# MDFahimAnjum/AliasFree-Diffusion-Models-PyTorch

Hardware: AMD Instinct MI355X
Metric: train_step_images_per_sec (higher is better)
Workload: dtype f32; 1 GPU; CIFAR-10 32x32x3 synthetic, UNet variant=3 (Config D), batch 256/GPU, T=1000, AdamW lr 3e-4, random-init weights (seed 42); global_batch=256, parallelism=dp1, hip_graph=True, launch_mode=lanes

## Files before the change

### aliasfree-diffusion-models-pytorch_amd/csrc/conv.hip

```cpp
#include <cstdlib>
#include <algorithm>
#include "common.h"

namespace afd {

using f32x16 = __attribute__((ext_vector_type(16))) float;

static inline int gs_grid(long total, int block = 256) {
  long g = (total + block - 1) / block;
  return (int)(g < 1 ? 1 : (g > 65536 ? 65536 : g));
}

template <int KS>
__global__ void conv_direct_fwd(const float* __restrict__ x, const float* __restrict__ w, const float* __restrict__ bias,
                                const float* __restrict__ res, float* __restrict__ y,
                                int Cin, int Cout, int H, int W, int act, long total) {
  constexpr int T = KS * KS, R = KS / 2;
  for (long i = blockIdx.x * (long)blockDim.x + threadIdx.x; i < total; i += (long)gridDim.x * blockDim.x) {
    const int xx = i % W, yy = (i / W) % H;
    const long bc = i / ((long)W * H);
    const int co = bc % Cout; const long b = bc / Cout;
    float acc = bias ? bias[co] : 0.f;
    for (int ci = 0; ci < Cin; ++ci) {
      const float* xp = x + (b * Cin + ci) * (long)H * W;
      const float* wp = w + ((long)co * Cin + ci) * T;
#pragma unroll
      for (int a = 0; a < KS; ++a) {
        const int r = yy + a - R;
        if (r < 0 || r >= H) continue;
#pragma unroll
        for (int c = 0; c < KS; ++c) {
          const int q = xx + c - R;
          if (q < 0 || q >= W) continue;
          acc += wp[a * KS + c] * xp[(long)r * W + q];
        }
      }
    }
    if (act == 1) acc = gelu_erf(acc);
    if (res) acc += res[i];
    y[i] = acc;
  }
}

template <int KS>
__global__ void conv_direct_dgrad(const float* __restrict__ dy, const float* __restrict__ w, float* __restrict__ dx,
                                  int Cin, int Cout, int H, int W, long total) {
  constexpr int T = KS * KS, R = KS / 2;
  for (long i = blockIdx.x * (long)blockDim.x + threadIdx.x; i < total; i += (long)gridDim.x * blockDim.x) {
    const int xx = i % W, yy = (i / W) % H;
    const long bc = i / ((long)W * H);
    const int ci = bc % Cin; const long b = bc / Cin;
    float acc = 0.f;
    for (int co = 0; co < Cout; ++co) {
      const float* gp = dy + (b * Cout + co) * (long)H * W;
      const float* wp = w + ((long)co * Cin + ci) * T;
#pragma unroll
      for (int a = 0; a < KS; ++a) {
        const int r = yy - a + R;
        if (r < 0 || r >= H) continue;
#pragma unroll
        for (int c = 0; c < KS; ++c) {
          const int q = xx - c + R;
          if (q < 0 || q >= W) continue;
          acc += wp[a * KS + c] * gp[(long)r * W + q];
        }
      }
    }
    dx[i] = acc;
  }
}

template <int KS>
__global__ __launch_bounds__(256) void conv_direct_wgrad(const float* __restrict__ x, const float* __restrict__ dy,
                                                         float* __restrict__ dw, int B, int Cin, int Cout, int H, int W,
                                                         int accumulate) {
  constexpr int T = KS * KS, R = KS / 2;
  __shared__ float red[16];
  const int co = blockIdx.x / Cin, ci = blockIdx.x % Cin;
  float acc[T];
#pragma unroll
  for (int t = 0; t < T; ++t) acc[t] = 0.f;
  const long HW = (long)H * W, P = (long)B * HW;
  for (long p = threadIdx.x; p < P; p += blockDim.x) {
    const long b = p / HW; const int pix = p % HW; const int yy = pix / W, xx = pix % W;
    const float g = dy[(b * Cout + co) * HW + pix];
    const float* xp = x + (b * Cin + ci) * HW;
#pragma unroll
    for (int a = 0; a < KS; ++a) {
      const int r = yy + a - R;
#pragma unroll
      for (int c = 0; c < KS; ++c) {
        const int q = xx + c - R;
        if (r >= 0 && r < H && q >= 0 && q < W) acc[a * KS + c] += g * xp[(long)r * W + q];
      }
    }
  }
#pragma unroll
  for (int t = 0; t < T; ++t) {
    const float s = block_sum(acc[t], red);
    if (threadIdx.x == 0) {
      float* o = dw + ((long)co * Cin + ci) * T + t;
      *o = accumulate ? *o + s : s;
    }
  }
}

__global__ __launch_bounds__(256) void conv_dbias_plane(const float* __restrict__ dy, float* __restrict__ part, long planes, int HW) {
  const long pl = ((long)blockIdx.x * blockDim.x + threadIdx.x) >> 6;
  const int lane = threadIdx.x & 63;
  if (pl >= planes) return;
  float s = 0.f;
  for (int i = lane; i < HW; i += 64) s += dy[pl * HW + i];
  s = wave_sum(s);
  if (lane == 0) part[pl] = s;
}
__global__ __launch_bounds__(256) void conv_dbias_final(const float* __restrict__ part, float* __restrict__ db, int B, int Cout, int accumulate) {
  __shared__ float red[8][33];
  const int c = blockIdx.x * 32 + (threadIdx.x & 31), g = threadIdx.x >> 5;
  float s = 0.f;
  if (c < Cout) for (int b = g; b < B; b += 8) s += part[(long)b * Cout + c];
  red[g][threadIdx.x & 31] = s;
  __syncthreads();
  if (g == 0 && c < Cout) {
    float t = 0.f;
#pragma unroll
    for (int k = 0; k < 8; ++k) t += red[k][threadIdx.x & 31];
    db[c] = accumulate ? db[c] + t : t;
  }
}

struct TileGeom {
  int TI, TR;
  int Wp;
  int BS;
  int XS;
};
static inline bool tile_ok(int H, int W, int PT) {
  const int HW = H * W;
  return (HW % PT == 0 && PT % W == 0) || (PT % HW == 0);
}
static inline TileGeom make_geom(int H, int W, int PT, int halo) {
  TileGeom g;
  const int HW = H * W;
  if (HW >= PT) { g.TI = 1; g.TR = PT / W; } else { g.TI = PT / HW; g.TR = H; }
  g.Wp = W + 2 * halo;
  g.BS = (g.TR + 2 * halo) * g.Wp;
  g.XS = g.TI * g.BS;
  return g;
}

__device__ __forceinline__ int pix_lds_off(int m, int W, const TileGeom& g, int halo) {
  const int per_img = g.TR * W;
  const int ti = m / per_img, r = (m % per_img) / W, c = m % W;
  return ti * g.BS + (r + halo) * g.Wp + (c + halo);
}

__device__ __forceinline__ void pos_source(int pos, long p0, int H, int W, long P, const TileGeom& g, int halo,
                                           long& img, int& off) {
  const int HW = H * W;
  const int ti = pos / g.BS, rem = pos % g.BS;
  const int rr = rem / g.Wp - halo, cc = rem % g.Wp - halo;
  const long pimg = p0 / HW + ti;
  const int row0 = (int)((p0 % HW) / W);
  const int y = row0 + rr;
  img = pimg; off = -1;
  if (cc < 0 || cc >= W || y < 0 || y >= H) return;
  if (pimg * HW >= P) return;
  off = y * W + cc;
}

template <int T, bool DGRAD, int BN, int KC, int NP>
struct Stager {
  static constexpr int WS = KC * T + 1;
  static constexpr int NW = BN * KC * T / 256;
  static_assert(BN * KC * T % 256 == 0, "weight chunk must divide over 256 threads");
  float wreg[NW];
  float xreg[NP][KC];
  unsigned long long wok;
  unsigned xok[NP];

  __device__ __forceinline__ void fetch(const float* __restrict__ w, const float* __restrict__ x, int k0, int K, int N,
                                        int n0, int HW, const int (&spos)[NP], const int (&soff)[NP],
                                        const long (&simg)[NP], int XS) {
    wok = 0;
#pragma unroll
    for (int e = 0; e < NW; ++e) {
      const int i = threadIdx.x + 256 * e;
      int n, kc, t;
      if (!DGRAD) { n = i / (KC * T); const int r = i % (KC * T); kc = r / T; t = r % T; }
      else        { kc = i / (BN * T); const int r = i % (BN * T); n = r / T; t = r % T; }
      const bool ok = (n0 + n < N) && (k0 + kc < K);
      const int nc = min(n0 + n, N - 1), kk = min(k0 + kc, K - 1);
      wreg[e] = DGRAD ? w[(unsigned)((kk * N + nc) * T + t)] : w[(unsigned)((nc * K + kk) * T + t)];
      wok |= (ok ? 1ull : 0ull) << e;
    }
#pragma unroll
    for (int p = 0; p < NP; ++p) {
      xok[p] = 0;
      if (spos[p] < XS) {
        const unsigned xb = soff[p] >= 0 ? (unsigned)simg[p] * (unsigned)(K * HW) + (unsigned)soff[p] : 0u;
#pragma unroll
        for (int kc = 0; kc < KC; ++kc) {
          xreg[p][kc] = x[xb + (unsigned)(min(k0 + kc, K - 1) * HW)];
          xok[p] |= ((soff[p] >= 0 && k0 + kc < K) ? 1u : 0u) << kc;
        }
      }
    }
  }

  __device__ __forceinline__ void commit(float* __restrict__ Ws, float* __restrict__ Xs, const int (&spos)[NP], int XS) const {
#pragma unroll
    for (int e = 0; e < NW; ++e) {
      const int i = threadIdx.x + 256 * e;
      int dst;
      if (!DGRAD) { dst = (i / (KC * T)) * WS + i % (KC * T); }
      else        { const int kc = i / (BN * T), r = i % (BN * T); dst = (r / T) * WS + kc * T + r % T; }
      Ws[dst] = ((wok >> e) & 1ull) ? wreg[e] : 0.f;
    }
#pragma unroll
    for (int p = 0; p < NP; ++p)
      if (spos[p] < XS) {
#pragma unroll
        for (int kc = 0; kc < KC; ++kc) Xs[kc * XS + spos[p]] = ((xok[p] >> kc) & 1u) ? xreg[p][kc] : 0.f;
      }
  }
};

template <int GEO> struct Geo { static constexpr int XS = 0, Wp = 0; };
template <> struct Geo<1> { static constexpr int XS = 204, Wp = 34; };
template <> struct Geo<2> { static constexpr int XS = 180, Wp = 18; };
template <> struct Geo<3> { static constexpr int XS = 200, Wp = 10; };
template <> struct Geo<4> { static constexpr int XS = 288, Wp = 6; };
template <> struct Geo<5> { static constexpr int XS = 128, Wp = 0; };

template <int T, bool DGRAD, int BN, int KC, int GEO>
__global__ __launch_bounds__(256) void conv_mfma(const float* __restrict__ x, const float* __restrict__ w,
                                                 const float* __restrict__ bias, const float* __restrict__ res,
                                                 float* __restrict__ y, int B, int K, int N, int H, int W, int act,
                                                 TileGeom g) {
  constexpr int PT = 128, HALO = (T == 9) ? 1 : 0;
  constexpr int TM = (BN == 64) ? 2 : 1;
  constexpr int WS = KC * T + 1;
  constexpr int NP = (T == 9) ? 2 : 1;
  constexpr int NW = BN * KC * T / 256;
  static_assert(BN * KC * T % 256 == 0, "weight chunk must divide over 256 threads");
  const int XS = GEO ? Geo<GEO>::XS : g.XS;
  const int Wp = GEO ? Geo<GEO>::Wp : g.Wp;
  extern __shared__ __attribute__((aligned(16))) float smem[];
  const int BUF = BN * WS + KC * XS;
  const int HW = H * W;
  const long P = (long)B * HW;
  const long p0 = (long)blockIdx.y * PT;
  const int n0 = blockIdx.x * BN;
  const int lane = threadIdx.x & 63, wv = threadIdx.x >> 6;
  const int nw = (BN == 64) ? (wv >> 1) * 32 : 0;
  const int mw = (BN == 64) ? (wv & 1) * 64 : wv * 32;
  const int half = lane >> 5, l31 = lane & 31;

  unsigned wsrc[NW]; int wdst[NW]; unsigned wmask = 0;
  int wkc[NW];
#pragma unroll
  for (int e = 0; e < NW; ++e) {
    const int i = threadIdx.x + 256 * e;
    int n, kc, t;
    if (!DGRAD) { n = i / (KC * T); const int r = i % (KC * T); kc = r / T; t = r % T; }
    else        { kc = i / (BN * T); const int r = i % (BN * T); n = r / T; t = r % T; }
    const int nc = min(n0 + n, N - 1);
    wsrc[e] = DGRAD ? (unsigned)((kc * N + nc) * T + t) : (unsigned)(nc * K * T + kc * T + t);
    wdst[e] = n * WS + kc * T + t;
    wkc[e] = kc;
    wmask |= (n0 + n < N ? 1u : 0u) << e;
  }
  int spos[NP]; unsigned xsrc[NP]; bool xval[NP];
#pragma unroll
  for (int e = 0; e < NP; ++e) {
    spos[e] = threadIdx.x + 256 * e;
    int soff = -1; long simg = 0;
    if (spos[e] < XS) pos_source(spos[e], p0, H, W, P, g, HALO, simg, soff);
    xval[e] = soff >= 0;
    xsrc[e] = xval[e] ? (unsigned)simg * (unsigned)(K * HW) + (unsigned)soff : 0u;
  }
  const int wstep = DGRAD ? N * T : T;
  int lbase[TM];
#pragma unroll
  for (int mt = 0; mt < TM; ++mt) lbase[mt] = half * XS + pix_lds_off(mw + mt * 32 + l31, W, g, HALO);
  const int abase = (nw + l31) * WS + half * T;

  float wreg[NW], xreg[NP][KC];
  auto fetch = [&](int k0) {
    const float* __restrict__ wk = w + (long)k0 * wstep;
    const float* __restrict__ xk = x + (long)k0 * HW;
    if (k0 + KC <= K) {
#pragma unroll
      for (int e = 0; e < NW; ++e) wreg[e] = wk[wsrc[e]];
#pragma unroll
      for (int p = 0; p < NP; ++p)
        if (spos[p] < XS) {
#pragma unroll
          for (int kc = 0; kc < KC; ++kc) xreg[p][kc] = xk[xsrc[p] + (unsigned)(kc * HW)];
        }
    } else {
#pragma unroll
      for (int e = 0; e < NW; ++e) wreg[e] = (k0 + wkc[e] < K) ? wk[wsrc[e]] : 0.f;
#pragma unroll
      for (int p = 0; p < NP; ++p)
        if (spos[p] < XS) {
#pragma unroll
          for (int kc = 0; kc < KC; ++kc) xreg[p][kc] = (k0 + kc < K) ? xk[xsrc[p] + (unsigned)(kc * HW)] : 0.f;
        }
    }
  };
  auto commit = [&](float* __restrict__ buf) {
    float* __restrict__ Ws = buf;
    float* __restrict__ Xs = buf + BN * WS;
#pragma unroll
    for (int e = 0; e < NW; ++e) Ws[wdst[e]] = ((wmask >> e) & 1u) ? wreg[e] : 0.f;
#pragma unroll
    for (int p = 0; p < NP; ++p)
      if (spos[p] < XS) {
#pragma unroll
        for (int kc = 0; kc < KC; ++kc) Xs[kc * XS + spos[p]] = xval[p] ? xreg[p][kc] : 0.f;
      }
  };

  f32x16 acc[TM];
#pragma unroll
  for (int mt = 0; mt < TM; ++mt)
#pragma unroll
    for (int r = 0; r < 16; ++r) acc[mt][r] = 0.f;

  fetch(0);
  commit(smem);
  if (KC < K) fetch(KC);
  __syncthreads();
  int cur = 0;
  for (int k0 = 0; k0 < K; k0 += KC, cur ^= 1) {
    if (k0 + KC < K) {
      commit(smem + (cur ^ 1) * BUF);
      if (k0 + 2 * KC < K) fetch(k0 + 2 * KC);
    }
    const float* __restrict__ Ws = smem + cur * BUF;
    const float* __restrict__ Xs = Ws + BN * WS;
#pragma unroll
    for (int t = 0; t < T; ++t) {
      const int toff = (T == 9) ? ((t / 3 - 1) * Wp + (t % 3 - 1)) : 0;
      const int tw = DGRAD ? (T - 1 - t) : t;
#pragma unroll
      for (int k2 = 0; k2 < KC / 2; ++k2) {
        const float a = Ws[abase + 2 * k2 * T + tw];
#pragma unroll
        for (int mt = 0; mt < TM; ++mt)
          acc[mt] = __builtin_amdgcn_mfma_f32_32x32x2f32(a, Xs[lbase[mt] + 2 * k2 * XS + toff], acc[mt], 0, 0, 0);
      }
    }
    __syncthreads();
  }
#pragma unroll
  for (int mt = 0; mt < TM; ++mt) {
    const long p = p0 + mw + mt * 32 + l31;
    if (p >= P) continue;
    const long b = p / HW; const int pix = p % HW;
#pragma unroll
    for (int r = 0; r < 16; ++r) {
      const int n = n0 + nw + (r & 3) + 8 * (r >> 2) + 4 * half;
      if (n >= N) continue;
      const long idx = (b * N + n) * (long)HW + pix;
      float v = acc[mt][r];
      if (bias) v += bias[n];
      if (act == 1) v = gelu_erf(v);
      if (res) v += res[idx];
      y[idx] = v;
    }
  }
}

template <int T, bool DGRAD>
__global__ __launch_bounds__(256) void conv_mfma_sk(const float* __restrict__ x, const float* __restrict__ w,
                                                    const float* __restrict__ bias, const float* __restrict__ res,
                                                    float* __restrict__ y, int B, int K, int N, int H, int W, int act,
                                                    TileGeom g) {
  constexpr int PT = 64, BN = 32, KC = 32, KW = KC / 4, TM = 2, HALO = (T == 9) ? 1 : 0;
  constexpr int WS = KC * T + 1;
  extern __shared__ __attribute__((aligned(16))) float smem[];
  float* Ws = smem;
  float* Xs = smem + BN * WS;
  const int HW = H * W;
  const long P = (long)B * HW;
  const long p0 = (long)blockIdx.y * PT;
  const int n0 = blockIdx.x * BN;
  const int lane = threadIdx.x & 63, wv = threadIdx.x >> 6;
  const int half = lane >> 5, l31 = lane & 31;

  int spos[1] = {(int)threadIdx.x}, soff[1] = {-1}; long simg[1] = {0};
  if (spos[0] < g.XS) pos_source(spos[0], p0, H, W, P, g, HALO, simg[0], soff[0]);
  int poff[TM];
#pragma unroll
  for (int mt = 0; mt < TM; ++mt) poff[mt] = pix_lds_off(mt * 32 + l31, W, g, HALO);

  f32x16 acc[TM];
#pragma unroll
  for (int mt = 0; mt < TM; ++mt)
#pragma unroll
    for (int r = 0; r < 16; ++r) acc[mt][r] = 0.f;

  Stager<T, DGRAD, BN, KC, 1> st;
  st.fetch(w, x, 0, K, N, n0, HW, spos, soff, simg, g.XS);
  for (int k0 = 0; k0 < K; k0 += KC) {
    __syncthreads();
    st.commit(Ws, Xs, spos, g.XS);
    __syncthreads();
    if (k0 + KC < K) st.fetch(w, x, k0 + KC, K, N, n0, HW, spos, soff, simg, g.XS);
#pragma unroll
    for (int t = 0; t < T; ++t) {
      const int toff = (T == 9) ? ((t / 3 - 1) * g.Wp + (t % 3 - 1)) : 0;
      const int tw = DGRAD ? (T - 1 - t) : t;
#pragma unroll
      for (int k2 = 0; k2 < KW / 2; ++k2) {
        const int kc = wv * KW + 2 * k2 + half;
        const float a = Ws[l31 * WS + kc * T + tw];
#pragma unroll
        for (int mt = 0; mt < TM; ++mt)
          acc[mt] = __builtin_amdgcn_mfma_f32_32x32x2f32(a, Xs[kc * g.XS + poff[mt] + toff], acc[mt], 0, 0, 0);
      }
    }
  }
  __syncthreads();
  float* red = smem;
#pragma unroll
  for (int mt = 0; mt < TM; ++mt)
#pragma unroll
    for (int r = 0; r < 16; ++r) red[((wv * TM + mt) * 16 + r) * 64 + lane] = acc[mt][r];
  __syncthreads();
#pragma unroll
  for (int e = 0; e < (TM * 16 * 64) / 256; ++e) {
    const int idx = threadIdx.x + 256 * e;
    const int mt = idx / 1024, r = (idx / 64) % 16, ln = idx % 64;
    float v = (red[idx] + red[idx + 2048]) + (red[idx + 4096] + red[idx + 6144]);
    const long p = p0 + mt * 32 + (ln & 31);
    const int n = n0 + (r & 3) + 8 * (r >> 2) + 4 * (ln >> 5);
    if (p < P && n < N) {
      const long b = p / HW; const int pix = p % HW;
      const long o = (b * N + n) * (long)HW + pix;
      if (bias) v += bias[n];
      if (act == 1) v = gelu_erf(v);
      if (res) v += res[o];
      y[o] = v;
    }
  }
}

template <int T, int WNn, int WCn, int NPB, int NW>
__global__ __launch_bounds__(64 * NW) void conv_wgrad_mfma(const float* __restrict__ x, const float* __restrict__ dy,
                                                       float* __restrict__ part, float* __restrict__ bias_part,
                                                       int B, int Cin, int Cout, int H, int W,
                                                       int chunks_per_split, int nchunks, TileGeom g) {
  constexpr int PT = 64, HALO = (T == 9) ? 1 : 0, S1 = PT + 1;
  constexpr int WK = NW / (WNn * WCn), BNo = 32 * WNn, BCi = 32 * WCn, NT_ = 64 * NW;
  constexpr int NG = BNo / NW;
  constexpr int NM = BCi / (2 * NW);
  extern __shared__ __attribute__((aligned(16))) float smem[];
  const int XSP = g.XS | 1;
  float* Gs = smem;
  float* Xs = smem + BNo * S1;
  int* Po = reinterpret_cast<int*>(Xs + BCi * XSP);
  const int HW = H * W;
  const long P = (long)B * HW;
  const int n0 = blockIdx.x * BNo, c0 = blockIdx.y * BCi, split = blockIdx.z;
  const int lane = threadIdx.x & 63, wv = threadIdx.x >> 6;
  const int wn = wv % WNn, wc = (wv / WNn) % WCn, wk = wv / (WNn * WCn);
  const int nw = wn * 32, cw = wc * 32;
  const int half = lane >> 5, l31 = lane & 31;
  const bool active = (n0 + nw < Cout) && (c0 + cw < Cin);

  if (threadIdx.x < PT) Po[threadIdx.x] = pix_lds_off(threadIdx.x, W, g, HALO);

  const int pp = threadIdx.x & 63, ng = threadIdx.x >> 6;
  const int gdb = (HW >= PT) ? 0 : pp / HW;
  const int gpix = (HW >= PT) ? pp : pp % HW;
  const int px = threadIdx.x & 31, cg = threadIdx.x >> 5;
  int p_ti[NPB], p_rr[NPB], p_cc[NPB];
#pragma unroll
  for (int e = 0; e < NPB; ++e) {
    const int pos = px + 32 * e;
    const int ti = pos / g.BS, rem = pos % g.BS;
    p_ti[e] = pos < g.XS ? ti : -1;
    p_rr[e] = rem / g.Wp - HALO;
    p_cc[e] = rem % g.Wp - HALO;
  }

  float gv[NG], xv[NPB][NM];
  unsigned gok, xok[NPB];
  int f_img, f_pix, f_row;
  auto fetch = [&]() {
    {
      const int b = f_img + gdb;
      const bool pin = b < B;
      const unsigned gb = pin ? (unsigned)(b * Cout) * (unsigned)HW + (unsigned)(f_pix + gpix) : 0u;
      gok = 0;
#pragma unroll
      for (int e = 0; e < NG; ++e) {
        const int n = n0 + ng + NW * e;
        gv[e] = dy[gb + (unsigned)(min(n, Cout - 1) * HW)];
        gok |= ((pin && n < Cout) ? 1u : 0u) << e;
      }
    }
#pragma unroll
    for (int e = 0; e < NPB; ++e) {
      xok[e] = 0;
      if (p_ti[e] >= 0) {
        const int img = f_img + p_ti[e];
        const int yy = f_row + p_rr[e];
        const bool ok = p_cc[e] >= 0 && p_cc[e] < W && yy >= 0 && yy < H && img < B;
        const unsigned xb = ok ? (unsigned)(img * Cin) * (unsigned)HW + (unsigned)(yy * W + p_cc[e]) : 0u;
#pragma unroll
        for (int m = 0; m < NM; ++m) {
          const int c = c0 + cg + 2 * NW * m;
          xv[e][m] = x[xb + (unsigned)(min(c, Cin - 1) * HW)];
          xok[e] |= ((ok && c < Cin) ? 1u : 0u) << m;
        }
      }
    }
    if (HW >= PT) {
      f_pix += PT; f_row += g.TR;
      if (f_pix >= HW) { f_pix = 0; f_row = 0; ++f_img; }
    } else {
      f_img += g.TI;
    }
  };
  auto commit = [&]() {
#pragma unroll
    for (int e = 0; e < NG; ++e) Gs[(ng + NW * e) * S1 + pp] = ((gok >> e) & 1u) ? gv[e] : 0.f;
#pragma unroll
    for (int e = 0; e < NPB; ++e)
      if (p_ti[e] >= 0) {
#pragma unroll
        for (int m = 0; m < NM; ++m) Xs[(cg + 2 * NW * m) * XSP + px + 32 * e] = ((xok[e] >> m) & 1u) ? xv[e][m] : 0.f;
      }
  };

  f32x16 acc[T];
#pragma unroll
  for (int t = 0; t < T; ++t)
#pragma unroll
    for (int r = 0; r < 16; ++r) acc[t][r] = 0.f;
  const bool do_bias = bias_part != nullptr && blockIdx.y == 0;
  float bsum = 0.f;

  const int cbeg = split * chunks_per_split;
  const int cend = min(nchunks, cbeg + chunks_per_split);
  {
    const unsigned pc0 = (unsigned)cbeg * PT;
    f_img = (int)(pc0 / (unsigned)HW);
    f_pix = (int)(pc0 % (unsigned)HW);
    f_row = f_pix / W;
  }
  if (cbeg < cend) fetch();
  for (int ch = cbeg; ch < cend; ++ch) {
    __syncthreads();
    commit();
    __syncthreads();
    if (ch + 1 < cend) fetch();
    if (do_bias) {
      const int bn = threadIdx.x >> 2, bq = threadIdx.x & 3;
      if (bn < BNo) {
        float t = 0.f;
#pragma unroll
        for (int j = 0; j < 16; ++j) t += Gs[bn * S1 + bq * 16 + j];
        bsum += t;
      }
    }
    if (active) {
#pragma unroll 4
      for (int s = wk * (PT / 2 / WK); s < (wk + 1) * (PT / 2 / WK); ++s) {
        const int pix = 2 * s + half;
        const float a = Gs[(nw + l31) * S1 + pix];
        const int xo = (cw + l31) * XSP + Po[pix];
#pragma unroll
        for (int t = 0; t < T; ++t) {
          const int toff = (T == 9) ? ((t / 3 - 1) * g.Wp + (t % 3 - 1)) : 0;
          acc[t] = __builtin_amdgcn_mfma_f32_32x32x2f32(a, Xs[xo + toff], acc[t], 0, 0, 0);
        }
      }
    }
  }
  if (do_bias) {
    float t = bsum;
    t += __shfl_xor(t, 1, kWave);
    t += __shfl_xor(t, 2, kWave);
    const int bn = threadIdx.x >> 2;
    if ((threadIdx.x & 3) == 0 && bn < BNo && n0 + bn < Cout) bias_part[(long)split * Cout + n0 + bn] = t;
  }
  float* out = part + (long)split * Cout * Cin * T;
  if (WK == 1) {
    if (!active) return;
    const int ci = c0 + cw + l31;
    if (ci < Cin) {
#pragma unroll
      for (int r = 0; r < 16; ++r) {
        const int n = n0 + nw + (r & 3) + 8 * (r >> 2) + 4 * half;
        if (n >= Cout) continue;
#pragma unroll
        for (int t = 0; t < T; ++t) out[((long)t * Cout + n) * Cin + ci] = acc[t][r];
      }
    }
  } else {
    float* red = smem;
    constexpr int NB = WNn * WCn;
#pragma unroll
    for (int t = 0; t < T; ++t) {
      __syncthreads();
#pragma unroll
      for (int r = 0; r < 16; ++r) red[(wv * 16 + r) * 64 + lane] = acc[t][r];
      __syncthreads();
      for (int idx = threadIdx.x; idx < NB * 1024; idx += NT_) {
        const int blk = idx / 1024, r = (idx / 64) % 16, ln = idx % 64;
        float v = 0.f;
#pragma unroll
        for (int k = 0; k < WK; ++k) v += red[((k * NB + blk) * 16 + r) * 64 + ln];
        const int bn = blk % WNn, bc = blk / WNn;
        const int n = n0 + bn * 32 + (r & 3) + 8 * (r >> 2) + 4 * (ln >> 5);
        const int ci = c0 + bc * 32 + (ln & 31);
        if (n < Cout && ci < Cin) out[((long)t * Cout + n) * Cin + ci] = v;
      }
    }
  }
}

__global__ __launch_bounds__(256) void wgrad_reduce(const float* __restrict__ part, float* __restrict__ dw, long n, int splits,
                                                    const float* __restrict__ bias_part, float* __restrict__ db, int nb,
                                                    int accumulate, int T) {
  __shared__ float red[8][33];
  const long i = (long)blockIdx.x * 32 + (threadIdx.x & 31);
  const int g = threadIdx.x >> 5;
  const bool isw = i < n;
  const long j = isw ? i : i - n;
  const long stride = isw ? n : nb;
  const float* __restrict__ src = isw ? part : bias_part;
  float s0 = 0.f, s1 = 0.f, s2 = 0.f, s3 = 0.f;
  if (i < n + nb) {
    int k = g;
    for (; k + 24 < splits; k += 32) {
      s0 += src[(long)k * stride + j]; s1 += src[(long)(k + 8) * stride + j];
      s2 += src[(long)(k + 16) * stride + j]; s3 += src[(long)(k + 24) * stride + j];
    }
    for (; k < splits; k += 8) s0 += src[(long)k * stride + j];
  }
  red[g][threadIdx.x & 31] = (s0 + s1) + (s2 + s3);
  __syncthreads();
  if (g == 0 && i < n + nb) {
    float t = 0.f;
#pragma unroll
    for (int k = 0; k < 8; ++k) t += red[k][threadIdx.x & 31];
    const long plane = n / T;
    float* o = isw ? dw + (j % plane) * T + j / plane : db + j;
    *o = accumulate ? *o + t : t;
  }
}

__global__ __launch_bounds__(256) void wgrad_reduce4(const float* __restrict__ part, float* __restrict__ dw, long n, int splits,
                                                     const float* __restrict__ bias_part, float* __restrict__ db, int nb,
                                                     int accumulate, int T) {
  __shared__ float4 red4[8][32];
  const int l = threadIdx.x & 31, g = threadIdx.x >> 5;
  const long wblocks = n >> 7;
  if (blockIdx.x < wblocks) {
    const long j = ((long)blockIdx.x << 7) + 4 * l;
    const float4* __restrict__ src = reinterpret_cast<const float4*>(part + j);
    const long stride = n >> 2;
    float4 s0 = {0.f, 0.f, 0.f, 0.f}, s1 = s0, s2 = s0, s3 = s0;
    int k = g;
    for (; k + 24 < splits; k += 32) {
      const float4 a = src[(long)k * stride], b = src[(long)(k + 8) * stride], c = src[(long)(k + 16) * stride],
                   d = src[(long)(k + 24) * stride];
      s0.x += a.x; s0.y += a.y; s0.z += a.z; s0.w += a.w;
      s1.x += b.x; s1.y += b.y; s1.z += b.z; s1.w += b.w;
      s2.x += c.x; s2.y += c.y; s2.z += c.z; s2.w += c.w;
      s3.x += d.x; s3.y += d.y; s3.z += d.z; s3.w += d.w;
    }
    for (; k < splits; k += 8) {
      const float4 a = src[(long)k * stride];
      s0.x += a.x; s0.y += a.y; s0.z += a.z; s0.w += a.w;
    }
    red4[g][l] = make_float4((s0.x + s1.x) + (s2.x + s3.x), (s0.y + s1.y) + (s2.y + s3.y), (s0.z + s1.z) + (s2.z + s3.z),
                             (s0.w + s1.w) + (s2.w + s3.w));
    __syncthreads();
    if (threadIdx.x < 128) {
      const int e = threadIdx.x;
      float t = 0.f;
#pragma unroll
      for (int q = 0; q < 8; ++q) t += reinterpret_cast<const float*>(&red4[q][e >> 2])[e & 3];
      const long je = ((long)blockIdx.x << 7) + e, plane = n / T;
      float* o = dw + (je % plane) * T + je / plane;
      *o = accumulate ? *o + t : t;
    }
  } else {
    __shared__ float red[8][33];
    const long j = (long)(blockIdx.x - wblocks) * 32 + l;
    float s0 = 0.f;
    if (j < nb)
      for (int k = g; k < splits; k += 8) s0 += bias_part[(long)k * nb + j];
    red[g][l] = s0;
    __syncthreads();
    if (g == 0 && j < nb) {
      float t = 0.f;
#pragma unroll
      for (int q = 0; q < 8; ++q) t += red[q][l];
      db[j] = accumulate ? db[j] + t : t;
    }
  }
}

int fold_launch(const afd_fold_desc* descs, int n, hipStream_t s);

struct FoldSink { afd_fold_desc* out; int n; };
static int launch_wgrad_reduce(const float* part, float* dw, long n, int slabs, const float* bp, float* db, int nb, int accumulate,
                               int T, hipStream_t s, FoldSink* sink) {
  afd_fold_desc d[2];
  int nd = 0;
  d[nd++] = afd_fold_desc{part, dw, n, n, n / T, (long)T, slabs, accumulate};
  if (nb > 0) d[nd++] = afd_fold_desc{bp, db, (long)nb, (long)nb, (long)nb, 1L, slabs, accumulate};
  if (sink) {
    for (int i = 0; i < nd; ++i) sink->out[sink->n++] = d[i];
    return AFD_OK;
  }
  return fold_launch(d, nd, s);
}

bool pw_launch(const float* in, const float* w, const float* bias, const float* res, float* out, int B, int K, int N, int P,
               int act, bool dgrad, hipStream_t s);
void pw_set_mode(int m);
int wino_plan(int B, int K, int N, int H, int W);
bool wino_conv(const float* x, const float* w, const float* bias, const float* res, float* y, float* U, int B, int K, int N, int H,
               int W, int act, bool dgrad, bool weights_ready, hipStream_t s);
void wino_set_mode(int m);
void wino_weights_launch(const float* w, float* Uf, float* Ud, int Cin, int Cout, int kinds, hipStream_t s);
bool bf3_ok(int B, int K, int N, int H, int W);
void bf3_set_mode(int m);
void direct_form_set(int m);
bool direct_form_is_bf3();
void h2_sk_set_mode(int m);
void h2_lds_set(int m);
void wino_weights_batched_launch(const afd_wino_desc* descs, const int* wg_desc, int n_wg, hipStream_t s);
void wino_set_grid(int g);
int wgrad_wino_plan(int B, int Cin, int Cout, int H, int W, int* bn, int* bk, int* cps, int* nchunks);
int wgrad_bf3_plan(int B, int Cin, int Cout, int H, int W, int* tps, int* ntiles);
int wgrad_bf3(const float* x, const float* dy, float* part, int B, int Cin, int Cout, int H, int W, hipStream_t s);
void wgrad_bf3_set_mode(int m);
void wgrad_arith_set(int m);
void wgrad_plan_target_set(long wgs);
bool wgrad_arith_is_bf3();
int wgrad_h2(const float* x, const float* dy, float* part, int B, int Cin, int Cout, int H, int W, hipStream_t s);
int pw_wgrad_h2(const float* x, const float* dy, float* part, float* bias_part, int B, int Cin, int Cout, int L, hipStream_t s);
bool ends_fwd(const float* x, const float* w, const float* bias, const float* res, float* y, int B, int Cin, int Cout, int H, int W,
              int ksize, int act, hipStream_t s);
bool ends_dgrad(const float* dy, const float* w, float* dx, int B, int Cin, int Cout, int H, int W, int ksize, hipStream_t s);
void ends_set_mode(int m);
int wgrad_cin3_plan(int B, int Cin, int Cout, int H, int W);
int wgrad_cin3(const float* x, const float* dy, float* part, int B, int Cin, int Cout, int H, int W, hipStream_t s);
void pw_wgrad_bf3_set_mode(int m);
int pw_wgrad_bf3_plan(int B, int Cin, int Cout, int L, int* sps, int* nsteps, int* nr, int* nt);
int pw_wgrad_bf3(const float* x, const float* dy, float* part, float* bias_part, int B, int Cin, int Cout, int L, hipStream_t s);
int wgrad_wino(const float* x, const float* dy, float* part, int B, int Cin, int Cout, int H, int W, hipStream_t s);
void wgrad_wino_set_mode(int m);

static inline bool use_mfma(int K, int N, int H, int W, int PT) { return N >= 8 && tile_ok(H, W, PT); }

static int g_conv_path = 0;

template <int T, bool DGRAD>
static int launch_mfma(const float* x, const float* w, const float* bias, const float* res, float* y,
                       int B, int K, int N, int H, int W, int act, hipStream_t s) {
  constexpr int KC = (T == 9) ? 8 : 32;
  const long P = (long)B * H * W;
  if (P * K >= (1L << 31) || (long)K * N * T >= (1L << 31)) return -1;
  const unsigned ptiles = (unsigned)((P + 127) / 128);
  const long wgs64 = (long)ptiles * ((N + 63) / 64), wgs32 = (long)ptiles * ((N + 31) / 32);
  bool use32 = N <= 32 || (wgs64 < 256 && wgs32 >= 256);
  const bool want_sk = g_conv_path == 2 || (g_conv_path == 0 && wgs64 < 256 && wgs32 < 256);
  if (g_conv_path == 1) use32 = N <= 32;
  if (want_sk && K >= 32 && tile_ok(H, W, 64)) {
    const TileGeom g = make_geom(H, W, 64, T == 9 ? 1 : 0);
    if (g.XS <= 256) {
      const size_t lds_main = sizeof(float) * (32 * (32 * T + 1) + (size_t)32 * g.XS);
      const size_t lds_red = sizeof(float) * 4 * 2 * 16 * 64;
      const size_t lds = lds_main > lds_red ? lds_main : lds_red;
      hipLaunchKernelGGL((conv_mfma_sk<T, DGRAD>), dim3((N + 31) / 32, (unsigned)((P + 63) / 64)), dim3(256), lds, s,
                         x, w, bias, res, y, B, K, N, H, W, act, g);
      return 0;
    }
  }
  const TileGeom g = make_geom(H, W, 128, T == 9 ? 1 : 0);
  if (g.XS > 512) return -1;
  int geo = 0;
  if (T == 1) geo = 5;
  else if (H == W && (W == 32 || W == 16 || W == 8 || W == 4)) geo = W == 32 ? 1 : (W == 16 ? 2 : (W == 8 ? 3 : 4));
  const size_t lds = 2 * sizeof(float) * ((use32 ? 32 : 64) * (KC * T + 1) + (size_t)KC * g.XS);
  const dim3 grid(use32 ? (N + 31) / 32 : (N + 63) / 64, ptiles);
#define AFD_CONV_LAUNCH(BN_, GEO_) hipLaunchKernelGGL((conv_mfma<T, DGRAD, BN_, KC, GEO_>), grid, dim3(256), lds, s, x, w, bias, res, y, B, K, N, H, W, act, g)
#define AFD_CONV_GEO(BN_)                                             \
  switch (geo) {                                                       \
    case 1: if constexpr (T == 9) { AFD_CONV_LAUNCH(BN_, 1); } break;  \
    case 2: if constexpr (T == 9) { AFD_CONV_LAUNCH(BN_, 2); } break;  \
    case 3: if constexpr (T == 9) { AFD_CONV_LAUNCH(BN_, 3); } break;  \
    case 4: if constexpr (T == 9) { AFD_CONV_LAUNCH(BN_, 4); } break;  \
    case 5: if constexpr (T == 1) { AFD_CONV_LAUNCH(BN_, 5); } break;  \
    default: AFD_CONV_LAUNCH(BN_, 0);                                  \
  }
  if (!use32) { AFD_CONV_GEO(64) } else { AFD_CONV_GEO(32) }
#undef AFD_CONV_GEO
#undef AFD_CONV_LAUNCH
  return 0;
}

static int g_wgrad_nw = 0;
struct WgradPlan { int wnn, wcn, wk, splits, slabs, nchunks, cps, npb; };
static inline WgradPlan wgrad_plan(int B, int Cin, int Cout, int H, int W, int ksize) {
  WgradPlan p;
  p.wnn = Cout > 32 ? 2 : 1;
  p.wcn = Cin > 32 ? 2 : 1;
  p.wk = 4 / (p.wnn * p.wcn);
  p.nchunks = (int)(((long)B * H * W + 63) / 64);
  const long tiles = (long)((Cout + 32 * p.wnn - 1) / (32 * p.wnn)) * ((Cin + 32 * p.wcn - 1) / (32 * p.wcn));
  static const long target = [] { const char* e = getenv("AFD_WG_TARGET"); return e ? atol(e) : 256L; }();
  long s = target / tiles;
  if (s < 1) s = 1;
  if (s > p.nchunks) s = p.nchunks;
  p.cps = (int)((p.nchunks + s - 1) / s);
  p.splits = (int)((p.nchunks + p.cps - 1) / p.cps);
  p.slabs = p.splits;
  const TileGeom g = make_geom(H, W, 64, ksize == 3 ? 1 : 0);
  const int need = (g.XS + 31) / 32;
  p.npb = ksize == 1 ? 2 : (need <= 4 ? 4 : (need <= 5 ? 5 : 8));
  return p;
}

template <int T, int WNn, int WCn, int NPB>
static void launch_wgrad(const float* x, const float* dy, float* part, float* bias_part, int B, int Cin, int Cout, int H, int W,
                         const WgradPlan& p, const TileGeom& g, hipStream_t s) {
  const int nw = g_wgrad_nw ? g_wgrad_nw : ((p.cps >= 8 || (p.cps >= 4 && H * W >= 256)) ? 8 : 4);
  size_t lds = sizeof(float) * ((size_t)32 * WNn * 65 + (size_t)32 * WCn * (g.XS | 1)) + sizeof(int) * 64;
  const size_t red = sizeof(float) * nw * 16 * 64;
  if (WNn * WCn < nw && lds < red) lds = red;
  const dim3 grid((Cout + 32 * WNn - 1) / (32 * WNn), (Cin + 32 * WCn - 1) / (32 * WCn), p.splits);
  if (nw == 8)
    hipLaunchKernelGGL((conv_wgrad_mfma<T, WNn, WCn, NPB, 8>), grid, dim3(512), lds, s, x, dy, part, bias_part, B, Cin, Cout, H, W, p.cps, p.nchunks, g);
  else
    hipLaunchKernelGGL((conv_wgrad_mfma<T, WNn, WCn, NPB, 4>), grid, dim3(256), lds, s, x, dy, part, bias_part, B, Cin, Cout, H, W, p.cps, p.nchunks, g);
}

template <int T, int NPB>
static void launch_wgrad_roles(const float* x, const float* dy, float* part, float* bp, int B, int Cin, int Cout, int H, int W,
                               const WgradPlan& p, const TileGeom& g, hipStream_t s) {
  if (p.wnn == 2 && p.wcn == 2) launch_wgrad<T, 2, 2, NPB>(x, dy, part, bp, B, Cin, Cout, H, W, p, g, s);
  else if (p.wnn == 2) launch_wgrad<T, 2, 1, NPB>(x, dy, part, bp, B, Cin, Cout, H, W, p, g, s);
  else if (p.wcn == 2) launch_wgrad<T, 1, 2, NPB>(x, dy, part, bp, B, Cin, Cout, H, W, p, g, s);
  else launch_wgrad<T, 1, 1, NPB>(x, dy, part, bp, B, Cin, Cout, H, W, p, g, s);
}

}
using namespace afd;

extern "C" {

int afd_debug_conv_path(int mode) {
  if (mode >= 92 && mode <= 93) { ends_set_mode(mode - 92); return AFD_OK; }
  if (mode >= 88 && mode <= 89) { pw_wgrad_bf3_set_mode(mode - 88); return AFD_OK; }
  if (mode >= 84 && mode <= 86) { wgrad_bf3_set_mode(mode - 84); return AFD_OK; }
  if (mode >= 48 && mode <= 49) { wgrad_plan_target_set(mode == 48 ? 256 : 160); return AFD_OK; }
  if (mode >= 59 && mode <= 63) { h2_lds_set(mode == 59 ? 4 : (mode == 60 ? 1 : (mode == 61 ? 0 : mode - 60))); return AFD_OK; }
  if (mode == 73) { h2_sk_set_mode(2); return AFD_OK; }
  if (mode >= 74 && mode <= 75) { h2_sk_set_mode(mode - 74); return AFD_OK; }
  if (mode >= 78 && mode <= 79) { wgrad_arith_set(mode - 78); return AFD_OK; }
  if (mode >= 76 && mode <= 77) { direct_form_set(mode - 76); return AFD_OK; }
  if (mode >= 80 && mode <= 82) { bf3_set_mode(mode - 80); return AFD_OK; }
  if (mode >= 8 && mode <= 10) { pw_set_mode(mode - 8); return AFD_OK; }
  if (mode >= 100000 && mode < 200000) { wino_set_grid(mode - 100000); return AFD_OK; }
  if (mode >= 96 && mode <= 98) { wgrad_wino_set_mode(mode - 96); return AFD_OK; }
  if (mode >= 64 && mode <= 70) { wino_set_mode(mode - 64); return AFD_OK; }
  if (mode >= 32 && mode <= 34) { g_wgrad_nw = mode == 32 ? 4 : (mode == 33 ? 8 : 0); return AFD_OK; }
  AFD_REQUIRE(mode >= 0 && mode <= 2, "afd_debug_conv_path: mode must be 0 (auto), 1 (big tile), 2 (split-K tile), 8..10 (1x1 streaming auto/off/forced), 32..34 (wgrad waves 4/8/auto), 64..69 (Winograd fwd/dgrad auto/off/forced shapes) or 96..98 (Winograd wgrad auto/off/forced)");
  g_conv_path = mode;
  return AFD_OK;
}

int afd_conv_fwd(const float* x, const float* w, const float* bias, const float* res, float* y,
                 int B, int Cin, int Cout, int H, int W, int ksize, int act, afd_stream_t st) {
  AFD_REQUIRE(x && w && y && B > 0 && Cin > 0 && Cout > 0 && H > 0 && W > 0, "afd_conv_fwd: bad argument");
  AFD_REQUIRE(ksize == 1 || ksize == 3, "afd_conv_fwd: ksize %d not in {1,3}", ksize);
  AFD_REQUIRE(act == 0 || act == 1, "afd_conv_fwd: act must be 0 or 1");
  hipStream_t s = as_stream(st);
  if (ends_fwd(x, w, bias, res, y, B, Cin, Cout, H, W, ksize, act, s)) return check_launch("afd_conv_fwd");
  if (ksize == 1 && pw_launch(x, w, bias, res, y, B, Cin, Cout, H * W, act, false, s)) return check_launch("afd_conv_fwd");
  int rc = -1;
  if (use_mfma(Cin, Cout, H, W, 128))
    rc = ksize == 3 ? launch_mfma<9, false>(x, w, bias, res, y, B, Cin, Cout, H, W, act, s)
                    : launch_mfma<1, false>(x, w, bias, res, y, B, Cin, Cout, H, W, act, s);
  if (rc != 0) {
    const long total = (long)B * Cout * H * W;
    if (ksize == 3) hipLaunchKernelGGL(conv_direct_fwd<3>, dim3(gs_grid(total)), dim3(256), 0, s, x, w, bias, res, y, Cin, Cout, H, W, act, total);
    else hipLaunchKernelGGL(conv_direct_fwd<1>, dim3(gs_grid(total)), dim3(256), 0, s, x, w, bias, res, y, Cin, Cout, H, W, act, total);
  }
  return check_launch("afd_conv_fwd");
}

int afd_conv_dgrad(const float* dy, const float* w, float* dx, int B, int Cin, int Cout, int H, int W, int ksize, afd_stream_t st) {
  AFD_REQUIRE(dy && w && dx && B > 0 && Cin > 0 && Cout > 0 && H > 0 && W > 0, "afd_conv_dgrad: bad argument");
  AFD_REQUIRE(ksize == 1 || ksize == 3, "afd_conv_dgrad: ksize %d not in {1,3}", ksize);
  hipStream_t s = as_stream(st);
  if (ends_dgrad(dy, w, dx, B, Cin, Cout, H, W, ksize, s)) return check_launch("afd_conv_dgrad");
  if (ksize == 1 && pw_launch(dy, w, nullptr, nullptr, dx, B, Cout, Cin, H * W, 0, true, s)) return check_launch("afd_conv_dgrad");
  int rc = -1;
  if (use_mfma(Cout, Cin, H, W, 128))
    rc = ksize == 3 ? launch_mfma<9, true>(dy, w, nullptr, nullptr, dx, B, Cout, Cin, H, W, 0, s)
                    : launch_mfma<1, true>(dy, w, nullptr, nullptr, dx, B, Cout, Cin, H, W, 0, s);
  if (rc != 0) {
    const long total = (long)B * Cin * H * W;
    if (ksize == 3) hipLaunchKernelGGL(conv_direct_dgrad<3>, dim3(gs_grid(total)), dim3(256), 0, s, dy, w, dx, Cin, Cout, H, W, total);
    else hipLaunchKernelGGL(conv_direct_dgrad<1>, dim3(gs_grid(total)), dim3(256), 0, s, dy, w, dx, Cin, Cout, H, W, total);
  }
  return check_launch("afd_conv_dgrad");
}

size_t afd_conv3x3_wino_workspace_bytes(int B, int Cin, int Cout, int H, int W, int dgrad) {
  if (B <= 0 || Cin <= 0 || Cout <= 0 || H <= 0 || W <= 0) return 0;
  const int K = dgrad ? Cout : Cin, N = dgrad ? Cin : Cout;
  return (bf3_ok(B, K, N, H, W) || wino_plan(B, K, N, H, W)) ? sizeof(float) * 16 * (size_t)Cin * Cout : 0;
}

int afd_conv3x3_weight_kinds(int B, int Cin, int Cout, int H, int W) {
  if (B <= 0 || Cin <= 0 || Cout <= 0 || H <= 0 || W <= 0) return 0;
  const int k = (bf3_ok(B, Cin, Cout, H, W) ? 1 : 0) | (bf3_ok(B, Cout, Cin, H, W) ? 2 : 0);
  return k && direct_form_is_bf3() ? k | 4 : k;
}

int afd_conv3x3_wino_weights(const float* w, float* u_fwd, float* u_dgrad, int Cin, int Cout, int kinds, afd_stream_t st) {
  AFD_REQUIRE(w && (u_fwd || u_dgrad) && Cin > 0 && Cout > 0 && Cin % 8 == 0 && Cout % 8 == 0, "afd_conv3x3_wino_weights: bad argument");
  AFD_REQUIRE(kinds >= 0 && kinds <= 7 && (!(kinds & 4) || (kinds & 3)) && (!(kinds & 3) || (Cin % 16 == 0 && Cout % 16 == 0)), "afd_conv3x3_wino_weights: bad kinds %d", kinds);
  wino_weights_launch(w, u_fwd, u_dgrad, Cin, Cout, kinds, as_stream(st));
  return check_launch("afd_conv3x3_wino_weights");
}

int afd_conv3x3_wino_weights_batched(const afd_wino_desc* descs, const int* wg_desc, int n_wg, afd_stream_t st) {
  AFD_REQUIRE(descs && wg_desc && n_wg > 0, "afd_conv3x3_wino_weights_batched: bad argument");
  wino_weights_batched_launch(descs, wg_desc, n_wg, as_stream(st));
  return check_launch("afd_conv3x3_wino_weights_batched");
}

static int check_kinds(const char* who, int kinds, int B, int Cin, int Cout, int H, int W, int dgrad) {
  const int now = afd_conv3x3_weight_kinds(B, Cin, Cout, H, W);
  const int bit = dgrad ? 2 : 1;
  AFD_REQUIRE(kinds >= 0 && (kinds & bit) == (now & bit) && (!(now & bit) || (kinds & 4) == (now & 4)),
              "%s: the weight image was built as kinds %d, but a call with (B %d, %d -> %d, %dx%d) under the current settings reads kinds %d "
              "(rebuild it: afd_conv3x3_weight_kinds depends on the batch size and on afd_debug_conv_path)", who, kinds, B, Cin, Cout, H, W, now);
  return AFD_OK;
}

int afd_conv3x3_wino_fwd(const float* x, const float* w, const float* bias, const float* res, float* y,
                         int B, int Cin, int Cout, int H, int W, int act, void* workspace, int weights_ready, int kinds, afd_stream_t st) {
  AFD_REQUIRE(x && w && y && workspace && B > 0 && Cin > 0 && Cout > 0 && H > 0 && W > 0, "afd_conv3x3_wino_fwd: bad argument");
  AFD_REQUIRE(act == 0 || act == 1, "afd_conv3x3_wino_fwd: act must be 0 or 1");
  if (weights_ready && check_kinds("afd_conv3x3_wino_fwd", kinds, B, Cin, Cout, H, W, 0) != AFD_OK) return AFD_EINVAL;
  AFD_REQUIRE(wino_conv(x, w, bias, res, y, static_cast<float*>(workspace), B, Cin, Cout, H, W, act, false, weights_ready != 0, as_stream(st)),
              "afd_conv3x3_wino_fwd: shape (%d,%d->%d,%dx%d) is not covered (afd_conv3x3_wino_workspace_bytes returns 0 for it)", B, Cin, Cout, H, W);
  return check_launch("afd_conv3x3_wino_fwd");
}

int afd_conv3x3_wino_dgrad(const float* dy, const float* w, float* dx, const float* add_to_dx, int B, int Cin, int Cout, int H, int W,
                           void* workspace, int weights_ready, int kinds, afd_stream_t st) {
  AFD_REQUIRE(dy && w && dx && workspace && B > 0 && Cin > 0 && Cout > 0 && H > 0 && W > 0, "afd_conv3x3_wino_dgrad: bad argument");
  if (weights_ready && check_kinds("afd_conv3x3_wino_dgrad", kinds, B, Cin, Cout, H, W, 1) != AFD_OK) return AFD_EINVAL;
  AFD_REQUIRE(wino_conv(dy, w, nullptr, add_to_dx, dx, static_cast<float*>(workspace), B, Cout, Cin, H, W, 0, true, weights_ready != 0, as_stream(st)),
              "afd_conv3x3_wino_dgrad: shape (%d,%d->%d,%dx%d) is not covered", B, Cin, Cout, H, W);
  return check_launch("afd_conv3x3_wino_dgrad");
}

size_t afd_conv_wgrad_workspace_bytes(int B, int Cin, int Cout, int H, int W, int ksize) {
  if (B <= 0 || Cin <= 0 || Cout <= 0 || H <= 0 || W <= 0) return 0;
  size_t pw = 0;
  if (ksize == 1) {
    int a, b, c, d;
    pw = sizeof(float) * (size_t)pw_wgrad_bf3_plan(B, Cin, Cout, H * W, &a, &b, &c, &d) * ((size_t)Cout * Cin + Cout);
  }
  if (!tile_ok(H, W, 64)) return std::max(pw, sizeof(float) * (size_t)B * Cout);
  size_t slabs = wgrad_plan(B, Cin, Cout, H, W, ksize).slabs;
  if (ksize == 3) {
    int bn, bk, cps, nch;
    const size_t ws = (size_t)wgrad_wino_plan(B, Cin, Cout, H, W, &bn, &bk, &cps, &nch);
    if (ws > slabs) slabs = ws;
    const size_t wb = (size_t)wgrad_bf3_plan(B, Cin, Cout, H, W, &cps, &nch);
    if (wb > slabs) slabs = wb;
    const size_t wc = (size_t)wgrad_cin3_plan(B, Cin, Cout, H, W);
    if (wc > slabs) slabs = wc;
  }
  const size_t need = slabs * ((size_t)Cout * Cin * ksize * ksize + Cout);
  const size_t direct = (size_t)B * Cout;
  return std::max(pw, sizeof(float) * (need > direct ? need : direct));
}

int afd_conv_wgrad_form(int B, int Cin, int Cout, int H, int W, int ksize) {
  if (B <= 0 || Cin <= 0 || Cout <= 0 || H <= 0 || W <= 0) return 0;
  int a, b, c, d;
  if (ksize == 1) return pw_wgrad_bf3_plan(B, Cin, Cout, H * W, &a, &b, &c, &d) ? (wgrad_arith_is_bf3() ? 2 : 4) : 0;
  if (ksize != 3) return 0;
  if (wgrad_bf3_plan(B, Cin, Cout, H, W, &a, &b)) return wgrad_arith_is_bf3() ? 2 : 4;
  if (wgrad_cin3_plan(B, Cin, Cout, H, W)) return 3;
  return wgrad_wino_plan(B, Cin, Cout, H, W, &a, &b, &c, &d) ? 1 : 0;
}

static int conv_wgrad_impl(const float* x, const float* dy, float* dw, float* dbias, int B, int Cin, int Cout, int H, int W,
                           int ksize, int accumulate, void* workspace, FoldSink* sink, hipStream_t s, const char* who) {
  AFD_REQUIRE(x && dy && dw && B > 0 && Cin > 0 && Cout > 0 && H > 0 && W > 0, "%s: bad argument", who);
  AFD_REQUIRE(ksize == 1 || ksize == 3, "%s: ksize %d not in {1,3}", who, ksize);
  const int T = ksize * ksize;
  const TileGeom g = make_geom(H, W, 64, ksize == 3 ? 1 : 0);
  int rc = AFD_OK;
  if (ksize == 3 && !dbias && workspace) {
    float* part = static_cast<float*>(workspace);
    int slabs = wgrad_arith_is_bf3() ? wgrad_bf3(x, dy, part, B, Cin, Cout, H, W, s) : wgrad_h2(x, dy, part, B, Cin, Cout, H, W, s);
    if (!slabs) slabs = wgrad_cin3(x, dy, part, B, Cin, Cout, H, W, s);
    if (!slabs) slabs = wgrad_wino(x, dy, part, B, Cin, Cout, H, W, s);
    if (slabs) {
      const long n = (long)Cout * Cin * 9;
      rc = launch_wgrad_reduce(part, dw, n, slabs, nullptr, nullptr, 0, accumulate, 9, s, sink);
      return rc != AFD_OK ? rc : check_launch(who);
    }
  }
  if (ksize == 1 && workspace) {
    int a, b, c, d;
    const int slabs = pw_wgrad_bf3_plan(B, Cin, Cout, H * W, &a, &b, &c, &d);
    if (slabs) {
      float* part = static_cast<float*>(workspace);
      const long n = (long)Cout * Cin;
      float* bp = dbias ? part + (size_t)slabs * n : nullptr;
      if (wgrad_arith_is_bf3()) pw_wgrad_bf3(x, dy, part, bp, B, Cin, Cout, H * W, s);
      else pw_wgrad_h2(x, dy, part, bp, B, Cin, Cout, H * W, s);
      rc = launch_wgrad_reduce(part, dw, n, slabs, bp, dbias, dbias ? Cout : 0, accumulate, 1, s, sink);
      return rc != AFD_OK ? rc : check_launch(who);
    }
  }
  if (tile_ok(H, W, 64) && g.XS <= 256 && (long)B * H * W * (Cin > Cout ? Cin : Cout) < (1L << 31)) {
    AFD_REQUIRE(workspace, "%s: workspace is NULL", who);
    const WgradPlan p = wgrad_plan(B, Cin, Cout, H, W, ksize);
    float* part = static_cast<float*>(workspace);
    const long n = (long)Cout * Cin * T;
    float* bp = dbias ? part + (size_t)p.slabs * n : nullptr;
    if (ksize == 1) launch_wgrad_roles<1, 2>(x, dy, part, bp, B, Cin, Cout, H, W, p, g, s);
    else if (p.npb == 4) launch_wgrad_roles<9, 4>(x, dy, part, bp, B, Cin, Cout, H, W, p, g, s);
    else if (p.npb == 5) launch_wgrad_roles<9, 5>(x, dy, part, bp, B, Cin, Cout, H, W, p, g, s);
    else launch_wgrad_roles<9, 8>(x, dy, part, bp, B, Cin, Cout, H, W, p, g, s);
    rc = launch_wgrad_reduce(part, dw, n, p.slabs, bp, dbias, dbias ? Cout : 0, accumulate, T, s, sink);
    return rc != AFD_OK ? rc : check_launch(who);
  } else {
    const dim3 grid((unsigned)(Cout * Cin));
    if (ksize == 3) hipLaunchKernelGGL(conv_direct_wgrad<3>, grid, dim3(256), 0, s, x, dy, dw, B, Cin, Cout, H, W, accumulate);
    else hipLaunchKernelGGL(conv_direct_wgrad<1>, grid, dim3(256), 0, s, x, dy, dw, B, Cin, Cout, H, W, accumulate);
  }
  if (dbias) {
    AFD_REQUIRE(workspace, "%s: workspace is NULL", who);
    float* bp = static_cast<float*>(workspace);
    const long planes = (long)B * Cout;
    hipLaunchKernelGGL(conv_dbias_plane, dim3((unsigned)((planes + 3) / 4)), dim3(256), 0, s, dy, bp, planes, H * W);
    hipLaunchKernelGGL(conv_dbias_final, dim3((Cout + 31) / 32), dim3(256), 0, s, bp, dbias, B, Cout, accumulate);
  }
  return check_launch(who);
}

int afd_conv_wgrad(const float* x, const float* dy, float* dw, float* dbias, int B, int Cin, int Cout, int H, int W,
                   int ksize, int accumulate, void* workspace, afd_stream_t st) {
  return conv_wgrad_impl(x, dy, dw, dbias, B, Cin, Cout, H, W, ksize, accumulate, workspace, nullptr, as_stream(st), "afd_conv_wgrad");
}

int afd_conv_wgrad_partials(const float* x, const float* dy, float* dw, float* dbias, int B, int Cin, int Cout, int H, int W,
                            int ksize, int accumulate, void* workspace, afd_fold_desc* folds_out, int* n_folds, afd_stream_t st) {
  AFD_REQUIRE(folds_out && n_folds, "afd_conv_wgrad_partials: folds_out / n_folds are NULL");
  FoldSink sink{folds_out, 0};
  const int rc = conv_wgrad_impl(x, dy, dw, dbias, B, Cin, Cout, H, W, ksize, accumulate, workspace, &sink, as_stream(st), "afd_conv_wgrad_partials");
  *n_folds = sink.n;
  return rc;
}

}
```

### aliasfree-diffusion-models-pytorch_amd/csrc/h2.hip

```cpp
#include <algorithm>
#include <cstdint>
#include "common.h"
#include "h2_common.h"

namespace afd {

using f32x4 = __attribute__((ext_vector_type(4))) float;

#ifndef AFD_H2_ABL
#define AFD_H2_ABL 0
#endif
#ifndef AFD_H2_AQ
#define AFD_H2_AQ 2
#endif
#ifndef AFD_H2_PRIO
#define AFD_H2_PRIO 0
#endif
#ifndef AFD_H2_SLEEP
#define AFD_H2_SLEEP 0
#endif
#ifndef AFD_H2_LDSPAD
#define AFD_H2_LDSPAD 0
#endif
#ifndef AFD_H2_STAMP
#define AFD_H2_STAMP 0
#endif

__global__ __launch_bounds__(256) void h2_wscale(const float* __restrict__ w, void* Wf, void* Wd, int Cin, int Cout) {
  h2_wscale_rows(w, Wf, Wd, Cin, Cout, blockIdx.x * 4 + (threadIdx.x >> 6), gridDim.x * 4, threadIdx.x & 63);
}
__global__ __launch_bounds__(256) void h2_weights(const float* __restrict__ w, void* Wf, void* Wd, int Cin, int Cout) {
  h2_weights_block(w, Wf, Wd, Cin, Cout, blockIdx.x * 4 + (threadIdx.x >> 6), threadIdx.x & 63);
}

template <int S> struct H2Geo {
  static constexpr int TP = 128;
  static constexpr int IPT = S * S >= TP ? 1 : TP / (S * S);
  static constexpr int R = S * S >= TP ? TP / S : S;
  static constexpr int TPI = S * S >= TP ? S * S / TP : 1;
  static constexpr int Wp = S + 2, IMG = (R + 2) * Wp, NPIX = IPT * IMG;
  static constexpr int NPP = (NPIX + 15) / 16 * 16;
  static constexpr int KG = 4;
  static constexpr int TASKS = KG * NPIX, NE = (TASKS + 255) / 256;
  __device__ static void pixel(int blk, int l15, int& i, int& r, int& c) {
    if (S == 8) { i = blk >> 2; r = (blk & 3) + 4 * (l15 >> 3); c = l15 & 7; }
    else { const int q = blk * 16 + l15; i = q / (R * S); const int rem = q - i * (R * S); r = rem / S; c = rem - r * S; }
  }
};

template <int S, int NBLK>
__global__ __launch_bounds__(256, 2) void conv_h2(const float* __restrict__ x, const h8* __restrict__ Wp,
                                                  const float* __restrict__ bias, const float* __restrict__ res,
                                                  float* __restrict__ y, int B, int K, int N, int act) {
  using G = H2Geo<S>;
  constexpr int PSW = 2 * NBLK, NPIX = G::NPIX, NPP = G::NPP, NE = G::NE;
  extern __shared__ __attribute__((aligned(16))) uint8_t smem_raw[];
  h8* Xp = reinterpret_cast<h8*>(smem_raw);
  float* wmax = reinterpret_cast<float*>(smem_raw + (size_t)2 * G::KG * NPP * 16);
#if AFD_H2_SLEEP
  if (__builtin_amdgcn_s_getreg(6148) & 1) __builtin_amdgcn_s_sleep(AFD_H2_SLEEP);
#endif
#if AFD_H2_PRIO
  if (__builtin_amdgcn_s_getreg(6148) & 1) __builtin_amdgcn_s_setprio(AFD_H2_PRIO);
#endif
  const int tid = threadIdx.x, lane = tid & 63, wv = tid >> 6, kgl = lane >> 4, l15 = lane & 15;
  const int nb = wv % NBLK, pgrp = wv / NBLK;
  const int tile = blockIdx.x, n0 = (blockIdx.y * NBLK + nb) * 32;
  const int img0 = G::IPT > 1 ? tile * G::IPT : tile / G::TPI;
  const int row0 = G::IPT > 1 ? 0 : (tile % G::TPI) * G::R;
  const int HW = S * S;

  int s_src[NE];
  int s_dst[NE];
#pragma unroll
  for (int e = 0; e < NE; ++e) {
    const int t = tid + 256 * e;
    s_src[e] = -1; s_dst[e] = -1;
    if (t < G::TASKS) {
      const int kg = t / NPIX, ridx = t - kg * NPIX;
      const int i = ridx / G::IMG, rem = ridx - i * G::IMG, rr = rem / G::Wp, cc = rem - rr * G::Wp;
      const int yy = row0 + rr - 1, xx = cc - 1, b = img0 + i;
      s_dst[e] = kg * NPP + ridx;
      if (yy >= 0 && yy < S && xx >= 0 && xx < S && b < B) s_src[e] = ((i * K + 8 * kg) * S + yy) * S + xx;
    }
  }
  const float* xb = x + (long)img0 * K * HW;
  float xr[NE][8];
  auto fetch = [&](int k0) {
#pragma unroll
    for (int e = 0; e < NE; ++e) {
      const float* p = xb + (long)k0 * HW + (s_src[e] >= 0 ? s_src[e] : 0);
#pragma unroll
      for (int j = 0; j < 8; ++j) xr[e][j] = (S == 32 || s_src[e] >= 0) ? p[(long)j * HW] : 0.f;
    }
  };
  auto chunk_amax = [&]() {
    float m = 0.f;
#pragma unroll
    for (int e = 0; e < NE; ++e)
#pragma unroll
      for (int j = 0; j < 8; ++j) { xr[e][j] = s_src[e] >= 0 ? xr[e][j] : 0.f; m = fmaxf(m, fabsf(xr[e][j])); }
    m = wave_amax(m);
    if (lane == 0) wmax[wv] = m;
  };
  auto commit = [&](float s) {
#pragma unroll
    for (int e = 0; e < NE; ++e) {
      if (s_dst[e] < 0) continue;
      h8 p0, p1;
      h2_split8(xr[e], s, p0, p1);
      Xp[s_dst[e]] = p0;
      Xp[G::KG * NPP + s_dst[e]] = p1;
    }
  };

  int bbase[PSW];
#pragma unroll
  for (int ps = 0; ps < PSW; ++ps) {
    int i, r, c;
    G::pixel(pgrp * PSW + ps, l15, i, r, c);
    bbase[ps] = kgl * NPP + i * G::IMG + r * G::Wp + c;
  }
  f32x4 acc[2][PSW];
#pragma unroll
  for (int ns = 0; ns < 2; ++ns)
#pragma unroll
    for (int ps = 0; ps < PSW; ++ps) acc[ns][ps] = f32x4{0.f, 0.f, 0.f, 0.f};

  const int KS = K >> 5, nit = KS * 9;
  const long pstride = (long)9 * (K >> 3) * N;
  const h8* wl = Wp + (long)kgl * N + n0 + l15;
  auto a_load = [&](h8 (&a)[2][2], int it) {
    const int ks = it / 9, tap = it - ks * 9;
    const long r = ((long)tap * (K >> 3) + 4 * ks) * N;
#pragma unroll
    for (int ns = 0; ns < 2; ++ns) { a[ns][0] = wl[r + 16 * ns]; a[ns][1] = wl[pstride + r + 16 * ns]; }
  };
  constexpr int AQ = AFD_H2_AQ;
  h8 aq[AQ][2][2];
#pragma unroll
  for (int d = 0; d < AQ; ++d)
    if (d < nit) a_load(aq[d], d);

  float sx = __uint_as_float(kH2ScaleCapBits);
  fetch(0);
  int it = 0;
  for (int k0 = 0; k0 < K; k0 += 32) {
    const bool stage = !(AFD_H2_ABL & 8) || k0 == 0;
    if (stage) chunk_amax();
    __syncthreads();
    if (stage) {
      const float m = fmaxf(fmaxf(wmax[0], wmax[1]), fmaxf(wmax[2], wmax[3]));
      const float sn = fminf(sx, h2_scale_for(m));
      if (sn != sx) {
        const float f = sn * h2_inv_pow2(sx);
#pragma unroll
        for (int ns = 0; ns < 2; ++ns)
#pragma unroll
          for (int ps = 0; ps < PSW; ++ps) acc[ns][ps] *= f;
        sx = sn;
      }
    }
    if (stage) commit(sx);
    __syncthreads();
    h8 bc[2], bn[2];
    bc[0] = Xp[bbase[0]]; bc[1] = Xp[G::KG * NPP + bbase[0]];
#pragma unroll
    for (int tap = 0; tap < 9; ++tap) {
      h8 a[2][2];
#pragma unroll
      for (int ns = 0; ns < 2; ++ns) { a[ns][0] = aq[0][ns][0]; a[ns][1] = aq[0][ns][1]; }
#pragma unroll
      for (int d = 0; d + 1 < AQ; ++d)
#pragma unroll
        for (int ns = 0; ns < 2; ++ns) { aq[d][ns][0] = aq[d + 1][ns][0]; aq[d][ns][1] = aq[d + 1][ns][1]; }
      if (it + AQ < nit && !(AFD_H2_ABL & 2)) a_load(aq[AQ - 1], it + AQ);
      ++it;
      if (tap == 0 && k0 + 32 < K && !(AFD_H2_ABL & 4)) fetch(k0 + 32);
#pragma unroll
      for (int ps = 0; ps < PSW; ++ps) {
        const int u = tap * PSW + ps + 1;
        if (u < 9 * PSW && !(AFD_H2_ABL & 16)) {
          const int tn = u / PSW, pn = u % PSW;
          const int o = bbase[pn] + (tn / 3) * G::Wp + (tn % 3);
          bn[0] = Xp[o]; bn[1] = Xp[G::KG * NPP + o];
        } else if (AFD_H2_ABL & 16) { bn[0] = bc[0]; bn[1] = bc[1]; }
        __builtin_amdgcn_sched_barrier(0);
#pragma unroll
        for (int ns = 0; ns < 2; ++ns) {
          if (AFD_H2_ABL & 1) { asm volatile("" :: "v"(a[ns][0]), "v"(a[ns][1]), "v"(bc[0]), "v"(bc[1])); continue; }
          acc[ns][ps] = __builtin_amdgcn_mfma_f32_16x16x32_f16(a[ns][0], bc[0], acc[ns][ps], 0, 0, 0);
          acc[ns][ps] = __builtin_amdgcn_mfma_f32_16x16x32_f16(a[ns][1], bc[0], acc[ns][ps], 0, 0, 0);
          acc[ns][ps] = __builtin_amdgcn_mfma_f32_16x16x32_f16(a[ns][0], bc[1], acc[ns][ps], 0, 0, 0);
        }
        __builtin_amdgcn_sched_barrier(0);
        bc[0] = bn[0]; bc[1] = bn[1];
      }
    }
  }

  if ((AFD_H2_ABL & 32) && act != 77) return;
  const float* isw = reinterpret_cast<const float*>(reinterpret_cast<const uint8_t*>(Wp) + h2_scale_offset_bytes(K, N));
  const float isx = h2_inv_pow2(sx);
  __syncthreads();
  float* T = reinterpret_cast<float*>(smem_raw) + wv * (32 * 36);
  const int cn = lane >> 3, cm = lane & 7;
  float sw[4], bv[4];
#pragma unroll
  for (int it = 0; it < 4; ++it) { sw[it] = isw[n0 + 8 * it + cn]; bv[it] = bias ? bias[n0 + 8 * it + cn] : 0.f; }
#pragma unroll
  for (int pp = 0; pp < PSW / 2; ++pp) {
#pragma unroll
    for (int h = 0; h < 2; ++h)
#pragma unroll
      for (int ns = 0; ns < 2; ++ns)
#pragma unroll
        for (int rg = 0; rg < 4; ++rg) T[(16 * ns + 4 * kgl + rg) * 36 + 16 * h + l15] = acc[ns][2 * pp + h][rg] * isx;
    int i, r, c;
    G::pixel(pgrp * PSW + 2 * pp + (cm >> 2), 4 * (cm & 3), i, r, c);
    const int b = img0 + i;
#pragma unroll
    for (int it = 0; it < 4; ++it) {
      const int nn = n0 + 8 * it + cn;
      f32x4 v = *reinterpret_cast<const f32x4*>(T + (8 * it + cn) * 36 + 4 * cm);
      if (b >= B) continue;
      const long o = ((long)b * N + nn) * HW + (row0 + r) * S + c;
#pragma unroll
      for (int e = 0; e < 4; ++e) {
        float u = v[e] * sw[it] + bv[it];
        if (act == 1) u = gelu_erf(u);
        v[e] = u;
      }
      if (res) v += *reinterpret_cast<const f32x4*>(res + o);
      *reinterpret_cast<f32x4*>(y + o) = v;
    }
  }
}

using f32x16 = __attribute__((ext_vector_type(16))) float;

template <int S, int TP> struct H2LGeo {
  static constexpr int IPT = S * S >= TP ? 1 : TP / (S * S);
  static constexpr int R = S * S >= TP ? TP / S : S;
  static constexpr int TPI = S * S >= TP ? S * S / TP : 1;
  static constexpr int Wp = S + 2, IMG = (R + 2) * Wp, NPIX = IPT * IMG;
  static constexpr int NPP = (NPIX + 15) / 16 * 16;
  static constexpr int KG = 4, TASKS = KG * NPIX, NE = (TASKS + 255) / 256;
  __device__ static void pixel(int blk, int l31, int& i, int& r, int& c) {
    if (S == 8) { i = blk >> 1; r = 2 * (blk & 1) + ((l31 >> 4) & 1) + 4 * ((l31 >> 3) & 1); c = l31 & 7; }
    else { const int q = blk * 32 + l31; i = q / (R * S); const int rem = q - i * (R * S); r = rem / S; c = rem - r * S; }
  }
};

template <int S, int TP, int NB>
__global__ __launch_bounds__(256, 2) void conv_h2l(const float* __restrict__ x, const h8* __restrict__ Wp,
                                                   const float* __restrict__ bias, const float* __restrict__ res,
                                                   float* __restrict__ y, int B, int K, int N, int act) {
  using G = H2LGeo<S, TP>;
  constexpr int NT = 32 * NB, PGR = 4 / NB, PB = TP / 32 / PGR;
  constexpr int NPIX = G::NPIX, NPP = G::NPP, NE = G::NE;
  constexpr int XREC = 2 * G::KG * NPP;
  constexpr int AROW = 2 * 3 * 4 * NT;
  constexpr int CPW = AROW / 64 / 4;
  extern __shared__ __attribute__((aligned(16))) uint8_t smem_raw[];
  h8* Xp = reinterpret_cast<h8*>(smem_raw);
  h8* Ab = Xp + XREC;
  float* wmax = reinterpret_cast<float*>(Ab + 2 * AROW);
  const int tid = threadIdx.x, lane = tid & 63, wv = tid >> 6, l31 = lane & 31, lh = lane >> 5;
  const int nb = wv % NB, pgrp = wv / NB;
  const int tile = blockIdx.x, n0w = blockIdx.y * NT, n0 = n0w + 32 * nb;
  const int img0 = G::IPT > 1 ? tile * G::IPT : tile / G::TPI;
  const int row0 = G::IPT > 1 ? 0 : (tile % G::TPI) * G::R;
  const int HW = S * S;
#if AFD_H2_SLEEP
  if (((blockIdx.y * gridDim.x + blockIdx.x) >> 8) & 1) { for (int z = 0; z < AFD_H2_SLEEP / 100; ++z) __builtin_amdgcn_s_sleep(100); }
#endif
#if AFD_H2_STAMP
  long* stamp = tid == 0 ? reinterpret_cast<long*>(const_cast<float*>(res)) + ((long)blockIdx.y * gridDim.x + blockIdx.x) * 16 : nullptr;
  int si = 0;
  res = nullptr;
#define AFD_STAMP() do { if (stamp) stamp[si] = (long)__builtin_amdgcn_s_memtime(); ++si; } while (0)
  if (stamp) stamp[15] = __builtin_amdgcn_s_getreg(6148 | (15 << 11));
  AFD_STAMP();
#else
#define AFD_STAMP() do { } while (0)
#endif

  int s_src[NE], s_dst[NE];
#pragma unroll
  for (int e = 0; e < NE; ++e) {
    const int t = tid + 256 * e;
    s_src[e] = -1; s_dst[e] = -1;
    if (t < G::TASKS) {
      const int kg = t / NPIX, ridx = t - kg * NPIX;
      const int i = ridx / G::IMG, rem = ridx - i * G::IMG, rr = rem / G::Wp, cc = rem - rr * G::Wp;
      const int yy = row0 + rr - 1, xx = cc - 1, b = img0 + i;
      s_dst[e] = kg * NPP + ridx;
      if (yy >= 0 && yy < S && xx >= 0 && xx < S && b < B) s_src[e] = ((i * K + 8 * kg) * S + yy) * S + xx;
    }
  }
  const float* xb = x + (long)img0 * K * HW;
  float xr[NE][8];
  auto fetch = [&](int k0) {
#pragma unroll
    for (int e = 0; e < NE; ++e) {
      const float* p = xb + (long)k0 * HW + (s_src[e] >= 0 ? s_src[e] : 0);
#pragma unroll
      for (int j = 0; j < 8; ++j) xr[e][j] = p[(long)j * HW];
    }
  };
  auto chunk_amax = [&]() {
    float m = 0.f;
#pragma unroll
    for (int e = 0; e < NE; ++e)
#pragma unroll
      for (int j = 0; j < 8; ++j) { xr[e][j] = s_src[e] >= 0 ? xr[e][j] : 0.f; m = fmaxf(m, fabsf(xr[e][j])); }
    m = wave_amax(m);
    if (lane == 0) wmax[wv] = m;
  };
  auto commit = [&](float s) {
#pragma unroll
    for (int e = 0; e < NE; ++e) {
      if (s_dst[e] < 0) continue;
      h8 p0, p1;
      h2_split8(xr[e], s, p0, p1);
      Xp[s_dst[e]] = p0;
      Xp[G::KG * NPP + s_dst[e]] = p1;
    }
  };

  const int K8 = K >> 3;
  int soff[CPW];
#pragma unroll
  for (int d = 0; d < CPW; ++d) {
    const int c = wv * CPW + d;
    const int pt = NT == 64 ? c >> 2 : c >> 1, kg = NT == 64 ? c & 3 : 2 * (c & 1) + lh, n = NT == 64 ? lane : l31;
    const int pc = pt / 3, tx = pt - 3 * pc;
    soff[d] = ((pc * 9 + tx) * K8 + kg) * N + n0w + n;
  }
  auto dma_row = [&](int q) {
    const int ks = q / 3, ty = q - 3 * ks;
    const h8* src = Wp + (long)(ty * 3 * K8 + 4 * ks) * N;
    h8* dst = Ab + (q & 1) * AROW + wv * CPW * 64;
#pragma unroll
    for (int d = 0; d < CPW; ++d)
      __builtin_amdgcn_global_load_lds((const __attribute__((address_space(1))) void*)(src + soff[d]),
                                       (__attribute__((address_space(3))) void*)(dst + d * 64), 16, 0, 0);
  };
#define AFD_ROW_END(younger)                                                                                              \
  do {                                                                                                                    \
    __builtin_amdgcn_sched_barrier(0);                                                                                    \
    __builtin_amdgcn_s_waitcnt(((younger) & 15) | 0x0F70 | (((younger) >> 4) << 14));                \
    asm volatile("" ::: "memory");                                                                                        \
    __builtin_amdgcn_s_barrier();                                                                                         \
    asm volatile("" ::: "memory");                                                                                        \
    __builtin_amdgcn_sched_barrier(0);                                                                                    \
  } while (0)

  dma_row(0);
  fetch(0);
  AFD_STAMP();

  int bbase[PB];
#pragma unroll
  for (int pb = 0; pb < PB; ++pb) {
    int i, r, c;
    G::pixel(pgrp * PB + pb, l31, i, r, c);
    bbase[pb] = lh * NPP + i * G::IMG + r * G::Wp + c;
  }
  const int abase = lh * NT + 32 * nb + l31;
  f32x16 acc[PB];
#pragma unroll
  for (int pb = 0; pb < PB; ++pb)
#pragma unroll
    for (int j = 0; j < 16; ++j) acc[pb][j] = 0.f;

  const int KS = K >> 5, nrows = 3 * KS;
  float sx = __uint_as_float(kH2ScaleCapBits);
  AFD_STAMP();
  int q = 0;
  for (int k0 = 0; k0 < K; k0 += 32) {
    chunk_amax();
    __builtin_amdgcn_sched_barrier(0);
    __builtin_amdgcn_s_waitcnt(0x0F70);
    __builtin_amdgcn_sched_barrier(0);
    if (k0 < 64) AFD_STAMP();
    __syncthreads();
    {
      const float m = fmaxf(fmaxf(wmax[0], wmax[1]), fmaxf(wmax[2], wmax[3]));
      const float sn = fminf(sx, h2_scale_for(m));
      if (sn != sx) {
        const float f = sn * h2_inv_pow2(sx);
#pragma unroll
        for (int pb = 0; pb < PB; ++pb) acc[pb] *= f;
        sx = sn;
      }
    }
    commit(sx);
    __syncthreads();
    if (k0 < 64) AFD_STAMP();
#pragma unroll
    for (int ty = 0; ty < 3; ++ty, ++q) {
      if (q + 1 < nrows) dma_row(q + 1);
      const bool prefetch = ty == 1 && k0 + 32 < K;
      if (prefetch) fetch(k0 + 32);
      const h8* Ar = Ab + (q & 1) * AROW + abase;
      constexpr int U = 3 * 2 * PB;
      h8 ac[2], an[2], bc[2], bn[2];
      ac[0] = Ar[0]; ac[1] = Ar[3 * 4 * NT];
      bc[0] = Xp[bbase[0] + ty * G::Wp]; bc[1] = Xp[G::KG * NPP + bbase[0] + ty * G::Wp];
#pragma unroll
      for (int u = 0; u < U; ++u) {
        const int pb = u % PB;
        if (u + 1 < U) {
          const int un = u + 1, txn = un / (2 * PB), khn = (un / PB) % 2, pbn = un % PB;
          if (pbn == 0) { an[0] = Ar[(txn * 4 + 2 * khn) * NT]; an[1] = Ar[((3 + txn) * 4 + 2 * khn) * NT]; }
          const int o = bbase[pbn] + ty * G::Wp + txn + 2 * khn * NPP;
          bn[0] = Xp[o]; bn[1] = Xp[G::KG * NPP + o];
        }
        __builtin_amdgcn_sched_barrier(0);
        acc[pb] = __builtin_amdgcn_mfma_f32_32x32x16_f16(ac[0], bc[0], acc[pb], 0, 0, 0);
        acc[pb] = __builtin_amdgcn_mfma_f32_32x32x16_f16(ac[1], bc[0], acc[pb], 0, 0, 0);
        acc[pb] = __builtin_amdgcn_mfma_f32_32x32x16_f16(ac[0], bc[1], acc[pb], 0, 0, 0);
        __builtin_amdgcn_sched_barrier(0);
        if (u + 1 < U) {
          if ((u + 1) % PB == 0) { ac[0] = an[0]; ac[1] = an[1]; }
          bc[0] = bn[0]; bc[1] = bn[1];
        }
      }
      if (ty == 0) AFD_ROW_END(0);
      if (ty == 1) { if (prefetch) AFD_ROW_END(NE * 8); else AFD_ROW_END(0); }
      if (k0 < 64) AFD_STAMP();
    }
  }

  const float* isw = reinterpret_cast<const float*>(reinterpret_cast<const uint8_t*>(Wp) + h2_scale_offset_bytes(K, N));
  const float isx = h2_inv_pow2(sx);
#if AFD_H2_STAMP
  si = 13;
#endif
  AFD_STAMP();
  __syncthreads();
  float* T = reinterpret_cast<float*>(smem_raw) + wv * (32 * 36);
  const int cn = lane >> 3, cm = lane & 7;
  float sw[4], bv[4];
#pragma unroll
  for (int it = 0; it < 4; ++it) { sw[it] = isw[n0 + 8 * it + cn]; bv[it] = bias ? bias[n0 + 8 * it + cn] : 0.f; }
#pragma unroll
  for (int pb = 0; pb < PB; ++pb) {
#pragma unroll
    for (int j = 0; j < 16; ++j) T[(8 * (j >> 2) + 4 * lh + (j & 3)) * 36 + l31] = acc[pb][j] * isx;
    int i, r, c;
    G::pixel(pgrp * PB + pb, 4 * cm, i, r, c);
    const int b = img0 + i;
#pragma unroll
    for (int it = 0; it < 4; ++it) {
      const int nn = n0 + 8 * it + cn;
      f32x4 v = *reinterpret_cast<const f32x4*>(T + (8 * it + cn) * 36 + 4 * cm);
      if (b >= B) continue;
      const long o = ((long)b * N + nn) * HW + (row0 + r) * S + c;
#pragma unroll
      for (int e = 0; e < 4; ++e) {
        float u = v[e] * sw[it] + bv[it];
        if (act == 1) u = gelu_erf(u);
        v[e] = u;
      }
      if (res) v += *reinterpret_cast<const f32x4*>(res + o);
      *reinterpret_cast<f32x4*>(y + o) = v;
    }
  }
  AFD_STAMP();
#undef AFD_STAMP
}

template <int S> struct SkGeo {
  static constexpr int IPS = S == 4 ? 2 : 1;
  static constexpr int R = 32 / (IPS * S);
  static constexpr int Wp = S + 2, IMG = (R + 2) * Wp, NPIX = IPS * IMG, NPP = (NPIX + 15) / 16 * 16;
  static constexpr int KG = 4, TASKS = KG * NPIX, NE = (TASKS + 63) / 64;
};

template <int S, int KSP>
__global__ __launch_bounds__(256, 2) void conv_h2_sk(const float* __restrict__ x, const h8* __restrict__ Wp,
                                                     const float* __restrict__ bias, const float* __restrict__ res,
                                                     float* __restrict__ y, int B, int K, int N, int act, int nslices) {
  using G = SkGeo<S>;
  constexpr int PSP = 4 / KSP, NPP = G::NPP, NE = G::NE, HW = S * S;
  extern __shared__ __attribute__((aligned(16))) uint8_t smem_raw[];
  const int tid = threadIdx.x, lane = tid & 63, wv = tid >> 6, kgl = lane >> 4, l15 = lane & 15;
  const int kw = wv % KSP, pw = wv / KSP;
  h8* Xw = reinterpret_cast<h8*>(smem_raw) + (size_t)wv * 2 * G::KG * NPP;
  float* red = reinterpret_cast<float*>(smem_raw + (size_t)4 * 2 * G::KG * NPP * 16);
  const int sl = blockIdx.x * PSP + pw, n0 = blockIdx.y * 32;
  const bool live = sl < nslices;
  const int img0 = S == 4 ? sl * 2 : sl / 2, row0 = S == 4 ? 0 : (sl & 1) * 4;

  int s_src[NE], s_dst[NE];
#pragma unroll
  for (int e = 0; e < NE; ++e) {
    const int t = lane + 64 * e;
    s_src[e] = -1; s_dst[e] = -1;
    if (t < G::TASKS) {
      const int kg = t / G::NPIX, ridx = t - kg * G::NPIX;
      const int i = ridx / G::IMG, rem = ridx - i * G::IMG, rr = rem / G::Wp, cc = rem - rr * G::Wp;
      const int yy = row0 + rr - 1, xx = cc - 1, b = img0 + i;
      s_dst[e] = kg * NPP + ridx;
      if (live && yy >= 0 && yy < S && xx >= 0 && xx < S && b < B) s_src[e] = ((i * K + 8 * kg) * S + yy) * S + xx;
    }
  }
  const float* xb = x + (long)(live ? img0 : 0) * K * HW;
  float xr[NE][8];
  auto fetch = [&](int k0) {
#pragma unroll
    for (int e = 0; e < NE; ++e) {
      const float* p = xb + (long)k0 * HW + (s_src[e] >= 0 ? s_src[e] : 0);
#pragma unroll
      for (int j = 0; j < 8; ++j) xr[e][j] = s_src[e] >= 0 ? p[(long)j * HW] : 0.f;
    }
  };
  int bbase[2];
#pragma unroll
  for (int ps = 0; ps < 2; ++ps) {
    const int q = ps * 16 + l15;
    const int i = q / (G::R * S), rem = q - i * (G::R * S), r = rem / S, c = rem - r * S;
    bbase[ps] = kgl * NPP + i * G::IMG + r * G::Wp + c;
  }
  f32x4 acc[2][2];
#pragma unroll
  for (int ns = 0; ns < 2; ++ns)
#pragma unroll
    for (int ps = 0; ps < 2; ++ps) acc[ns][ps] = f32x4{0.f, 0.f, 0.f, 0.f};

  const int KS = K >> 5;
  const long pstride = (long)9 * (K >> 3) * N;
  const h8* wl = Wp + (long)kgl * N + n0 + l15;
  float sx = __uint_as_float(kH2ScaleCapBits);
  if (kw < KS) fetch(32 * kw);
  for (int ks = kw; ks < KS; ks += KSP) {
    h8 ac[3][2][2], an[3][2][2];
    auto a_row = [&](h8 (&a)[3][2][2], int ty) {
#pragma unroll
      for (int tx = 0; tx < 3; ++tx) {
        const long r = ((long)(ty * 3 + tx) * (K >> 3) + 4 * ks) * N;
#pragma unroll
        for (int ns = 0; ns < 2; ++ns) { a[tx][ns][0] = wl[r + 16 * ns]; a[tx][ns][1] = wl[pstride + r + 16 * ns]; }
      }
    };
    a_row(ac, 0);
    {
      float m = 0.f;
#pragma unroll
      for (int e = 0; e < NE; ++e)
#pragma unroll
        for (int j = 0; j < 8; ++j) m = fmaxf(m, fabsf(xr[e][j]));
      const float sn = fminf(sx, h2_scale_for(wave_amax(m)));
      if (sn != sx) {
        const float f = sn * h2_inv_pow2(sx);
#pragma unroll
        for (int ns = 0; ns < 2; ++ns)
#pragma unroll
          for (int ps = 0; ps < 2; ++ps) acc[ns][ps] *= f;
        sx = sn;
      }
    }
#pragma unroll
    for (int e = 0; e < NE; ++e) {
      if (s_dst[e] < 0) continue;
      h8 p0, p1;
      h2_split8(xr[e], sx, p0, p1);
      Xw[s_dst[e]] = p0;
      Xw[G::KG * NPP + s_dst[e]] = p1;
    }
    if (ks + KSP < KS) fetch(32 * (ks + KSP));
#pragma unroll
    for (int ty = 0; ty < 3; ++ty) {
      if (ty < 2) a_row(an, ty + 1);
      __builtin_amdgcn_sched_barrier(0);
#pragma unroll
      for (int tx = 0; tx < 3; ++tx) {
#pragma unroll
        for (int ps = 0; ps < 2; ++ps) {
          const int o = bbase[ps] + ty * G::Wp + tx;
          const h8 b0 = Xw[o], b1 = Xw[G::KG * NPP + o];
#pragma unroll
          for (int ns = 0; ns < 2; ++ns) {
            acc[ns][ps] = __builtin_amdgcn_mfma_f32_16x16x32_f16(ac[tx][ns][0], b0, acc[ns][ps], 0, 0, 0);
            acc[ns][ps] = __builtin_amdgcn_mfma_f32_16x16x32_f16(ac[tx][ns][1], b0, acc[ns][ps], 0, 0, 0);
            acc[ns][ps] = __builtin_amdgcn_mfma_f32_16x16x32_f16(ac[tx][ns][0], b1, acc[ns][ps], 0, 0, 0);
          }
        }
      }
      __builtin_amdgcn_sched_barrier(0);
      if (ty < 2) {
#pragma unroll
        for (int tx = 0; tx < 3; ++tx)
#pragma unroll
          for (int ns = 0; ns < 2; ++ns) { ac[tx][ns][0] = an[tx][ns][0]; ac[tx][ns][1] = an[tx][ns][1]; }
      }
    }
  }
  {
    const float isx = h2_inv_pow2(sx);
#pragma unroll
    for (int ns = 0; ns < 2; ++ns)
#pragma unroll
      for (int ps = 0; ps < 2; ++ps)
#pragma unroll
        for (int rg = 0; rg < 4; ++rg) red[(wv * 16 + (ns * 2 + ps) * 4 + rg) * 64 + lane] = acc[ns][ps][rg] * isx;
  }
  __syncthreads();
  if (kw != 0 || !live) return;
  const float* isw = reinterpret_cast<const float*>(reinterpret_cast<const uint8_t*>(Wp) + h2_scale_offset_bytes(K, N));
#pragma unroll
  for (int ps = 0; ps < 2; ++ps) {
    const int q = ps * 16 + l15;
    const int i = q / (G::R * S), rem = q - i * (G::R * S), r = rem / S, c = rem - r * S;
    const int b = img0 + i;
    if (b >= B) continue;
#pragma unroll
    for (int ns = 0; ns < 2; ++ns) {
      const int nn = n0 + 16 * ns + 4 * kgl;
      const long o = ((long)b * N + nn) * HW + (row0 + r) * S + c;
#pragma unroll
      for (int rg = 0; rg < 4; ++rg) {
        float v = 0.f;
#pragma unroll
        for (int g = 0; g < KSP; ++g) v += red[((pw * KSP + g) * 16 + (ns * 2 + ps) * 4 + rg) * 64 + lane];
        v *= isw[nn + rg];
        if (bias) v += bias[nn + rg];
        if (act == 1) v = gelu_erf(v);
        if (res) v += res[o + (long)rg * HW];
        y[o + (long)rg * HW] = v;
      }
    }
  }
}

static int h2_nblk(long tiles, int N, int S) {
  static const long minwg = [] { const char* e = getenv("AFD_H2_MINWG"); return e ? atol(e) : 512L; }();
  for (int nb = S == 16 ? 4 : 2; nb > 1; nb >>= 1)
    if (N % (32 * nb) == 0 && tiles * (N / (32 * nb)) >= minwg) return nb;
  return 1;
}

void h2_weights_launch(const float* w, void* Wf, void* Wd, int Cin, int Cout, hipStream_t s) {
  const int rows = (Wf ? Cout : 0) + (Wd ? Cin : 0);
  hipLaunchKernelGGL(h2_wscale, dim3((unsigned)((rows + 3) / 4)), dim3(256), 0, s, w, Wf, Wd, Cin, Cout);
  hipLaunchKernelGGL(h2_weights, dim3((unsigned)((Cin * Cout / 64 + 3) / 4)), dim3(256), 0, s, w, Wf, Wd, Cin, Cout);
}

template <int S, int NBLK>
static void h2_launch_t(const float* x, const void* Wp, const float* bias, const float* res, float* y, int B, int K, int N, int act,
                        hipStream_t s) {
  using G = H2Geo<S>;
  const size_t lds = (size_t)2 * G::KG * G::NPP * 16 + 16;
  const long tiles = G::IPT > 1 ? ((long)B + G::IPT - 1) / G::IPT : (long)B * G::TPI;
  hipLaunchKernelGGL((conv_h2<S, NBLK>), dim3((unsigned)tiles, (unsigned)(N / (32 * NBLK))), dim3(256), lds, s, x,
                     static_cast<const h8*>(Wp), bias, res, y, B, K, N, act);
}
template <int S, int KSP>
static void h2_sk_launch_t(const float* x, const void* Wp, const float* bias, const float* res, float* y, int B, int K, int N, int act,
                           hipStream_t s) {
  using G = SkGeo<S>;
  const size_t lds = (size_t)4 * 2 * G::KG * G::NPP * 16 + sizeof(float) * 4 * 16 * 64;
  const int nslices = (int)(((long)B * S * S + 31) / 32), psp = 4 / KSP;
  hipLaunchKernelGGL((conv_h2_sk<S, KSP>), dim3((unsigned)((nslices + psp - 1) / psp), (unsigned)(N / 32)), dim3(256), lds, s, x,
                     static_cast<const h8*>(Wp), bias, res, y, B, K, N, act, nslices);
}
bool h2_sk_ok(int B, int K, int N, int H, int W, bool force) {
  if (H != W || (W != 4 && W != 8) || K % 32 || N % 32 || K < 64) return false;
  if ((long)B * K * H * W >= (1L << 31) || (long)B * N * H * W >= (1L << 31)) return false;
  if (force) return true;
  const long slices = ((long)B * H * W + 31) / 32;
  const int ksp = K >= 128 ? 4 : 2;
  return ((slices + 4 / ksp - 1) / (4 / ksp)) * (N / 32) >= 128;
}
static int g_h2_lds = 1;
void h2_lds_set(int m) { g_h2_lds = m; }
template <int S, int TP, int NB>
static int h2l_launch_t(const float* x, const void* Wp, const float* bias, const float* res, float* y, int B, int K, int N, int act,
                        hipStream_t s) {
  using G = H2LGeo<S, TP>;
  const size_t lds = (size_t)(2 * G::KG * G::NPP + 2 * 2 * 3 * 4 * 32 * NB) * 16 + 16 + AFD_H2_LDSPAD;
  if (int rc = lds_opt_in(conv_h2l<S, TP, NB>, lds)) return rc;
  const long tiles = G::IPT > 1 ? ((long)B + G::IPT - 1) / G::IPT : (long)B * G::TPI;
  hipLaunchKernelGGL((conv_h2l<S, TP, NB>), dim3((unsigned)tiles, (unsigned)(N / (32 * NB))), dim3(256), lds, s, x,
                     static_cast<const h8*>(Wp), bias, res, y, B, K, N, act);
  return AFD_OK;
}
template <int S>
static int h2l_launch(const float* x, const void* Wp, const float* bias, const float* res, float* y, int B, int K, int N, int act,
                      hipStream_t s) {
  const long px = (long)B * S * S;
  if (g_h2_lds != 4 && N % 64 == 0 && (g_h2_lds == 2 || (g_h2_lds == 1 && ((px + 127) / 128) * (N / 64) >= 512)))
    return h2l_launch_t<S, 128, 2>(x, Wp, bias, res, y, B, K, N, act, s);
  if constexpr (S >= 16) {
    if (g_h2_lds == 3 || (g_h2_lds == 1 && ((px + 255) / 256) * (N / 32) >= 512)) return h2l_launch_t<S, 256, 1>(x, Wp, bias, res, y, B, K, N, act, s);
  }
  return h2l_launch_t<S, 128, 1>(x, Wp, bias, res, y, B, K, N, act, s);
}

void h2_conv(const float* x, const void* Wp, const float* bias, const float* res, float* y, int B, int K, int N, int S, int act,
             hipStream_t s, bool small) {
  if (small) {
    if (S == 4) { if (K >= 128) h2_sk_launch_t<4, 4>(x, Wp, bias, res, y, B, K, N, act, s); else h2_sk_launch_t<4, 2>(x, Wp, bias, res, y, B, K, N, act, s); }
    else { if (K >= 128) h2_sk_launch_t<8, 4>(x, Wp, bias, res, y, B, K, N, act, s); else h2_sk_launch_t<8, 2>(x, Wp, bias, res, y, B, K, N, act, s); }
    return;
  }
  if (g_h2_lds > 1 || (g_h2_lds == 1 && S == 32 && N % 64 != 0)) {
    if (S == 32) h2l_launch<32>(x, Wp, bias, res, y, B, K, N, act, s);
    else if (S == 16) h2l_launch<16>(x, Wp, bias, res, y, B, K, N, act, s);
    else h2l_launch<8>(x, Wp, bias, res, y, B, K, N, act, s);
    return;
  }
  const int nblk = h2_nblk(((long)B * S * S + 127) / 128, N, S);
#define AFD_H2(S_)                                                                      \
  if (nblk == 4 && S_ == 16) h2_launch_t<16, 4>(x, Wp, bias, res, y, B, K, N, act, s);  \
  else if (nblk == 2) h2_launch_t<S_, 2>(x, Wp, bias, res, y, B, K, N, act, s);         \
  else h2_launch_t<S_, 1>(x, Wp, bias, res, y, B, K, N, act, s)
  if (S == 32) { AFD_H2(32); } else if (S == 16) { AFD_H2(16); } else { AFD_H2(8); }
#undef AFD_H2
}

}
```

### aliasfree-diffusion-models-pytorch_amd/csrc/wino.hip

```cpp
#include <cstdlib>
#include "common.h"
#include "bf3_weights.h"
#include "h2_common.h"

namespace afd {

using f32x4 = __attribute__((ext_vector_type(4))) float;
using f32x2 = __attribute__((ext_vector_type(2))) float;

template <int S, int NT> struct WGeo {
  static constexpr int W = S, TPR = S / 2, TPI = TPR * TPR;
  static constexpr int TI = NT <= TPI ? 1 : NT / TPI;
  static constexpr int TROWS = NT <= TPI ? NT / TPR : TPR;
  static constexpr int GPI = NT <= TPI ? TPI / NT : 1;
  static constexpr int PXR = 2 * TROWS, Wp = S + 2, IMG = (PXR + 2) * Wp, RS = TI * IMG;
  static constexpr int RSP = RS + ((32 - RS % 64) + 64) % 64;
  static_assert(NT % TPR == 0 && (NT <= TPI ? TPI % NT == 0 : NT % TPI == 0), "tile group must be whole tile rows or whole images");
};

template <int OFF0, int OFF1>
__device__ __forceinline__ void lds_issue_pair(f32x2& a, f32x2& b, unsigned base) {
  asm volatile("ds_read_b64 %0, %2 offset:%3\n\tds_read_b64 %1, %2 offset:%4" : "=&v"(a), "=&v"(b) : "v"(base), "n"(OFF0), "n"(OFF1));
}
template <int N>
__device__ __forceinline__ void lds_wait(f32x2& a, f32x2& b) {
  asm volatile("s_waitcnt lgkmcnt(%2)" : "+v"(a), "+v"(b) : "n"(N));
}

__device__ __forceinline__ int kperm8(int k) { return 2 * (k & 3) + (k >> 2); }

__device__ __forceinline__ void wino_weights_block(const float* __restrict__ w, float* __restrict__ Uf, float* __restrict__ Ud,
                                                   int Cin, int Cout, int blk, int lane) {
  const int nci8 = Cin >> 3;
  if (blk >= nci8 * (Cout >> 3)) return;
  const int ci = (blk % nci8) * 8 + (lane & 7), co = (blk / nci8) * 8 + (lane >> 3);
  const float* p = w + ((long)co * Cin + ci) * 9;
  float g[9];
#pragma unroll
  for (int t = 0; t < 9; ++t) g[t] = p[t];
  float t[4][3], u[16];
#pragma unroll
  for (int c = 0; c < 3; ++c) {
    const float g0 = g[c], g1 = g[3 + c], g2 = g[6 + c];
    t[0][c] = g0;
    t[1][c] = 0.5f * (g0 + g1 + g2);
    t[2][c] = 0.5f * (g0 - g1 + g2);
    t[3][c] = g2;
  }
#pragma unroll
  for (int i = 0; i < 4; ++i) {
    const float a = t[i][0], b = t[i][1], c = t[i][2];
    u[4 * i + 0] = a;
    u[4 * i + 1] = 0.5f * (a + b + c);
    u[4 * i + 2] = 0.5f * (a - b + c);
    u[4 * i + 3] = c;
  }
  if (Uf) {
    float* o = Uf + ((long)(ci >> 3) * 16 * Cout + co) * 8 + kperm8(ci & 7);
    const long xs = (long)Cout * 8;
#pragma unroll
    for (int xi = 0; xi < 16; ++xi) o[xi * xs] = u[xi];
  }
  if (Ud) {
    float* o = Ud + ((long)(co >> 3) * 16 * Cin + ci) * 8 + kperm8(co & 7);
    const long xs = (long)Cin * 8;
#pragma unroll
    for (int i = 0; i < 4; ++i)
#pragma unroll
      for (int j = 0; j < 4; ++j) {
        const int pi = i == 0 ? 3 : (i == 3 ? 0 : i), pj = j == 0 ? 3 : (j == 3 ? 0 : j);
        o[(4 * i + j) * xs] = u[4 * pi + pj];
      }
  }
}

__global__ __launch_bounds__(256) void wino_weights(const float* __restrict__ w, float* __restrict__ Uf, float* __restrict__ Ud,
                                                    int Cin, int Cout) {
  wino_weights_block(w, Uf, Ud, Cin, Cout, blockIdx.x * 4 + (threadIdx.x >> 6), threadIdx.x & 63);
}


__global__ __launch_bounds__(256) void wino_weights_batched(const afd_wino_desc* __restrict__ descs, const int* __restrict__ wg_desc) {
  const afd_wino_desc d = descs[wg_desc[blockIdx.x]];
  const int blk = (blockIdx.x - d.first_wg) * 4 + (threadIdx.x >> 6), lane = threadIdx.x & 63;
  float* wf = (d.kinds & 1) ? nullptr : d.u_fwd; float* wd = (d.kinds & 2) ? nullptr : d.u_dgrad;
  if (wf || wd) wino_weights_block(d.w, wf, wd, d.Cin, d.Cout, blk, lane);
  void* bf = (d.kinds & 1) ? d.u_fwd : nullptr; void* bd = (d.kinds & 2) ? d.u_dgrad : nullptr;
  if (bf || bd) {
    if (d.kinds & 4) bf3_weights_block(d.w, static_cast<__bf16*>(bf), static_cast<__bf16*>(bd), d.Cin, d.Cout, blk, lane);
    else h2_weights_block(d.w, bf, bd, d.Cin, d.Cout, blk, lane);
  }
}
__global__ __launch_bounds__(256) void h2_wscale_batched(const afd_wino_desc* __restrict__ descs, const int* __restrict__ wg_desc) {
  const afd_wino_desc d = descs[wg_desc[blockIdx.x]];
  if (d.kinds & 4) return;
  void* bf = (d.kinds & 1) ? d.u_fwd : nullptr; void* bd = (d.kinds & 2) ? d.u_dgrad : nullptr;
  const int nw = 4 * ((d.Cin * d.Cout / 64 + 3) / 4);
  if (bf || bd) h2_wscale_rows(d.w, bf, bd, d.Cin, d.Cout, (blockIdx.x - d.first_wg) * 4 + (threadIdx.x >> 6), nw, threadIdx.x & 63);
}

template <int GEO, int BN, int NT>
__global__ __launch_bounds__(BN * NT / 8, BN * NT == 4096 ? 1 : 2) void conv_wino(const float* __restrict__ x, const float* __restrict__ U,
                                                    const float* __restrict__ bias, const float* __restrict__ res,
                                                    float* __restrict__ y, int B, int K, int N, int act, int items) {
  using G = WGeo<GEO, NT>;
  constexpr int KC = 8, SU = 10, NTH = BN * NT / 8;
  constexpr int W = G::W, H = G::W, HW = W * W, Wp = G::Wp, IMG = G::IMG, RS = G::RS, RSP = G::RSP;
  constexpr int NPOS = (RS + NTH - 1) / NTH;
  constexpr int NUV = 16 * BN * 2 / NTH;
  extern __shared__ __attribute__((aligned(16))) float smem[];
  constexpr int BUF = 16 * BN * SU + KC * RSP;
  float* Us = smem;
  float* Rs = Us + 16 * BN * SU;
  const int tid = threadIdx.x, lane = tid & 63, wv = tid >> 6;
  const int NB = N / BN;

  unsigned rsrc[NPOS]; unsigned rvalid = 0; unsigned usrc0 = 0;
  constexpr int XSTEP = NTH / (2 * BN);
  static_assert(NTH % (2 * BN) == 0 && XSTEP * NUV == 16, "U chunk must split into whole xi planes per pass");
  const int u_h = tid & 1, u_n = (tid >> 1) % BN, u_xi = tid / (2 * BN);
  const int udst0 = (((u_n >> 4) * 16 + u_xi) * 16 + (u_n & 15)) * SU + 4 * u_h;
  const long ustep = (long)XSTEP * N * 8;
  auto plan = [&](int w) {
    const int tg = w / NB, n0 = (w % NB) * BN;
    const int b0 = (G::TI == 1) ? tg / G::GPI : tg * G::TI;
    const int row0 = (G::TI == 1) ? (tg % G::GPI) * G::PXR : 0;
    rvalid = 0;
#pragma unroll
    for (int e = 0; e < NPOS; ++e) {
      const int pos = tid + NTH * e;
      bool ok = false; unsigned src = 0;
      if (pos < RS) {
        const int ti = pos / IMG, rem = pos % IMG;
        const int yy = row0 + rem / Wp - 1, xx = rem % Wp - 1, b = b0 + ti;
        ok = b < B && yy >= 0 && yy < H && xx >= 0 && xx < W;
        if (ok) src = (unsigned)(b * K) * (unsigned)HW + (unsigned)(yy * W + xx);
      }
      rsrc[e] = src; rvalid |= (ok ? 1u : 0u) << e;
    }
    usrc0 = (unsigned)((u_xi * N + n0 + u_n) * 8 + 4 * u_h);
  };
  const int wn = wv % (BN / 32), wt = wv / (BN / 32);
  const int li = lane & 15, lq = lane >> 4;
  const int tt = wt * 16 + li;
  const int poff = (tt / (G::TROWS * G::TPR)) * IMG + 2 * ((tt / G::TPR) % G::TROWS) * Wp + 2 * (tt % G::TPR);

  struct Regs { float r[NPOS][KC]; f32x4 u[NUV]; unsigned ok; };
  Regs S0, S1;
  auto fetch = [&](Regs& S, int c) {
    const float* __restrict__ xk = x + (long)c * KC * HW;
    const float* __restrict__ uk = U + (long)c * 16 * N * 8;
#pragma unroll
    for (int e = 0; e < NUV; ++e) S.u[e] = *reinterpret_cast<const f32x4*>(uk + e * ustep + usrc0);
#pragma unroll
    for (int e = 0; e < NPOS; ++e)
      if (tid + NTH * e < RS) {
#pragma unroll
        for (int kc = 0; kc < KC; ++kc) S.r[e][kc] = (xk + kc * HW)[rsrc[e]];
      }
    S.ok = rvalid;
  };
  auto commit = [&](const Regs& S, int stage) {
    float* Us = smem + stage * BUF;
    float* Rs = Us + 16 * BN * SU;
#pragma unroll
    for (int e = 0; e < NUV; ++e) {
      float2* d = reinterpret_cast<float2*>(Us + udst0 + e * (XSTEP * 16 * SU));
      d[0] = make_float2(S.u[e][0], S.u[e][1]);
      d[1] = make_float2(S.u[e][2], S.u[e][3]);
    }
#pragma unroll
    for (int e = 0; e < NPOS; ++e)
      if (tid + NTH * e < RS) {
        const bool ok = (S.ok >> e) & 1u;
#pragma unroll
        for (int kc = 0; kc < KC; ++kc) Rs[kc * RSP + tid + NTH * e] = ok ? S.r[e][kc] : 0.f;
      }
  };
  auto patch = [&](const float* Rs, int k, float (&v)[16]) {
    const float* r = Rs + k * RSP + poff;
    float d[4][4];
#pragma unroll
    for (int a = 0; a < 4; ++a) {
      const float2 lo = *reinterpret_cast<const float2*>(r + a * Wp);
      const float2 hi = *reinterpret_cast<const float2*>(r + a * Wp + 2);
      d[a][0] = lo.x; d[a][1] = lo.y; d[a][2] = hi.x; d[a][3] = hi.y;
    }
    float w[4][4];
#pragma unroll
    for (int j = 0; j < 4; ++j) {
      w[0][j] = d[0][j] - d[2][j];
      w[1][j] = d[1][j] + d[2][j];
      w[2][j] = d[2][j] - d[1][j];
      w[3][j] = d[1][j] - d[3][j];
    }
#pragma unroll
    for (int i = 0; i < 4; ++i) {
      v[4 * i + 0] = w[i][0] - w[i][2];
      v[4 * i + 1] = w[i][1] + w[i][2];
      v[4 * i + 2] = w[i][2] - w[i][1];
      v[4 * i + 3] = w[i][1] - w[i][3];
    }
  };
  const unsigned ap = (unsigned)(size_t)(Us + (wn * 2 * 256 + li) * SU + 2 * lq);
  const int o_ti = tt / (G::TROWS * G::TPR), o_ty = (tt / G::TPR) % G::TROWS, o_tx = tt % G::TPR;
  const int nchunks = K / KC;

  for (int w = blockIdx.x; w < items; w += gridDim.x) {
    plan(w);
    fetch(S0, 0);
    if (nchunks > 1) fetch(S1, 1);
    f32x4 acc[16][2];
#pragma unroll
    for (int xi = 0; xi < 16; ++xi)
#pragma unroll
      for (int h = 0; h < 2; ++h) acc[xi][h] = f32x4{0.f, 0.f, 0.f, 0.f};

    auto multiply = [&](int st) {
      const float* Rc = Rs + st * BUF;
      const unsigned apc = ap + (unsigned)(st * BUF * 4);
      f32x2 alo[2], ahi[2];
      lds_issue_pair<0, 256 * SU * 4>(alo[0], ahi[0], apc);
      float v0[16], v1[16];
      patch(Rc, lq, v0);
      patch(Rc, lq + 4, v1);
#pragma unroll
      for (int xi = 0; xi < 16; ++xi) {
        constexpr int STEP = 16 * SU * 4;
        f32x2& lo = alo[xi & 1]; f32x2& hi = ahi[xi & 1];
        if (xi < 15) {
          switch (xi) {
#define AFD_NEXT(X) case X: lds_issue_pair<(X + 1) * STEP, (X + 1) * STEP + 256 * SU * 4>(alo[(X + 1) & 1], ahi[(X + 1) & 1], apc); break;
            AFD_NEXT(0) AFD_NEXT(1) AFD_NEXT(2) AFD_NEXT(3) AFD_NEXT(4) AFD_NEXT(5) AFD_NEXT(6) AFD_NEXT(7)
            AFD_NEXT(8) AFD_NEXT(9) AFD_NEXT(10) AFD_NEXT(11) AFD_NEXT(12) AFD_NEXT(13) AFD_NEXT(14)
#undef AFD_NEXT
          }
          lds_wait<2>(lo, hi);
        } else {
          lds_wait<0>(lo, hi);
        }
        acc[xi][0] = __builtin_amdgcn_mfma_f32_16x16x4f32(lo[0], v0[xi], acc[xi][0], 0, 0, 0);
        acc[xi][1] = __builtin_amdgcn_mfma_f32_16x16x4f32(hi[0], v0[xi], acc[xi][1], 0, 0, 0);
        acc[xi][0] = __builtin_amdgcn_mfma_f32_16x16x4f32(lo[1], v1[xi], acc[xi][0], 0, 0, 0);
        acc[xi][1] = __builtin_amdgcn_mfma_f32_16x16x4f32(hi[1], v1[xi], acc[xi][1], 0, 0, 0);
      }
    };

    __syncthreads();
    commit(S0, 0);
    if (nchunks > 2) fetch(S0, 2);
    __syncthreads();
    for (int c = 0; c < nchunks; c += 2) {
      multiply(0);
      if (c + 1 < nchunks) {
        commit(S1, 1);
        if (c + 3 < nchunks) fetch(S1, c + 3);
        __syncthreads();
        multiply(1);
        if (c + 2 < nchunks) {
          commit(S0, 0);
          if (c + 4 < nchunks) fetch(S0, c + 4);
          __syncthreads();
        }
      }
    }

    const int tg = w / NB, n0 = (w % NB) * BN;
    const int ob = ((G::TI == 1) ? tg / G::GPI : tg * G::TI) + o_ti;
    const int row0 = (G::TI == 1) ? (tg % G::GPI) * G::PXR : 0;
    if (ob < B) {
      const int opix = (row0 + 2 * o_ty) * W + 2 * o_tx;
#pragma unroll
      for (int h = 0; h < 2; ++h)
#pragma unroll
        for (int r = 0; r < 4; ++r) {
          const int n = n0 + wn * 32 + 16 * h + 4 * lq + r;
          float tcol[4][2];
#pragma unroll
          for (int i = 0; i < 4; ++i) {
            const float m0 = acc[4 * i + 0][h][r], m1 = acc[4 * i + 1][h][r], m2 = acc[4 * i + 2][h][r], m3 = acc[4 * i + 3][h][r];
            tcol[i][0] = (m0 + m1) + m2;
            tcol[i][1] = (m1 - m2) - m3;
          }
          float y00 = (tcol[0][0] + tcol[1][0]) + tcol[2][0], y01 = (tcol[0][1] + tcol[1][1]) + tcol[2][1];
          float y10 = (tcol[1][0] - tcol[2][0]) - tcol[3][0], y11 = (tcol[1][1] - tcol[2][1]) - tcol[3][1];
          const unsigned idx = (unsigned)((ob * N + n) * HW + opix);
          if (bias) { const float bb = bias[n]; y00 += bb; y01 += bb; y10 += bb; y11 += bb; }
          if (act == 1) { y00 = gelu_erf(y00); y01 = gelu_erf(y01); y10 = gelu_erf(y10); y11 = gelu_erf(y11); }
          if (res) {
            const float2 r0 = *reinterpret_cast<const float2*>(res + idx), r1 = *reinterpret_cast<const float2*>(res + idx + W);
            y00 += r0.x; y01 += r0.y; y10 += r1.x; y11 += r1.y;
          }
          *reinterpret_cast<float2*>(y + idx) = make_float2(y00, y01);
          *reinterpret_cast<float2*>(y + idx + W) = make_float2(y10, y11);
        }
    }
  }
}

template <int S>
__global__ __launch_bounds__(256, 2) void conv_wino_sk(const float* __restrict__ x, const float* __restrict__ U,
                                                       const float* __restrict__ bias, const float* __restrict__ res,
                                                       float* __restrict__ y, int B, int K, int N, int act) {
  using G = WGeo<S, 16>;
  static_assert(G::GPI == 1, "tile groups must be whole images");
  constexpr int KC = 8, W = S, HW = S * S, Wp = G::Wp, IMG = G::IMG, RS = G::RS, RSP = G::RSP, TI = G::TI;
  constexpr int UPC = TI * S * (S / 4);
  static_assert(UPC == 16, "one chunk = 128 float4 pieces per wave");
  constexpr int DEPTH = 8;
  extern __shared__ __attribute__((aligned(16))) float smem[];
  const int lane = threadIdx.x & 63, wv = threadIdx.x >> 6;
  float* Rs = smem + wv * (KC * RSP);
  float* red = smem + 4 * KC * RSP;
  const int n0 = blockIdx.x * 32, tg = blockIdx.y, b0 = tg * TI;
  const int li = lane & 15, lq = lane >> 4;
  const int poff = (li / (G::TROWS * G::TPR)) * IMG + 2 * ((li / G::TPR) % G::TROWS) * Wp + 2 * (li % G::TPR);
  const int KS = K / 4, nchunks = KS / KC, kw = wv * KS;

  for (int i = lane; i < KC * RSP; i += 64) Rs[i] = 0.f;

  unsigned rsrc[2]; int rdst[2]; bool rok[2];
#pragma unroll
  for (int e = 0; e < 2; ++e) {
    const int u = lane + 64 * e, ch = u / UPC, q = u % UPC;
    const int ti = q / (S * (S / 4)), rr = (q / (S / 4)) % S, x4 = q % (S / 4);
    rok[e] = b0 + ti < B;
    rsrc[e] = rok[e] ? (unsigned)(((b0 + ti) * K + kw + ch) * HW + rr * W + 4 * x4) : 0u;
    rdst[e] = ch * RSP + ti * IMG + (rr + 1) * Wp + 1 + 4 * x4;
  }
  f32x4 rreg[2];
  auto fetch = [&](int c) {
    const float* xk = x + (long)c * KC * HW;
#pragma unroll
    for (int e = 0; e < 2; ++e) rreg[e] = *reinterpret_cast<const f32x4*>(xk + rsrc[e]);
  };
  auto commit = [&]() {
#pragma unroll
    for (int e = 0; e < 2; ++e) {
      float* d = Rs + rdst[e];
      const bool ok = rok[e];
      d[0] = ok ? rreg[e][0] : 0.f; d[1] = ok ? rreg[e][1] : 0.f; d[2] = ok ? rreg[e][2] : 0.f; d[3] = ok ? rreg[e][3] : 0.f;
    }
  };
  auto patch = [&](int k, float (&v)[16]) {
    const float* r = Rs + k * RSP + poff;
    float d[4][4];
#pragma unroll
    for (int a = 0; a < 4; ++a) {
      const float2 lo = *reinterpret_cast<const float2*>(r + a * Wp);
      const float2 hi = *reinterpret_cast<const float2*>(r + a * Wp + 2);
      d[a][0] = lo.x; d[a][1] = lo.y; d[a][2] = hi.x; d[a][3] = hi.y;
    }
    float w[4][4];
#pragma unroll
    for (int j = 0; j < 4; ++j) {
      w[0][j] = d[0][j] - d[2][j];
      w[1][j] = d[1][j] + d[2][j];
      w[2][j] = d[2][j] - d[1][j];
      w[3][j] = d[1][j] - d[3][j];
    }
#pragma unroll
    for (int i = 0; i < 4; ++i) {
      v[4 * i + 0] = w[i][0] - w[i][2];
      v[4 * i + 1] = w[i][1] + w[i][2];
      v[4 * i + 2] = w[i][2] - w[i][1];
      v[4 * i + 3] = w[i][1] - w[i][3];
    }
  };
  const float* ua = U + ((long)(kw / KC) * 16 * N + n0 + li) * 8 + 2 * lq;
  const long xstep = (long)N * 8;
  const int total = nchunks * 16;
  f32x2 abuf[DEPTH][2];
  auto aload = [&](int g, int slot) {
    const float* p = ua + (long)g * xstep;
    abuf[slot][0] = *reinterpret_cast<const f32x2*>(p);
    abuf[slot][1] = *reinterpret_cast<const f32x2*>(p + 128);
  };

  f32x4 acc[16][2];
#pragma unroll
  for (int xi = 0; xi < 16; ++xi)
#pragma unroll
    for (int h = 0; h < 2; ++h) acc[xi][h] = f32x4{0.f, 0.f, 0.f, 0.f};

#pragma unroll
  for (int g = 0; g < DEPTH; ++g) aload(g, g);
  fetch(0);
  for (int c = 0; c < nchunks; ++c) {
    commit();
    if (c + 1 < nchunks) fetch(c + 1);
    float v0[16], v1[16];
    patch(lq, v0);
    patch(lq + 4, v1);
#pragma unroll
    for (int xi = 0; xi < 16; ++xi) {
      const f32x2 lo = abuf[xi % DEPTH][0], hi = abuf[xi % DEPTH][1];
      const int gn = c * 16 + xi + DEPTH;
      if (gn < total) aload(gn, xi % DEPTH);
      __builtin_amdgcn_sched_barrier(0);
      acc[xi][0] = __builtin_amdgcn_mfma_f32_16x16x4f32(lo[0], v0[xi], acc[xi][0], 0, 0, 0);
      acc[xi][1] = __builtin_amdgcn_mfma_f32_16x16x4f32(hi[0], v0[xi], acc[xi][1], 0, 0, 0);
      acc[xi][0] = __builtin_amdgcn_mfma_f32_16x16x4f32(lo[1], v1[xi], acc[xi][0], 0, 0, 0);
      acc[xi][1] = __builtin_amdgcn_mfma_f32_16x16x4f32(hi[1], v1[xi], acc[xi][1], 0, 0, 0);
    }
  }

#pragma unroll
  for (int h = 0; h < 2; ++h)
#pragma unroll
    for (int r = 0; r < 4; ++r) {
      float tcol[4][2];
#pragma unroll
      for (int i = 0; i < 4; ++i) {
        const float m0 = acc[4 * i + 0][h][r], m1 = acc[4 * i + 1][h][r], m2 = acc[4 * i + 2][h][r], m3 = acc[4 * i + 3][h][r];
        tcol[i][0] = (m0 + m1) + m2;
        tcol[i][1] = (m1 - m2) - m3;
      }
      float* o = red + ((wv * 32 + (h * 4 + r) * 4) * 64) + lane;
      o[0] = (tcol[0][0] + tcol[1][0]) + tcol[2][0];
      o[64] = (tcol[0][1] + tcol[1][1]) + tcol[2][1];
      o[128] = (tcol[1][0] - tcol[2][0]) - tcol[3][0];
      o[192] = (tcol[1][1] - tcol[2][1]) - tcol[3][1];
    }
  __syncthreads();
  const int ob = b0 + li / (G::TROWS * G::TPR);
  if (ob >= B) return;
  const int opix = 2 * ((li / G::TPR) % G::TROWS) * W + 2 * (li % G::TPR);
#pragma unroll
  for (int e = 0; e < 2; ++e) {
    const int hr = 2 * wv + e, h = hr >> 2, r = hr & 3;
    float yv[4];
#pragma unroll
    for (int j = 0; j < 4; ++j) {
      const float* q = red + (hr * 4 + j) * 64 + lane;
      yv[j] = (q[0] + q[32 * 64]) + (q[2 * 32 * 64] + q[3 * 32 * 64]);
    }
    const int n = n0 + 16 * h + 4 * lq + r;
    const unsigned idx = (unsigned)((ob * N + n) * HW + opix);
    if (bias) { const float bb = bias[n]; yv[0] += bb; yv[1] += bb; yv[2] += bb; yv[3] += bb; }
    if (act == 1) { yv[0] = gelu_erf(yv[0]); yv[1] = gelu_erf(yv[1]); yv[2] = gelu_erf(yv[2]); yv[3] = gelu_erf(yv[3]); }
    if (res) {
      const float2 r0 = *reinterpret_cast<const float2*>(res + idx), r1 = *reinterpret_cast<const float2*>(res + idx + W);
      yv[0] += r0.x; yv[1] += r0.y; yv[2] += r1.x; yv[3] += r1.y;
    }
    *reinterpret_cast<float2*>(y + idx) = make_float2(yv[0], yv[1]);
    *reinterpret_cast<float2*>(y + idx + W) = make_float2(yv[2], yv[3]);
  }
}

template <int S>
static void wino_sk_launch(const float* x, const float* U, const float* bias, const float* res, float* y, int B, int K, int N, int act,
                           hipStream_t s) {
  using G = WGeo<S, 16>;
  const size_t lds = sizeof(float) * (4 * 8 * G::RSP + 4 * 32 * 64);
  const int tg = (B + G::TI - 1) / G::TI;
  hipLaunchKernelGGL((conv_wino_sk<S>), dim3(N / 32, tg), dim3(256), lds, s, x, U, bias, res, y, B, K, N, act);
}

static int g_wino_grid = 0;
void wino_set_grid(int g) { g_wino_grid = g; }
static int g_wino_mode = 0;
void wino_set_mode(int m) { g_wino_mode = m; }

int wino_plan(int B, int K, int N, int H, int W) {
  if (g_wino_mode == 1) return 0;
  if (H != W || (W != 64 && W != 32 && W != 16 && W != 8 && W != 4)) return 0;
  if (K % 8 || N % 32 || K < 8) return 0;
  if ((long)B * K * H * W >= (1L << 31) || (long)B * N * H * W >= (1L << 31) || (long)16 * N * K >= (1L << 28)) return 0;
  const bool n64 = N % 64 == 0;
  if (g_wino_mode == 2) return (n64 ? 64 : 32) * 256 + 64;
  if (g_wino_mode == 3) return 32 * 256 + 64;
  if (g_wino_mode == 4) return (n64 ? 64 : 32) * 256 + 32;
  if (g_wino_mode == 5) return 32 * 256 + 32;
  const long tiles = (long)B * (H / 2) * (W / 2);
  if (g_wino_mode == 6) return (W <= 8 && K % 32 == 0 && K >= 64) ? 1 : 0;
  if (W <= 8 && K % 32 == 0 && K >= 64 && !(n64 && (tiles / 64) * (N / 64) >= 256) && (tiles / 16) * (N / 32) >= 128) return 1;
  if (K < 32 || W < 8) return 0;
  if (n64 && (tiles / 64) * (N / 64) >= 256) return 64 * 256 + 64;
  if ((tiles / 64) * (N / 32) >= 256) return 32 * 256 + 64;
  return 0;
}

template <int GEO, int BN, int NT>
static void wino_launch_t(const float* x, const float* U, const float* bias, const float* res, float* y, int B, int K, int N, int act,
                          hipStream_t s) {
  using G = WGeo<GEO, NT>;
  const size_t lds = 2 * sizeof(float) * (16 * BN * 10 + 8 * G::RSP);
  (void)lds_opt_in(&conv_wino<GEO, BN, NT>, lds);
  const int tg = G::TI == 1 ? B * G::GPI : (B + G::TI - 1) / G::TI;
  const int items = tg * (N / BN);
  int grid = g_wino_grid > 0 ? g_wino_grid : items;
  if (grid > items) grid = items;
  hipLaunchKernelGGL((conv_wino<GEO, BN, NT>), dim3(grid), dim3(BN * NT / 8), lds, s, x, U, bias, res, y, B, K, N, act, items);
}

bool bf3_ok(int B, int K, int N, int H, int W);
bool direct_form_is_bf3();
void bf3_weights_launch(const float* w, void* Wf, void* Wd, int Cin, int Cout, hipStream_t s);
void bf3_conv(const float* x, const void* Wp, const float* bias, const float* res, float* y, int B, int K, int N, int S, int act,
              hipStream_t s);
void h2_weights_launch(const float* w, void* Wf, void* Wd, int Cin, int Cout, hipStream_t s);
void h2_conv(const float* x, const void* Wp, const float* bias, const float* res, float* y, int B, int K, int N, int S, int act,
             hipStream_t s, bool small);
int direct_plan(int B, int K, int N, int H, int W);

bool wino_conv(const float* x, const float* w, const float* bias, const float* res, float* y, float* U, int B, int K, int N, int H,
               int W, int act, bool dgrad, bool weights_ready, hipStream_t s) {
  const int Cin = dgrad ? N : K, Cout = dgrad ? K : N;
  if (U && bf3_ok(B, K, N, H, W)) {
    if (direct_form_is_bf3()) {
      if (!weights_ready) bf3_weights_launch(w, dgrad ? nullptr : U, dgrad ? U : nullptr, Cin, Cout, s);
      bf3_conv(x, U, bias, res, y, B, K, N, W, act, s);
    } else {
      if (!weights_ready) h2_weights_launch(w, dgrad ? nullptr : U, dgrad ? U : nullptr, Cin, Cout, s);
      h2_conv(x, U, bias, res, y, B, K, N, W, act, s, direct_plan(B, K, N, H, W) == 2);
    }
    return true;
  }
  const int plan = wino_plan(B, K, N, H, W);
  if (!plan || !U) return false;
  const int bn = plan >> 8, nt = plan & 255;
  if (plan == 1) {
    if (!weights_ready)
      hipLaunchKernelGGL(wino_weights, dim3((unsigned)((K * N / 64 + 3) / 4)), dim3(256), 0, s, w, dgrad ? nullptr : U, dgrad ? U : nullptr, Cin, Cout);
    if (W == 4) wino_sk_launch<4>(x, U, bias, res, y, B, K, N, act, s); else wino_sk_launch<8>(x, U, bias, res, y, B, K, N, act, s);
    return true;
  }
  if (!weights_ready)
    hipLaunchKernelGGL(wino_weights, dim3((unsigned)((K * N / 64 + 3) / 4)), dim3(256), 0, s, w, dgrad ? nullptr : U, dgrad ? U : nullptr, Cin, Cout);
#define AFD_WINO(GEO_)                                                                            \
  if (bn == 64 && nt == 64) wino_launch_t<GEO_, 64, 64>(x, U, bias, res, y, B, K, N, act, s);     \
  else if (bn == 32 && nt == 64) wino_launch_t<GEO_, 32, 64>(x, U, bias, res, y, B, K, N, act, s); \
  else if (bn == 64) wino_launch_t<GEO_, 64, 32>(x, U, bias, res, y, B, K, N, act, s);            \
  else wino_launch_t<GEO_, 32, 32>(x, U, bias, res, y, B, K, N, act, s)
  if (W == 64) { AFD_WINO(64); } else if (W == 32) { AFD_WINO(32); } else if (W == 16) { AFD_WINO(16); } else if (W == 8) { AFD_WINO(8); } else { AFD_WINO(4); }
#undef AFD_WINO
  return true;
}


template <int S> struct WgGeo {
  using G = WGeo<S, 16>;
  static constexpr int W = S, HW = S * S, Wp = G::Wp, PXR = G::PXR, TI = G::TI, RTX = PXR + 2, IMG = G::IMG, RS = G::RS;
  static constexpr int RSX = RS + ((4 - RS % 8) + 8) % 8;
  static constexpr int DS = 68;
  static constexpr int poff(int t) { return (t / (G::TROWS * G::TPR)) * IMG + 2 * ((t / G::TPR) % G::TROWS) * Wp + 2 * (t % G::TPR); }
  static constexpr int doff(int t) { return (t / (G::TROWS * G::TPR)) * PXR * W + 2 * ((t / G::TPR) % G::TROWS) * W + 2 * (t % G::TPR); }
};

template <int S, int BN, int BK>
__global__ __launch_bounds__((BN / 32) * (BK / 16) * 64, (BN / 32) * (BK / 16) == 8 ? 1 : 2)
void wgrad_wino(const float* __restrict__ x, const float* __restrict__ dy, float* __restrict__ part,
                int B, int Cin, int Cout, int chunks_per_split, int nchunks) {
  using Q = WgGeo<S>;
  using G = WGeo<S, 16>;
  constexpr int W = S, H = S, HW = S * S, Wp = Q::Wp, PXR = Q::PXR, TI = Q::TI, RTX = Q::RTX, IMG = Q::IMG, RSX = Q::RSX, DS = Q::DS;
  constexpr int NWN = BN / 32, NWK = BK / 16, NTH = NWN * NWK * 64, W4 = W / 4;
  constexpr int XUNITS = BK * TI * RTX * W4, NX = (XUNITS + NTH - 1) / NTH;
  constexpr int DUNITS = BN * TI * PXR * W4, ND = (DUNITS + NTH - 1) / NTH;
  extern __shared__ __attribute__((aligned(16))) float smem[];
  float* Xs = smem;
  float* Gs = smem + BK * RSX;
  const int tid = threadIdx.x, lane = tid & 63, wv = tid >> 6;
  const int n0 = blockIdx.x * BN, k0 = blockIdx.y * BK, split = blockIdx.z;
  const int wn = wv % NWN, wk = wv / NWN;
  const int li = lane & 15, lq = lane >> 4;

  for (int i = tid; i < BK * RSX; i += NTH) Xs[i] = 0.f;

  const int cbeg = split * chunks_per_split, cend = min(nchunks, cbeg + chunks_per_split);
  int f_b = (TI == 1) ? cbeg / G::GPI : cbeg * TI;
  int f_g = (TI == 1) ? cbeg % G::GPI : 0;

  f32x4 xreg[NX], greg[ND];
  unsigned xok, gok;
  auto fetch = [&]() {
    const int row0 = f_g * PXR;
    xok = 0; gok = 0;
#pragma unroll
    for (int e = 0; e < NX; ++e) {
      const int u = tid + NTH * e;
      const int x4 = u % W4, ch = (u / W4) % BK, rl = u / (W4 * BK);
      const int ti = rl / RTX, rr = rl % RTX;
      const int yy = row0 - 1 + rr, b = f_b + ti;
      const bool ok = (XUNITS % NTH == 0 || u < XUNITS) && yy >= 0 && yy < H && b < B;
      const unsigned src = ok ? (unsigned)((b * Cin + k0 + ch) * HW + yy * W + 4 * x4) : 0u;
      xreg[e] = *reinterpret_cast<const f32x4*>(x + src);
      xok |= (ok ? 1u : 0u) << e;
    }
#pragma unroll
    for (int e = 0; e < ND; ++e) {
      const int u = tid + NTH * e;
      const int x4 = u % W4, n = (u / W4) % BN, rl = u / (W4 * BN);
      const int ti = rl / PXR, rr = rl % PXR;
      const int b = f_b + ti;
      const bool ok = (DUNITS % NTH == 0 || u < DUNITS) && b < B;
      const unsigned src = ok ? (unsigned)((b * Cout + n0 + n) * HW + (row0 + rr) * W + 4 * x4) : 0u;
      greg[e] = *reinterpret_cast<const f32x4*>(dy + src);
      gok |= (ok ? 1u : 0u) << e;
    }
    if (TI == 1) { if (++f_g == G::GPI) { f_g = 0; ++f_b; } } else { f_b += TI; }
  };
  auto commit = [&]() {
#pragma unroll
    for (int e = 0; e < NX; ++e) {
      const int u = tid + NTH * e;
      if (XUNITS % NTH == 0 || u < XUNITS) {
        const int x4 = u % W4, ch = (u / W4) % BK, rl = u / (W4 * BK);
        float* d = Xs + ch * RSX + (rl / RTX) * IMG + (rl % RTX) * Wp + 1 + 4 * x4;
        const bool ok = (xok >> e) & 1u;
        d[0] = ok ? xreg[e][0] : 0.f; d[1] = ok ? xreg[e][1] : 0.f; d[2] = ok ? xreg[e][2] : 0.f; d[3] = ok ? xreg[e][3] : 0.f;
      }
    }
#pragma unroll
    for (int e = 0; e < ND; ++e) {
      const int u = tid + NTH * e;
      if (DUNITS % NTH == 0 || u < DUNITS) {
        const int x4 = u % W4, n = (u / W4) % BN, rl = u / (W4 * BN);
        const bool ok = (gok >> e) & 1u;
        f32x4 v = greg[e];
        if (!ok) v = f32x4{0.f, 0.f, 0.f, 0.f};
        *reinterpret_cast<f32x4*>(Gs + n * DS + (rl / PXR) * PXR * W + (rl % PXR) * W + 4 * x4) = v;
      }
    }
  };

  const float* xp = Xs + (wk * 16 + li) * RSX + Q::poff(0) + (lq == 0 ? Q::poff(0) : lq == 1 ? Q::poff(1) : lq == 2 ? Q::poff(2) : Q::poff(3));
  const float* gp = Gs + (wn * 32 + li) * DS + (lq == 0 ? Q::doff(0) : lq == 1 ? Q::doff(1) : lq == 2 ? Q::doff(2) : Q::doff(3));

  f32x4 acc[16][2];
#pragma unroll
  for (int xi = 0; xi < 16; ++xi)
#pragma unroll
    for (int h = 0; h < 2; ++h) acc[xi][h] = f32x4{0.f, 0.f, 0.f, 0.f};

#ifndef AFD_WGW_ABL
#define AFD_WGW_ABL 0
#endif
  if (cbeg < cend) fetch();
  for (int c = cbeg; c < cend; ++c) {
    __syncthreads();
    if (!(AFD_WGW_ABL & 8) || c == cbeg) commit();
    if (c + 1 < cend && (!(AFD_WGW_ABL & 4))) fetch();
    __syncthreads();
#pragma unroll
    for (int s = 0; s < 4; ++s) {
      float v[16];
      {
        const float* r = xp + Q::poff(4 * s);
        float d[4][4];
#pragma unroll
        for (int a = 0; a < 4; ++a) {
          const float2 lo = *reinterpret_cast<const float2*>(r + a * Wp);
          const float2 hi = *reinterpret_cast<const float2*>(r + a * Wp + 2);
          d[a][0] = lo.x; d[a][1] = lo.y; d[a][2] = hi.x; d[a][3] = hi.y;
        }
        float w[4][4];
        if (AFD_WGW_ABL & 1) {
#pragma unroll
          for (int i = 0; i < 16; ++i) v[i] = d[i >> 2][i & 3];
        } else {
#pragma unroll
        for (int j = 0; j < 4; ++j) {
          w[0][j] = d[0][j] - d[2][j];
          w[1][j] = d[1][j] + d[2][j];
          w[2][j] = d[2][j] - d[1][j];
          w[3][j] = d[1][j] - d[3][j];
        }
#pragma unroll
        for (int i = 0; i < 4; ++i) {
          v[4 * i + 0] = w[i][0] - w[i][2];
          v[4 * i + 1] = w[i][1] + w[i][2];
          v[4 * i + 2] = w[i][2] - w[i][1];
          v[4 * i + 3] = w[i][1] - w[i][3];
        }
        }
      }
#pragma unroll
      for (int h = 0; h < 2; ++h) {
        const float* q = gp + h * 16 * DS + Q::doff(4 * s);
        const float2 r0 = *reinterpret_cast<const float2*>(q), r1 = *reinterpret_cast<const float2*>(q + W);
        const float a = r0.x, b = r0.y, cc = r1.x, d = r1.y;
        const float ac = a + cc, bd = b + d, amc = a - cc, bmd = b - d;
        float m[16];
        m[0] = a;    m[1] = a + b;     m[2] = a - b;     m[3] = b;
        m[4] = ac;   m[5] = ac + bd;   m[6] = ac - bd;   m[7] = bd;
        m[8] = amc;  m[9] = amc + bmd; m[10] = amc - bmd; m[11] = bmd;
        m[12] = cc;  m[13] = cc + d;   m[14] = cc - d;   m[15] = d;
#pragma unroll
        for (int xi = 0; xi < 16; ++xi) {
          if (AFD_WGW_ABL & 2) { asm volatile("" :: "v"(m[xi]), "v"(v[xi])); }
          else acc[xi][h] = __builtin_amdgcn_mfma_f32_16x16x4f32(m[xi], v[xi], acc[xi][h], 0, 0, 0);
        }
      }
    }
  }

  float* out = part + (long)split * Cout * Cin * 9;
  const long plane = (long)Cout * Cin;
  const int kk = k0 + wk * 16 + li;
#pragma unroll
  for (int h = 0; h < 2; ++h)
#pragma unroll
    for (int r = 0; r < 4; ++r) {
      const unsigned o = (unsigned)((n0 + wn * 32 + 16 * h + 4 * lq + r) * Cin + kk);
      float t[3][4];
#pragma unroll
      for (int j = 0; j < 4; ++j) {
        const float sg3 = (j == 3) ? 1.f : -1.f;
        const float u0 = (j == 3) ? -acc[j][h][r] : acc[j][h][r];
        const float u1 = (j == 3) ? -acc[4 + j][h][r] : acc[4 + j][h][r];
        const float u2 = (j == 3) ? -acc[8 + j][h][r] : acc[8 + j][h][r];
        const float u3 = sg3 * acc[12 + j][h][r];
        const float hs = 0.5f * (u1 + u2), hd = 0.5f * (u1 - u2);
        t[0][j] = u0 + hs; t[1][j] = hd; t[2][j] = hs + u3;
      }
#pragma unroll
      for (int a = 0; a < 3; ++a) {
        const float hs = 0.5f * (t[a][1] + t[a][2]), hd = 0.5f * (t[a][1] - t[a][2]);
        (out + (3 * a + 0) * plane)[o] = t[a][0] + hs;
        (out + (3 * a + 1) * plane)[o] = hd;
        (out + (3 * a + 2) * plane)[o] = hs + t[a][3];
      }
    }
}

static int g_wgwino_mode = 0;
void wgrad_wino_set_mode(int m) { g_wgwino_mode = m; }

int wgrad_wino_plan(int B, int Cin, int Cout, int H, int W, int* bn, int* bk, int* cps, int* nchunks) {
  if (g_wgwino_mode == 1) return 0;
  if (H != W || (W != 32 && W != 16 && W != 8 && W != 4)) return 0;
  if (Cin % 32 || Cout % 32) return 0;
  if ((long)B * H * W * (Cin > Cout ? Cin : Cout) >= (1L << 31)) return 0;
  const int tpi = (W / 2) * (W / 2);
  const int nch = tpi >= 16 ? B * (tpi / 16) : (B + 16 / tpi - 1) / (16 / tpi);
  const int BN = Cout % 64 == 0 ? 64 : 32, BK = Cin % 64 == 0 ? 64 : 32;
  const int waves = (BN / 32) * (BK / 16);
  const long blocks = (long)(Cout / BN) * (Cin / BK);
  static const long target = [] { const char* e = getenv("AFD_WGW_TARGET"); return e ? atol(e) : 128L; }();
  long s = (target * (waves == 8 ? 1 : (waves == 4 ? 2 : 4))) / blocks;
  if (s < 1) s = 1;
  if (s > nch) s = nch;
  const int c = (int)((nch + s - 1) / s);
  *bn = BN; *bk = BK; *cps = c; *nchunks = nch;
  return (nch + c - 1) / c;
}

template <int S, int BN, int BK>
static void wgrad_wino_launch_t(const float* x, const float* dy, float* part, int B, int Cin, int Cout, int cps, int nch, int splits,
                                hipStream_t s) {
  using Q = WgGeo<S>;
  const size_t lds = sizeof(float) * ((size_t)BK * Q::RSX + (size_t)BN * Q::DS);
  (void)lds_opt_in(&wgrad_wino<S, BN, BK>, lds);
  hipLaunchKernelGGL((wgrad_wino<S, BN, BK>), dim3(Cout / BN, Cin / BK, splits), dim3((BN / 32) * (BK / 16) * 64), lds, s,
                     x, dy, part, B, Cin, Cout, cps, nch);
}

int wgrad_wino(const float* x, const float* dy, float* part, int B, int Cin, int Cout, int H, int W, hipStream_t s) {
  int bn, bk, cps, nch;
  const int splits = wgrad_wino_plan(B, Cin, Cout, H, W, &bn, &bk, &cps, &nch);
  if (!splits) return 0;
#define AFD_WGW(S_)                                                                                              \
  if (bn == 64 && bk == 64) wgrad_wino_launch_t<S_, 64, 64>(x, dy, part, B, Cin, Cout, cps, nch, splits, s);     \
  else if (bn == 32 && bk == 64) wgrad_wino_launch_t<S_, 32, 64>(x, dy, part, B, Cin, Cout, cps, nch, splits, s); \
  else if (bn == 64) wgrad_wino_launch_t<S_, 64, 32>(x, dy, part, B, Cin, Cout, cps, nch, splits, s);            \
  else wgrad_wino_launch_t<S_, 32, 32>(x, dy, part, B, Cin, Cout, cps, nch, splits, s)
  if (W == 32) { AFD_WGW(32); } else if (W == 16) { AFD_WGW(16); } else if (W == 8) { AFD_WGW(8); } else { AFD_WGW(4); }
#undef AFD_WGW
  return splits;
}

void wino_weights_launch(const float* w, float* Uf, float* Ud, int Cin, int Cout, int kinds, hipStream_t s) {
  float* wf = (kinds & 1) ? nullptr : Uf; float* wd = (kinds & 2) ? nullptr : Ud;
  if (wf || wd) hipLaunchKernelGGL(wino_weights, dim3((unsigned)((Cin * Cout / 64 + 3) / 4)), dim3(256), 0, s, w, wf, wd, Cin, Cout);
  void* bf = (kinds & 1) ? Uf : nullptr; void* bd = (kinds & 2) ? Ud : nullptr;
  if (bf || bd) {
    if (kinds & 4) bf3_weights_launch(w, bf, bd, Cin, Cout, s);
    else h2_weights_launch(w, bf, bd, Cin, Cout, s);
  }
}

void wino_weights_batched_launch(const afd_wino_desc* descs, const int* wg_desc, int n_wg, hipStream_t s) {
  hipLaunchKernelGGL(h2_wscale_batched, dim3((unsigned)n_wg), dim3(256), 0, s, descs, wg_desc);
  hipLaunchKernelGGL(wino_weights_batched, dim3((unsigned)n_wg), dim3(256), 0, s, descs, wg_desc);
}

}
```

### include/afd.h

```cpp
#ifndef AFD_H_
#define AFD_H_

#include <stddef.h>
#include <stdint.h>

#ifdef __cplusplus
extern "C" {
#endif

#define AFD_OK 0
#define AFD_EINVAL 1
#define AFD_ELAUNCH 2
#define AFD_MAX_TAPS 15

typedef void* afd_stream_t;

const char* afd_version(void);
const char* afd_last_error(void);
int afd_device_count(void);

int afd_lowpass_kernel(double omega_c, int N, int has_beta, double beta, float* taps_out);

int afd_filt_up2_fwd(const float* x, float* y, int B, int C, int H, int W, long x_bstride, long y_bstride,
                     const float* taps, int N, afd_stream_t stream);
int afd_filt_up2_bwd(const float* dy, float* dx, int B, int C, int H, int W, long dy_bstride, long dx_bstride,
                     const float* taps, int N, afd_stream_t stream);

int afd_filt_down2_fwd(const float* x, float* y, int B, int C, int H, int W, long x_bstride, long y_bstride,
                       const float* taps, int N, afd_stream_t stream);
int afd_filt_down2_bwd(const float* dy, float* dx, int B, int C, int H, int W, long dy_bstride, long dx_bstride,
                       const float* taps, int N, afd_stream_t stream);

size_t afd_filt_act_workspace_bytes(int B, int C, int H, int W, int N, int backward);
int afd_filt_act_fwd(const float* x, float* y, int B, int C, int H, int W,
                     const float* stats, const float* gamma, const float* beta, const float* res,
                     const float* taps_up, const float* taps_down, int N,
                     void* workspace, afd_stream_t stream);
size_t afd_filt_act_fwd_gn_supported(int C, int H, int W, int N);
int afd_filt_act_fwd_gn(const float* x, float* y, int B, int C, int H, int W, float eps, float* stats_out,
                        const float* gamma, const float* beta, const float* res,
                        const float* taps_up, const float* taps_down, int N, afd_stream_t stream);
int afd_filt_act_bwd_gn(const float* x, const float* dy, float* dx, float* dres, int B, int C, int H, int W, const float* stats,
                        const float* gamma, const float* beta, const float* res, const float* taps_up, const float* taps_down, int N,
                        float* gn_partials, afd_stream_t stream);
int afd_filt_act_bwd(const float* x, const float* dy, float* dv, int B, int C, int H, int W,
                     const float* stats, const float* gamma, const float* beta, const float* res,
                     const float* taps_up, const float* taps_down, int N,
                     void* workspace, float* gn_partials, afd_stream_t stream);

int afd_groupnorm1_fwd(const float* x, float* y, float* stats_out, int B, int C, int HW, float eps,
                       const float* gamma, const float* beta, const float* res, int act, const float* emb,
                       afd_stream_t stream);
int afd_debug_norm_path(int mode);
int afd_groupnorm1_bwd(const float* x, const float* dy, const float* stats, int B, int C, int HW,
                       const float* gamma, const float* beta, const float* res, int act,
                       float* dx, float* dres, float* dgamma_dbeta_partial , float* demb ,
                       int have_partials ,
                       float* dgamma , float* dbeta , int accumulate, afd_stream_t stream);
int afd_colsum(const float* in, float* out, int rows, int cols, int accumulate, afd_stream_t stream);
int afd_colsum_strided(const float* in, long row_stride, float* out, int rows, int cols, int accumulate, afd_stream_t stream);
int afd_colsum2(const float* in, float* out_a, float* out_b, int rows, int C, int accumulate, afd_stream_t stream);

int afd_debug_conv_path(int mode);
int afd_conv_fwd(const float* x, const float* w, const float* bias, const float* res, float* y,
                 int B, int Cin, int Cout, int H, int W, int ksize, int act, afd_stream_t stream);
int afd_conv_dgrad(const float* dy, const float* w, float* dx,
                   int B, int Cin, int Cout, int H, int W, int ksize, afd_stream_t stream);
size_t afd_conv_wgrad_workspace_bytes(int B, int Cin, int Cout, int H, int W, int ksize);
int afd_conv_wgrad_form(int B, int Cin, int Cout, int H, int W, int ksize);
int afd_conv_wgrad(const float* x, const float* dy, float* dw, float* dbias ,
                   int B, int Cin, int Cout, int H, int W, int ksize, int accumulate,
                   void* workspace, afd_stream_t stream);

typedef struct afd_fold_desc {
  const float* part;
  float* dst;
  long n;
  long stride;
  long inner, rstride;
  int splits;
  int accumulate;
} afd_fold_desc;
int afd_fold_batched(const afd_fold_desc* descs, int n, afd_stream_t stream);
int afd_conv_wgrad_partials(const float* x, const float* dy, float* dw, float* dbias ,
                            int B, int Cin, int Cout, int H, int W, int ksize, int accumulate,
                            void* workspace, afd_fold_desc* folds_out, int* n_folds, afd_stream_t stream);

size_t afd_conv3x3_wino_workspace_bytes(int B, int Cin, int Cout, int H, int W, int dgrad);
int afd_conv3x3_wino_weights(const float* w, float* u_fwd, float* u_dgrad, int Cin, int Cout, int kinds, afd_stream_t stream);
int afd_conv3x3_weight_kinds(int B, int Cin, int Cout, int H, int W);
typedef struct afd_wino_desc {
  const float* w;
  float* u_fwd;
  float* u_dgrad;
  int Cin, Cout, first_wg, kinds;
} afd_wino_desc;
int afd_conv3x3_wino_weights_batched(const afd_wino_desc* descs, const int* wg_desc, int n_wg, afd_stream_t stream);
int afd_conv3x3_wino_fwd(const float* x, const float* w, const float* bias, const float* res, float* y,
                         int B, int Cin, int Cout, int H, int W, int act, void* workspace, int weights_ready, int kinds,
                         afd_stream_t stream);
int afd_conv3x3_wino_dgrad(const float* dy, const float* w, float* dx, const float* add_to_dx ,
                           int B, int Cin, int Cout, int H, int W, void* workspace, int weights_ready, int kinds,
                           afd_stream_t stream);

int afd_layernorm_c_fwd(const float* x, float* y, float* stats_out, int B, int C, int HW, float eps,
                        const float* gamma, const float* beta, afd_stream_t stream);
int afd_layernorm_c_bwd(const float* x, const float* dy, const float* stats, int B, int C, int HW,
                        const float* gamma, float* dx, const float* add_to_dx ,
                        float* dgamma_dbeta_partial ,
                        float* dgamma , float* dbeta , int accumulate,
                        afd_stream_t stream);
int afd_layernorm_c_bwd_params(const float* x, const float* dy, const float* stats, int B, int C, int HW,
                               float* dgamma_dbeta_partial , float* dgamma, float* dbeta, int accumulate,
                               afd_stream_t stream);
int afd_layernorm_c_bwd_partials(const float* x, const float* dy, const float* stats, int B, int C, int HW, float* part,
                                 afd_stream_t stream);

int afd_debug_attn_rows(int rows);
int afd_attn_fwd(const float* qkv, float* o, float* lse, int B, int heads, int d, int L, afd_stream_t stream);
int afd_attn_bwd(const float* qkv, const float* o, const float* d_o, const float* lse, float* dqkv,
                 float* delta_workspace , int B, int heads, int d, int L, afd_stream_t stream);

int afd_tok_supported(int C);
int afd_debug_tok_grid(int max_workgroups);
int afd_debug_tok_path(int mode);
int afd_tok_head_fwd(const float* x, const float* gamma, const float* beta, const float* w_in, const float* b_in,
                     float* h_out, float* stats_out, float* qkv, int B, int C, int P, float eps, afd_stream_t stream);
int afd_tok_tail_fwd(const float* att, const float* x, const float* w_o, const float* b_o, const float* gamma, const float* beta,
                     const float* w_1, const float* b_1, const float* w_2, const float* b_2,
                     float* a_out, float* stats_out, float* f_out, float* u_out, float* g_out, float* out,
                     int B, int C, int P, float eps, afd_stream_t stream);
int afd_tok_tail_bwd(const float* d_out, const float* u, const float* a, const float* stats, const float* gamma,
                     const float* w_2, const float* w_1, const float* w_o,
                     float* du_out, float* df_out, float* da_out, float* datt_out, int B, int C, int P, afd_stream_t stream);
int afd_tok_head_bwd(const float* dqkv, const float* x, const float* stats, const float* gamma, const float* w_in,
                     const float* d_res, float* dh_out, float* dx_out, int B, int C, int P, afd_stream_t stream);

int afd_gelu_fwd(const float* x, float* y, long n, afd_stream_t stream);
int afd_gelu_bwd(const float* x, const float* dy, float* dx, long n, afd_stream_t stream);
int afd_maxpool2_fwd(const float* x, float* y, int B, int C, int H, int W, afd_stream_t stream);
int afd_maxpool2_bwd(const float* x, const float* dy, float* dx, int B, int C, int H, int W, afd_stream_t stream);
int afd_bilinear_up2_fwd(const float* x, float* y, int B, int C, int H, int W, long y_bstride, afd_stream_t stream);
int afd_bilinear_up2_bwd(const float* dy, float* dx, int B, int C, int H, int W, long dy_bstride, afd_stream_t stream);
int afd_copy_batched(const float* src, float* dst, int B, long n, long src_bstride, long dst_bstride, afd_stream_t stream);
int afd_add(const float* a, const float* b, float* y, long n, afd_stream_t stream);

int afd_pos_encoding(const int64_t* t, const float* inv_freq, float* temb, int B, int half, afd_stream_t stream);
int afd_silu_linear_fwd(const float* temb, const float* w, const float* bias, float* out,
                        int B, int K, int N, afd_stream_t stream);
int afd_silu_linear_bwd(const float* temb, const float* w, const float* dout, float* dw, float* dbias,
                        float* dtemb , int B, int K, int N, int accumulate, afd_stream_t stream);
typedef struct afd_silu_desc {
  const float* w;
  const float* bias;
  float* out;
  int N;
} afd_silu_desc;
int afd_silu_linear_fwd_batched(const float* temb, const afd_silu_desc* descs, int n, int B, int K, afd_stream_t stream);
int afd_gather_rows_batched(const int64_t* idx, const afd_silu_desc* descs, int n, int B, int rows, afd_stream_t stream);

int afd_embed_add_fwd(const float* temb, const float* table, const int64_t* y, float* out, int B, int D, int num_classes,
                      afd_stream_t stream);
int afd_label_embed_add_fwd(const float* temb, const float* table, const int64_t* y, float* out, int B, int D, int num_classes,
                            afd_stream_t stream);
int afd_embed_add_bwd(const float* dout, const int64_t* y, float* dtable, int B, int D, int num_classes, int accumulate,
                      afd_stream_t stream);

int afd_noise_images(const float* x, const float* eps, const int64_t* t, const float* alpha_hat,
                     float* x_t, int B, long per_sample, afd_stream_t stream);
int afd_denoise_step(const float* x, const float* eps_pred, const float* noise ,
                     const float* alpha, const float* alpha_hat, const float* beta, int i,
                     float* x_out, long n, afd_stream_t stream);
int afd_denoise_step_dev(const float* x, const float* eps_pred, const float* noise,
                         const float* alpha, const float* alpha_hat, const float* beta, const int64_t* t_dev,
                         float* x_out, long n, afd_stream_t stream);
int afd_denoise_step_cfg(const float* x, const float* eps2, const float* noise ,
                         const float* alpha, const float* alpha_hat, const float* beta, int i, float cfg_scale,
                         float* x_out, float* x_out2, long n, afd_stream_t stream);
int afd_denoise_step_cfg_dev(const float* x, const float* eps2, const float* noise,
                             const float* alpha, const float* alpha_hat, const float* beta, const int64_t* t_dev, float cfg_scale,
                             float* x_out, float* x_out2, long n, afd_stream_t stream);
int afd_ddim_step(const float* x, const float* eps, const float* noise , const float* alpha_hat, int t, int t_prev,
                  float eta, float* x_out, long n, afd_stream_t stream);
int afd_ddim_step_dev(const float* x, const float* eps, const float* noise, const float* alpha_hat, const int64_t* t_dev,
                      const int64_t* t_prev_dev, float eta, float* x_out, long n, afd_stream_t stream);
int afd_ddim_step_cfg(const float* x, const float* eps2, const float* noise, const float* alpha_hat, int t, int t_prev, float eta,
                      float cfg_scale, float* x_out, float* x_out2, long n, afd_stream_t stream);
int afd_ddim_step_cfg_dev(const float* x, const float* eps2, const float* noise, const float* alpha_hat, const int64_t* t_dev,
                          const int64_t* t_prev_dev, float eta, float cfg_scale, float* x_out, float* x_out2, long n,
                          afd_stream_t stream);
int afd_dpmpp_step(const float* x, const float* eps, const float* x0_prev , const float* coef, float* x_out,
                   float* x0_out, long n, afd_stream_t stream);
int afd_dpmpp_step_cfg(const float* x, const float* eps2, const float* x0_prev, const float* coef, float cfg_scale, float* x_out,
                       float* x_out2, float* x0_out, long n, afd_stream_t stream);
int afd_noise_images_gather(const float* x0, long n_img, const int64_t* img, const float* eps, const int64_t* t, const float* alpha_hat,
                            float* x_t, long rows, long per, afd_stream_t stream);
int afd_vlb_terms(const float* x0, long n_img, const int64_t* img, const float* x_t, const float* eps, const float* eps_hat,
                  const int64_t* t, const double* coef, long T, const float* alpha, const float* alpha_hat, const float* beta,
                  double* term, double* sq, long rows, long per, afd_stream_t stream);
int afd_vlb_prior(const float* x0, double half_ah, double* out, long n_img, long per, afd_stream_t stream);
int afd_denoise_step_masked(const float* x, const float* eps_pred, const float* noise, const float* x0, const uint8_t* mask,
                            const float* alpha, const float* alpha_hat, const float* beta, int i, float* x_out, long n,
                            afd_stream_t stream);
int afd_denoise_step_masked_dev(const float* x, const float* eps_pred, const float* noise, const float* x0, const uint8_t* mask,
                                const float* alpha, const float* alpha_hat, const float* beta, const int64_t* t_dev, float* x_out,
                                long n, afd_stream_t stream);
int afd_denoise_step_masked_cfg(const float* x, const float* eps2, const float* noise, const float* x0, const uint8_t* mask,
                                const float* alpha, const float* alpha_hat, const float* beta, int i, float cfg_scale, float* x_out,
                                float* x_out2, long n, afd_stream_t stream);
int afd_denoise_step_masked_cfg_dev(const float* x, const float* eps2, const float* noise, const float* x0, const uint8_t* mask,
                                    const float* alpha, const float* alpha_hat, const float* beta, const int64_t* t_dev,
                                    float cfg_scale, float* x_out, float* x_out2, long n, afd_stream_t stream);
int afd_ddim_step_masked(const float* x, const float* eps, const float* noise, const float* x0, const uint8_t* mask,
                         const float* alpha_hat, int t, int t_prev, float eta, float* x_out, long n, afd_stream_t stream);
int afd_ddim_step_masked_dev(const float* x, const float* eps, const float* noise, const float* x0, const uint8_t* mask,
                             const float* alpha_hat, const int64_t* t_dev, const int64_t* t_prev_dev, float eta, float* x_out, long n,
                             afd_stream_t stream);
int afd_ddim_step_masked_cfg(const float* x, const float* eps2, const float* noise, const float* x0, const uint8_t* mask,
                             const float* alpha_hat, int t, int t_prev, float eta, float cfg_scale, float* x_out, float* x_out2, long n,
                             afd_stream_t stream);
int afd_ddim_step_masked_cfg_dev(const float* x, const float* eps2, const float* noise, const float* x0, const uint8_t* mask,
                                 const float* alpha_hat, const int64_t* t_dev, const int64_t* t_prev_dev, float eta, float cfg_scale,
                                 float* x_out, float* x_out2, long n, afd_stream_t stream);
int afd_renoise(const float* x, const float* noise, const float* alpha_hat, int t_from, int t_to, float* x_out, long n,
                afd_stream_t stream);
int afd_quantize_u8(const float* x, uint8_t* out, long n, afd_stream_t stream);

size_t afd_rotate_workspace_bytes(long planes, int H, int W);
int afd_affine_spline3_wrap(const float* x, float* y, long planes, int H, int W, const double* matrix4, const double* offset2,
                            void* workspace, afd_stream_t stream);
int afd_spline3_prefilter_wrap(const float* x, double* coef, long planes, int H, int W, afd_stream_t stream);
int afd_affine_spline3_wrap_rows(const double* coef, long n_src, const int64_t* img, const double* affine, long K, const int64_t* k,
                                 float* out, long rows, int C, int H, int W, afd_stream_t stream);
int afd_eq_terms(const double* coef, long n_src, const int64_t* img, const double* affine, long K, const int64_t* k, const float* g,
                 double margin, double* out, long rows, int C, int H, int W, afd_stream_t stream);

int afd_mse_fwd(const float* pred, const float* target, float* loss_out, float* workspace, long n, afd_stream_t stream);
int afd_mse_bwd(const float* pred, const float* target, const float* dloss, float* dpred, long n, afd_stream_t stream);
int afd_adamw_tick(float* state, float beta1, float beta2, afd_stream_t stream);
int afd_adamw_step(float* p, const float* g, float* m, float* v, long n, const float* state,
                   float lr, float beta1, float beta2, float eps, float weight_decay, float grad_scale,
                   afd_stream_t stream);

int afd_ema_step(float* ema, const float* p, long n, int copy, float beta, float one_minus_beta, afd_stream_t stream);
int afd_adamw_ema_tick(float* adam_state, float beta1, float beta2, int* ema_state, int start, afd_stream_t stream);
int afd_adamw_ema_step(float* p, const float* g, float* m, float* v, long n_active, const float* adam_state, float lr,
                       float beta1, float beta2, float eps, float weight_decay, float grad_scale, float* ema, long n_ema,
                       const int* ema_state, float beta, float one_minus_beta, afd_stream_t stream);

#define AFD_LR_CONSTANT 0
#define AFD_LR_LINEAR 1
#define AFD_LR_COSINE 2
typedef struct afd_opt_ctl {
  double base_lr;
  long warmup, total;
  int kind;
  double min_ratio;
  double max_norm;
  int skip_nonfinite;
} afd_opt_ctl;
int afd_grad_sqnorm_n_partials(void);
int afd_grad_sqnorm_partials(const float* g, long n, float grad_scale, double* partials, int n_partials, afd_stream_t stream);
int afd_adamw_ctl_tick(float* adam_state, float beta1, float beta2, int* ema_state, int ema_start, const double* partials,
                       int n_partials, const afd_opt_ctl* cfg, double* ctl, afd_stream_t stream);
int afd_adamw_ctl_step(float* p, const float* g, float* m, float* v, long n_active, const float* adam_state, const double* ctl,
                       float beta1, float beta2, float eps, float weight_decay, float grad_scale, float* ema, long n_ema,
                       const int* ema_state, float beta, float one_minus_beta, afd_stream_t stream);

int afd_replay_build(void* hip_graph, void** out_handle, int* counts);
int afd_replay_run(void* handle, afd_stream_t main_stream, afd_stream_t side_stream);
int afd_replay_free(void* handle);

#ifdef __cplusplus
}
#endif
#endif
```

Measured before the change: 38500 images/s.

## Add persistent tile-walk variant of h2 3x3 conv kernels for 32x32 maps

```diff
diff --git a/aliasfree-diffusion-models-pytorch_amd/csrc/conv.hip b/aliasfree-diffusion-models-pytorch_amd/csrc/conv.hip
--- a/aliasfree-diffusion-models-pytorch_amd/csrc/conv.hip
+++ b/aliasfree-diffusion-models-pytorch_amd/csrc/conv.hip
@@ -730,8 +730,8 @@
                int act, bool dgrad, hipStream_t s);
 void pw_set_mode(int m);
 int wino_plan(int B, int K, int N, int H, int W);
-bool wino_conv(const float* x, const float* w, const float* bias, const float* res, float* y, float* U, int B, int K, int N, int H,
-               int W, int act, bool dgrad, bool weights_ready, hipStream_t s);
+int wino_conv(const float* x, const float* w, const float* bias, const float* res, float* y, float* U, int B, int K, int N, int H,
+              int W, int act, bool dgrad, bool weights_ready, hipStream_t s);
 void wino_set_mode(int m);
 void wino_weights_launch(const float* w, float* Uf, float* Ud, int Cin, int Cout, int kinds, hipStream_t s);
 bool bf3_ok(int B, int K, int N, int H, int W);
@@ -740,6 +740,9 @@
 bool direct_form_is_bf3();
 void h2_sk_set_mode(int m);
 void h2_lds_set(int m);
+void h2_pw_set(int m);
+void h2_grid_set(int g);
+int h2_walk_grid(long tiles, int blocks, int tpi, long slots, bool forced);
 void wino_weights_batched_launch(const afd_wino_desc* descs, const int* wg_desc, int n_wg, hipStream_t s);
 void wino_set_grid(int g);
 int wgrad_wino_plan(int B, int Cin, int Cout, int H, int W, int* bn, int* bk, int* cps, int* nchunks);
@@ -868,6 +871,8 @@
   if (mode >= 84 && mode <= 86) { wgrad_bf3_set_mode(mode - 84); return AFD_OK; }
   if (mode >= 48 && mode <= 49) { wgrad_plan_target_set(mode == 48 ? 256 : 160); return AFD_OK; }
   if (mode >= 59 && mode <= 63) { h2_lds_set(mode == 59 ? 4 : (mode == 60 ? 1 : (mode == 61 ? 0 : mode - 60))); return AFD_OK; }
+  if (mode >= 56 && mode <= 58) { h2_pw_set(mode - 56); return AFD_OK; }
+  if (mode >= 200000 && mode < 300000) { h2_grid_set(mode - 200000); return AFD_OK; }
   if (mode == 73) { h2_sk_set_mode(2); return AFD_OK; }
   if (mode >= 74 && mode <= 75) { h2_sk_set_mode(mode - 74); return AFD_OK; }
   if (mode >= 78 && mode <= 79) { wgrad_arith_set(mode - 78); return AFD_OK; }
@@ -880,6 +885,12 @@
   if (mode >= 32 && mode <= 34) { g_wgrad_nw = mode == 32 ? 4 : (mode == 33 ? 8 : 0); return AFD_OK; }
   AFD_REQUIRE(mode >= 0 && mode <= 2, "afd_debug_conv_path: mode must be 0 (auto), 1 (big tile), 2 (split-K tile), 8..10 (1x1 streaming auto/off/forced), 32..34 (wgrad waves 4/8/auto), 64..69 (Winograd fwd/dgrad auto/off/forced shapes) or 96..98 (Winograd wgrad auto/off/forced)");
   g_conv_path = mode;
+  return AFD_OK;
+}
+
+int afd_conv3x3_walk_grid(int tiles, int blocks, int tiles_per_image, int slots, int forced, int* grid_x) {
+  AFD_REQUIRE(tiles > 0 && blocks > 0 && tiles_per_image > 0 && slots > 0 && grid_x, "afd_conv3x3_walk_grid: bad argument");
+  *grid_x = h2_walk_grid(tiles, blocks, tiles_per_image, slots, forced != 0);
   return AFD_OK;
 }
 
@@ -960,8 +971,9 @@
   AFD_REQUIRE(x && w && y && workspace && B > 0 && Cin > 0 && Cout > 0 && H > 0 && W > 0, "afd_conv3x3_wino_fwd: bad argument");
   AFD_REQUIRE(act == 0 || act == 1, "afd_conv3x3_wino_fwd: act must be 0 or 1");
   if (weights_ready && check_kinds("afd_conv3x3_wino_fwd", kinds, B, Cin, Cout, H, W, 0) != AFD_OK) return AFD_EINVAL;
-  AFD_REQUIRE(wino_conv(x, w, bias, res, y, static_cast<float*>(workspace), B, Cin, Cout, H, W, act, false, weights_ready != 0, as_stream(st)),
-              "afd_conv3x3_wino_fwd: shape (%d,%d->%d,%dx%d) is not covered (afd_conv3x3_wino_workspace_bytes returns 0 for it)", B, Cin, Cout, H, W);
+  const int rc = wino_conv(x, w, bias, res, y, static_cast<float*>(workspace), B, Cin, Cout, H, W, act, false, weights_ready != 0, as_stream(st));
+  if (rc < 0) return AFD_ELAUNCH;
+  AFD_REQUIRE(rc, "afd_conv3x3_wino_fwd: shape (%d,%d->%d,%dx%d) is not covered (afd_conv3x3_wino_workspace_bytes returns 0 for it)", B, Cin, Cout, H, W);
   return check_launch("afd_conv3x3_wino_fwd");
 }
 
@@ -969,8 +981,9 @@
                            void* workspace, int weights_ready, int kinds, afd_stream_t st) {
   AFD_REQUIRE(dy && w && dx && workspace && B > 0 && Cin > 0 && Cout > 0 && H > 0 && W > 0, "afd_conv3x3_wino_dgrad: bad argument");
   if (weights_ready && check_kinds("afd_conv3x3_wino_dgrad", kinds, B, Cin, Cout, H, W, 1) != AFD_OK) return AFD_EINVAL;
-  AFD_REQUIRE(wino_conv(dy, w, nullptr, add_to_dx, dx, static_cast<float*>(workspace), B, Cout, Cin, H, W, 0, true, weights_ready != 0, as_stream(st)),
-              "afd_conv3x3_wino_dgrad: shape (%d,%d->%d,%dx%d) is not covered", B, Cin, Cout, H, W);
+  const int rc = wino_conv(dy, w, nullptr, add_to_dx, dx, static_cast<float*>(workspace), B, Cout, Cin, H, W, 0, true, weights_ready != 0, as_stream(st));
+  if (rc < 0) return AFD_ELAUNCH;
+  AFD_REQUIRE(rc, "afd_conv3x3_wino_dgrad: shape (%d,%d->%d,%dx%d) is not covered", B, Cin, Cout, H, W);
   return check_launch("afd_conv3x3_wino_dgrad");
 }
 
diff --git a/aliasfree-diffusion-models-pytorch_amd/csrc/h2.hip b/aliasfree-diffusion-models-pytorch_amd/csrc/h2.hip
--- a/aliasfree-diffusion-models-pytorch_amd/csrc/h2.hip
+++ b/aliasfree-diffusion-models-pytorch_amd/csrc/h2.hip
@@ -32,6 +32,16 @@
 __global__ __launch_bounds__(256) void h2_weights(const float* __restrict__ w, void* Wf, void* Wd, int Cin, int Cout) {
   h2_weights_block(w, Wf, Wd, Cin, Cout, blockIdx.x * 4 + (threadIdx.x >> 6), threadIdx.x & 63);
 }
+
+#define AFD_LDS_BARRIER()                                                                                                 \
+  do {                                                                                                                    \
+    __builtin_amdgcn_sched_barrier(0);                                                                                    \
+    __builtin_amdgcn_s_waitcnt(0xC07F);                                                               \
+    asm volatile("" ::: "memory");                                                                                        \
+    __builtin_amdgcn_s_barrier();                                                                                         \
+    asm volatile("" ::: "memory");                                                                                        \
+    __builtin_amdgcn_sched_barrier(0);                                                                                    \
+  } while (0)
 
 template <int S> struct H2Geo {
   static constexpr int TP = 128;
@@ -48,11 +58,12 @@
   }
 };
 
-template <int S, int NBLK>
+template <int S, int NBLK, bool PW = false>
 __global__ __launch_bounds__(256, 2) void conv_h2(const float* __restrict__ x, const h8* __restrict__ Wp,
                                                   const float* __restrict__ bias, const float* __restrict__ res,
-                                                  float* __restrict__ y, int B, int K, int N, int act) {
+                                                  float* __restrict__ y, int B, int K, int N, int act, int tiles) {
   using G = H2Geo<S>;
+  static_assert(!PW || (G::IPT == 1 && AFD_H2_ABL == 0), "the persistent walk is built for the maps with whole tiles per image");
   constexpr int PSW = 2 * NBLK, NPIX = G::NPIX, NPP = G::NPP, NE = G::NE;
   extern __shared__ __attribute__((aligned(16))) uint8_t smem_raw[];
   h8* Xp = reinterpret_cast<h8*>(smem_raw);
@@ -65,9 +76,10 @@
 #endif
   const int tid = threadIdx.x, lane = tid & 63, wv = tid >> 6, kgl = lane >> 4, l15 = lane & 15;
   const int nb = wv % NBLK, pgrp = wv / NBLK;
-  const int tile = blockIdx.x, n0 = (blockIdx.y * NBLK + nb) * 32;
-  const int img0 = G::IPT > 1 ? tile * G::IPT : tile / G::TPI;
-  const int row0 = G::IPT > 1 ? 0 : (tile % G::TPI) * G::R;
+  int tile = blockIdx.x;
+  const int n0 = (blockIdx.y * NBLK + nb) * 32;
+  int img0 = G::IPT > 1 ? tile * G::IPT : tile / G::TPI;
+  int row0 = G::IPT > 1 ? 0 : (tile % G::TPI) * G::R;
   const int HW = S * S;
 
   int s_src[NE];
@@ -85,6 +97,17 @@
     }
   }
   const float* xb = x + (long)img0 * K * HW;
+  auto replan = [&](int r0) {
+#pragma unroll
+    for (int e = 0; e < NE; ++e) {
+      const int t = tid + 256 * e;
+      if (t < G::TASKS) {
+        const int kg = t / NPIX, ridx = t - kg * NPIX;
+        const int rr = ridx / G::Wp, cc = ridx - rr * G::Wp, yy = r0 + rr - 1, xx = cc - 1;
+        s_src[e] = (yy >= 0 && yy < S && xx >= 0 && xx < S) ? (8 * kg * S + yy) * S + xx : -1;
+      }
+    }
+  };
   float xr[NE][8];
   auto fetch = [&](int k0) {
 #pragma unroll
@@ -122,10 +145,6 @@
     bbase[ps] = kgl * NPP + i * G::IMG + r * G::Wp + c;
   }
   f32x4 acc[2][PSW];
-#pragma unroll
-  for (int ns = 0; ns < 2; ++ns)
-#pragma unroll
-    for (int ps = 0; ps < PSW; ++ps) acc[ns][ps] = f32x4{0.f, 0.f, 0.f, 0.f};
 
   const int KS = K >> 5, nit = KS * 9;
   const long pstride = (long)9 * (K >> 3) * N;
@@ -142,12 +161,29 @@
   for (int d = 0; d < AQ; ++d)
     if (d < nit) a_load(aq[d], d);
 
+  fetch(0);
+  const float* isw = reinterpret_cast<const float*>(reinterpret_cast<const uint8_t*>(Wp) + h2_scale_offset_bytes(K, N));
+  const int cn = lane >> 3, cm = lane & 7;
+  float sw[4], bv[4];
+  if constexpr (PW) {
+#pragma unroll
+    for (int it = 0; it < 4; ++it) { sw[it] = isw[n0 + 8 * it + cn]; bv[it] = bias ? bias[n0 + 8 * it + cn] : 0.f; }
+#pragma unroll
+    for (int it = 0; it < 4; ++it) asm volatile("" : "+v"(sw[it]), "+v"(bv[it]));
+  }
+  for (;;) {
+  const int tnext = tile + (int)gridDim.x;
+  const bool more = PW && tnext < tiles;
+#pragma unroll
+  for (int ns = 0; ns < 2; ++ns)
+#pragma unroll
+    for (int ps = 0; ps < PSW; ++ps) acc[ns][ps] = f32x4{0.f, 0.f, 0.f, 0.f};
   float sx = __uint_as_float(kH2ScaleCapBits);
-  fetch(0);
   int it = 0;
   for (int k0 = 0; k0 < K; k0 += 32) {
     const bool stage = !(AFD_H2_ABL & 8) || k0 == 0;
     if (stage) chunk_amax();
+    if constexpr (PW) AFD_LDS_BARRIER(); else
     __syncthreads();
     if (stage) {
       const float m = fmaxf(fmaxf(wmax[0], wmax[1]), fmaxf(wmax[2], wmax[3]));
@@ -162,7 +198,7 @@
       }
     }
     if (stage) commit(sx);
-    __syncthreads();
+    if constexpr (PW) AFD_LDS_BARRIER(); else __syncthreads();
     h8 bc[2], bn[2];
     bc[0] = Xp[bbase[0]]; bc[1] = Xp[G::KG * NPP + bbase[0]];
 #pragma unroll
@@ -175,8 +211,15 @@
 #pragma unroll
         for (int ns = 0; ns < 2; ++ns) { aq[d][ns][0] = aq[d + 1][ns][0]; aq[d][ns][1] = aq[d + 1][ns][1]; }
       if (it + AQ < nit && !(AFD_H2_ABL & 2)) a_load(aq[AQ - 1], it + AQ);
+      else if (more) a_load(aq[AQ - 1], it + AQ - nit);
       ++it;
       if (tap == 0 && k0 + 32 < K && !(AFD_H2_ABL & 4)) fetch(k0 + 32);
+      if (PW && tap == 0 && k0 + 32 >= K && more) {
+        const int nrow0 = (tnext % G::TPI) * G::R;
+        if (nrow0 != row0) replan(nrow0);
+        xb = x + (long)(tnext / G::TPI) * K * HW;
+        fetch(0);
+      }
 #pragma unroll
       for (int ps = 0; ps < PSW; ++ps) {
         const int u = tap * PSW + ps + 1;
@@ -200,14 +243,13 @@
   }
 
   if ((AFD_H2_ABL & 32) && act != 77) return;
-  const float* isw = reinterpret_cast<const float*>(reinterpret_cast<const uint8_t*>(Wp) + h2_scale_offset_bytes(K, N));
   const float isx = h2_inv_pow2(sx);
-  __syncthreads();
+  if constexpr (PW) AFD_LDS_BARRIER(); else __syncthreads();
   float* T = reinterpret_cast<float*>(smem_raw) + wv * (32 * 36);
-  const int cn = lane >> 3, cm = lane & 7;
-  float sw[4], bv[4];
-#pragma unroll
-  for (int it = 0; it < 4; ++it) { sw[it] = isw[n0 + 8 * it + cn]; bv[it] = bias ? bias[n0 + 8 * it + cn] : 0.f; }
+  if constexpr (!PW) {
+#pragma unroll
+    for (int it = 0; it < 4; ++it) { sw[it] = isw[n0 + 8 * it + cn]; bv[it] = bias ? bias[n0 + 8 * it + cn] : 0.f; }
+  }
 #pragma unroll
   for (int pp = 0; pp < PSW / 2; ++pp) {
 #pragma unroll
@@ -234,6 +276,9 @@
       if (res) v += *reinterpret_cast<const f32x4*>(res + o);
       *reinterpret_cast<f32x4*>(y + o) = v;
     }
+  }
+  if (!more) break;
+  tile = tnext; img0 = tile / G::TPI; row0 = (tile % G::TPI) * G::R;
   }
 }
 
@@ -252,11 +297,12 @@
   }
 };
 
-template <int S, int TP, int NB>
+template <int S, int TP, int NB, bool PW = false>
 __global__ __launch_bounds__(256, 2) void conv_h2l(const float* __restrict__ x, const h8* __restrict__ Wp,
                                                    const float* __restrict__ bias, const float* __restrict__ res,
-                                                   float* __restrict__ y, int B, int K, int N, int act) {
+                                                   float* __restrict__ y, int B, int K, int N, int act, int tiles) {
   using G = H2LGeo<S, TP>;
+  static_assert(!PW || G::IPT == 1, "the persistent walk is built for the maps with whole tiles per image");
   constexpr int NT = 32 * NB, PGR = 4 / NB, PB = TP / 32 / PGR;
   constexpr int NPIX = G::NPIX, NPP = G::NPP, NE = G::NE;
   constexpr int XREC = 2 * G::KG * NPP;
@@ -268,9 +314,10 @@
   float* wmax = reinterpret_cast<float*>(Ab + 2 * AROW);
   const int tid = threadIdx.x, lane = tid & 63, wv = tid >> 6, l31 = lane & 31, lh = lane >> 5;
   const int nb = wv % NB, pgrp = wv / NB;
-  const int tile = blockIdx.x, n0w = blockIdx.y * NT, n0 = n0w + 32 * nb;
-  const int img0 = G::IPT > 1 ? tile * G::IPT : tile / G::TPI;
-  const int row0 = G::IPT > 1 ? 0 : (tile % G::TPI) * G::R;
+  int tile = blockIdx.x;
+  const int n0w = blockIdx.y * NT, n0 = n0w + 32 * nb;
+  int img0 = G::IPT > 1 ? tile * G::IPT : tile / G::TPI;
+  int row0 = G::IPT > 1 ? 0 : (tile % G::TPI) * G::R;
   const int HW = S * S;
 #if AFD_H2_SLEEP
   if (((blockIdx.y * gridDim.x + blockIdx.x) >> 8) & 1) { for (int z = 0; z < AFD_H2_SLEEP / 100; ++z) __builtin_amdgcn_s_sleep(100); }
@@ -300,6 +347,17 @@
     }
   }
   const float* xb = x + (long)img0 * K * HW;
+  auto replan = [&](int r0) {
+#pragma unroll
+    for (int e = 0; e < NE; ++e) {
+      const int t = tid + 256 * e;
+      if (t < G::TASKS) {
+        const int kg = t / NPIX, ridx = t - kg * NPIX;
+        const int rr = ridx / G::Wp, cc = ridx - rr * G::Wp, yy = r0 + rr - 1, xx = cc - 1;
+        s_src[e] = (yy >= 0 && yy < S && xx >= 0 && xx < S) ? (8 * kg * S + yy) * S + xx : -1;
+      }
+    }
+  };
   float xr[NE][8];
   auto fetch = [&](int k0) {
 #pragma unroll
@@ -338,10 +396,10 @@
     const int pc = pt / 3, tx = pt - 3 * pc;
     soff[d] = ((pc * 9 + tx) * K8 + kg) * N + n0w + n;
   }
-  auto dma_row = [&](int q) {
+  auto dma_row = [&](int q, int buf) {
     const int ks = q / 3, ty = q - 3 * ks;
     const h8* src = Wp + (long)(ty * 3 * K8 + 4 * ks) * N;
-    h8* dst = Ab + (q & 1) * AROW + wv * CPW * 64;
+    h8* dst = Ab + buf * AROW + wv * CPW * 64;
 #pragma unroll
     for (int d = 0; d < CPW; ++d)
       __builtin_amdgcn_global_load_lds((const __attribute__((address_space(1))) void*)(src + soff[d]),
@@ -357,7 +415,7 @@
     __builtin_amdgcn_sched_barrier(0);                                                                                    \
   } while (0)
 
-  dma_row(0);
+  dma_row(0, 0);
   fetch(0);
   AFD_STAMP();
 
@@ -370,14 +428,30 @@
   }
   const int abase = lh * NT + 32 * nb + l31;
   f32x16 acc[PB];
+
+  const int KS = K >> 5, nrows = 3 * KS;
+  const float* isw = reinterpret_cast<const float*>(reinterpret_cast<const uint8_t*>(Wp) + h2_scale_offset_bytes(K, N));
+  const int cn = lane >> 3, cm = lane & 7;
+  float sw[4], bv[4];
+  if constexpr (PW) {
+#pragma unroll
+    for (int it = 0; it < 4; ++it) { sw[it] = isw[n0 + 8 * it + cn]; bv[it] = bias ? bias[n0 + 8 * it + cn] : 0.f; }
+#pragma unroll
+    for (int it = 0; it < 4; ++it) asm volatile("" : "+v"(sw[it]), "+v"(bv[it]));
+  }
+  AFD_STAMP();
+  int qb = 0;
+  for ([[maybe_unused]] bool first = true;; first = false) {
+  const int tnext = tile + (int)gridDim.x;
+  const bool more = PW && tnext < tiles;
+#if AFD_H2_STAMP
+  if (!first) { si = 0; AFD_STAMP(); AFD_STAMP(); AFD_STAMP(); }
+#endif
 #pragma unroll
   for (int pb = 0; pb < PB; ++pb)
 #pragma unroll
     for (int j = 0; j < 16; ++j) acc[pb][j] = 0.f;
-
-  const int KS = K >> 5, nrows = 3 * KS;
   float sx = __uint_as_float(kH2ScaleCapBits);
-  AFD_STAMP();
   int q = 0;
   for (int k0 = 0; k0 < K; k0 += 32) {
     chunk_amax();
@@ -385,6 +459,7 @@
     __builtin_amdgcn_s_waitcnt(0x0F70);
     __builtin_amdgcn_sched_barrier(0);
     if (k0 < 64) AFD_STAMP();
+    if constexpr (PW) AFD_LDS_BARRIER(); else
     __syncthreads();
     {
       const float m = fmaxf(fmaxf(wmax[0], wmax[1]), fmaxf(wmax[2], wmax[3]));
@@ -397,14 +472,22 @@
       }
     }
     commit(sx);
+    if constexpr (PW) AFD_LDS_BARRIER(); else
     __syncthreads();
     if (k0 < 64) AFD_STAMP();
 #pragma unroll
-    for (int ty = 0; ty < 3; ++ty, ++q) {
-      if (q + 1 < nrows) dma_row(q + 1);
-      const bool prefetch = ty == 1 && k0 + 32 < K;
-      if (prefetch) fetch(k0 + 32);
-      const h8* Ar = Ab + (q & 1) * AROW + abase;
+    for (int ty = 0; ty < 3; ++ty, ++q, ++qb) {
+      if (q + 1 < nrows) dma_row(q + 1, (qb + 1) & 1);
+      else if (more) dma_row(0, (qb + 1) & 1);
+      const bool lastc = k0 + 32 >= K;
+      const bool prefetch = ty == 1 && (!lastc || more);
+      if (PW && prefetch && lastc) {
+        const int nrow0 = (tnext % G::TPI) * G::R;
+        if (nrow0 != row0) replan(nrow0);
+        xb = x + (long)(tnext / G::TPI) * K * HW;
+      }
+      if (prefetch) fetch(lastc ? 0 : k0 + 32);
+      const h8* Ar = Ab + (qb & 1) * AROW + abase;
       constexpr int U = 3 * 2 * PB;
       h8 ac[2], an[2], bc[2], bn[2];
       ac[0] = Ar[0]; ac[1] = Ar[3 * 4 * NT];
@@ -434,18 +517,18 @@
     }
   }
 
-  const float* isw = reinterpret_cast<const float*>(reinterpret_cast<const uint8_t*>(Wp) + h2_scale_offset_bytes(K, N));
   const float isx = h2_inv_pow2(sx);
 #if AFD_H2_STAMP
   si = 13;
 #endif
   AFD_STAMP();
+  if constexpr (PW) AFD_LDS_BARRIER(); else
   __syncthreads();
   float* T = reinterpret_cast<float*>(smem_raw) + wv * (32 * 36);
-  const int cn = lane >> 3, cm = lane & 7;
-  float sw[4], bv[4];
-#pragma unroll
-  for (int it = 0; it < 4; ++it) { sw[it] = isw[n0 + 8 * it + cn]; bv[it] = bias ? bias[n0 + 8 * it + cn] : 0.f; }
+  if constexpr (!PW) {
+#pragma unroll
+    for (int it = 0; it < 4; ++it) { sw[it] = isw[n0 + 8 * it + cn]; bv[it] = bias ? bias[n0 + 8 * it + cn] : 0.f; }
+  }
 #pragma unroll
   for (int pb = 0; pb < PB; ++pb) {
 #pragma unroll
@@ -470,6 +553,9 @@
     }
   }
   AFD_STAMP();
+  if (!more) break;
+  tile = tnext; img0 = tile / G::TPI; row0 = (tile % G::TPI) * G::R;
+  }
 #undef AFD_STAMP
 }
 
@@ -649,14 +735,49 @@
   hipLaunchKernelGGL(h2_weights, dim3((unsigned)((Cin * Cout / 64 + 3) / 4)), dim3(256), 0, s, w, Wf, Wd, Cin, Cout);
 }
 
+static int g_h2_pw = 0, g_h2_grid = 0;
+void h2_pw_set(int m) { g_h2_pw = m; }
+void h2_grid_set(int g) { g_h2_grid = g; }
+int h2_walk_grid(long tiles, int blocks, int tpi, long slots, bool forced) {
+  long gx = slots / blocks;
+  if (gx < 1) gx = 1;
+  if (gx >= tiles) return (int)tiles;
+  if (!forced && gx >= tpi) gx -= gx % tpi;
+  return (int)gx;
+}
+static long h2_slots() {
+  static long cached[16] = {0};
+  int dev = 0;
+  if (hipGetDevice(&dev) != hipSuccess || dev < 0 || dev >= 16) return 512;
+  if (!cached[dev]) {
+    int cus = 0;
+    cached[dev] = hipDeviceGetAttribute(&cus, hipDeviceAttributeMultiprocessorCount, dev) == hipSuccess && cus > 0 ? 2L * cus : 512;
+  }
+  return cached[dev];
+}
+static int h2_pw_grid(long tiles, int blocks, int tpi, int S) {
+  if (S != 32 || g_h2_pw == 1) return 0;
+  const long slots = g_h2_grid > 0 ? g_h2_grid : h2_slots();
+  if (g_h2_pw == 0 && tiles * blocks <= slots) return 0;
+  return h2_walk_grid(tiles, blocks, tpi, slots, g_h2_grid > 0);
+}
+
 template <int S, int NBLK>
-static void h2_launch_t(const float* x, const void* Wp, const float* bias, const float* res, float* y, int B, int K, int N, int act,
-                        hipStream_t s) {
+static int h2_launch_t(const float* x, const void* Wp, const float* bias, const float* res, float* y, int B, int K, int N, int act,
+                       hipStream_t s) {
   using G = H2Geo<S>;
   const size_t lds = (size_t)2 * G::KG * G::NPP * 16 + 16;
   const long tiles = G::IPT > 1 ? ((long)B + G::IPT - 1) / G::IPT : (long)B * G::TPI;
+  if constexpr (S == 32) {
+    if (const int gx = h2_pw_grid(tiles, N / (32 * NBLK), G::TPI, S)) {
+      hipLaunchKernelGGL((conv_h2<S, NBLK, true>), dim3((unsigned)gx, (unsigned)(N / (32 * NBLK))), dim3(256), lds, s, x,
+                         static_cast<const h8*>(Wp), bias, res, y, B, K, N, act, (int)tiles);
+      return AFD_OK;
+    }
+  }
   hipLaunchKernelGGL((conv_h2<S, NBLK>), dim3((unsigned)tiles, (unsigned)(N / (32 * NBLK))), dim3(256), lds, s, x,
-                     static_cast<const h8*>(Wp), bias, res, y, B, K, N, act);
+                     static_cast<const h8*>(Wp), bias, res, y, B, K, N, act, (int)tiles);
+  return AFD_OK;
 }
 template <int S, int KSP>
 static void h2_sk_launch_t(const float* x, const void* Wp, const float* bias, const float* res, float* y, int B, int K, int N, int act,
@@ -682,10 +803,18 @@
                         hipStream_t s) {
   using G = H2LGeo<S, TP>;
   const size_t lds = (size_t)(2 * G::KG * G::NPP + 2 * 2 * 3 * 4 * 32 * NB) * 16 + 16 + AFD_H2_LDSPAD;
+  const long tiles = G::IPT > 1 ? ((long)B + G::IPT - 1) / G::IPT : (long)B * G::TPI;
+  if constexpr (S == 32) {
+    if (const int gx = h2_pw_grid(tiles, N / (32 * NB), G::TPI, S)) {
+      if (int rc = lds_opt_in(conv_h2l<S, TP, NB, true>, lds)) return rc;
+      hipLaunchKernelGGL((conv_h2l<S, TP, NB, true>), dim3((unsigned)gx, (unsigned)(N / (32 * NB))), dim3(256), lds, s, x,
+                         static_cast<const h8*>(Wp), bias, res, y, B, K, N, act, (int)tiles);
+      return AFD_OK;
+    }
+  }
   if (int rc = lds_opt_in(conv_h2l<S, TP, NB>, lds)) return rc;
-  const long tiles = G::IPT > 1 ? ((long)B + G::IPT - 1) / G::IPT : (long)B * G::TPI;
   hipLaunchKernelGGL((conv_h2l<S, TP, NB>), dim3((unsigned)tiles, (unsigned)(N / (32 * NB))), dim3(256), lds, s, x,
-                     static_cast<const h8*>(Wp), bias, res, y, B, K, N, act);
+                     static_cast<const h8*>(Wp), bias, res, y, B, K, N, act, (int)tiles);
   return AFD_OK;
 }
 template <int S>
@@ -700,24 +829,23 @@
   return h2l_launch_t<S, 128, 1>(x, Wp, bias, res, y, B, K, N, act, s);
 }
 
-void h2_conv(const float* x, const void* Wp, const float* bias, const float* res, float* y, int B, int K, int N, int S, int act,
+int h2_conv(const float* x, const void* Wp, const float* bias, const float* res, float* y, int B, int K, int N, int S, int act,
              hipStream_t s, bool small) {
   if (small) {
     if (S == 4) { if (K >= 128) h2_sk_launch_t<4, 4>(x, Wp, bias, res, y, B, K, N, act, s); else h2_sk_launch_t<4, 2>(x, Wp, bias, res, y, B, K, N, act, s); }
     else { if (K >= 128) h2_sk_launch_t<8, 4>(x, Wp, bias, res, y, B, K, N, act, s); else h2_sk_launch_t<8, 2>(x, Wp, bias, res, y, B, K, N, act, s); }
-    return;
+    return AFD_OK;
   }
   if (g_h2_lds > 1 || (g_h2_lds == 1 && S == 32 && N % 64 != 0)) {
-    if (S == 32) h2l_launch<32>(x, Wp, bias, res, y, B, K, N, act, s);
-    else if (S == 16) h2l_launch<16>(x, Wp, bias, res, y, B, K, N, act, s);
-    else h2l_launch<8>(x, Wp, bias, res, y, B, K, N, act, s);
-    return;
+    if (S == 32) return h2l_launch<32>(x, Wp, bias, res, y, B, K, N, act, s);
+    if (S == 16) return h2l_launch<16>(x, Wp, bias, res, y, B, K, N, act, s);
+    return h2l_launch<8>(x, Wp, bias, res, y, B, K, N, act, s);
   }
   const int nblk = h2_nblk(((long)B * S * S + 127) / 128, N, S);
 #define AFD_H2(S_)                                                                      \
-  if (nblk == 4 && S_ == 16) h2_launch_t<16, 4>(x, Wp, bias, res, y, B, K, N, act, s);  \
-  else if (nblk == 2) h2_launch_t<S_, 2>(x, Wp, bias, res, y, B, K, N, act, s);         \
-  else h2_launch_t<S_, 1>(x, Wp, bias, res, y, B, K, N, act, s)
+  if (nblk == 4 && S_ == 16) return h2_launch_t<16, 4>(x, Wp, bias, res, y, B, K, N, act, s);  \
+  else if (nblk == 2) return h2_launch_t<S_, 2>(x, Wp, bias, res, y, B, K, N, act, s);         \
+  else return h2_launch_t<S_, 1>(x, Wp, bias, res, y, B, K, N, act, s)
   if (S == 32) { AFD_H2(32); } else if (S == 16) { AFD_H2(16); } else { AFD_H2(8); }
 #undef AFD_H2
 }
diff --git a/aliasfree-diffusion-models-pytorch_amd/csrc/wino.hip b/aliasfree-diffusion-models-pytorch_amd/csrc/wino.hip
--- a/aliasfree-diffusion-models-pytorch_amd/csrc/wino.hip
+++ b/aliasfree-diffusion-models-pytorch_amd/csrc/wino.hip
@@ -500,11 +500,11 @@
 void bf3_conv(const float* x, const void* Wp, const float* bias, const float* res, float* y, int B, int K, int N, int S, int act,
               hipStream_t s);
 void h2_weights_launch(const float* w, void* Wf, void* Wd, int Cin, int Cout, hipStream_t s);
-void h2_conv(const float* x, const void* Wp, const float* bias, const float* res, float* y, int B, int K, int N, int S, int act,
-             hipStream_t s, bool small);
+int h2_conv(const float* x, const void* Wp, const float* bias, const float* res, float* y, int B, int K, int N, int S, int act,
+            hipStream_t s, bool small);
 int direct_plan(int B, int K, int N, int H, int W);
 
-bool wino_conv(const float* x, const float* w, const float* bias, const float* res, float* y, float* U, int B, int K, int N, int H,
+int wino_conv(const float* x, const float* w, const float* bias, const float* res, float* y, float* U, int B, int K, int N, int H,
                int W, int act, bool dgrad, bool weights_ready, hipStream_t s) {
   const int Cin = dgrad ? N : K, Cout = dgrad ? K : N;
   if (U && bf3_ok(B, K, N, H, W)) {
@@ -513,18 +513,18 @@
       bf3_conv(x, U, bias, res, y, B, K, N, W, act, s);
     } else {
       if (!weights_ready) h2_weights_launch(w, dgrad ? nullptr : U, dgrad ? U : nullptr, Cin, Cout, s);
-      h2_conv(x, U, bias, res, y, B, K, N, W, act, s, direct_plan(B, K, N, H, W) == 2);
-    }
-    return true;
+      if (h2_conv(x, U, bias, res, y, B, K, N, W, act, s, direct_plan(B, K, N, H, W) == 2) != AFD_OK) return -1;
+    }
+    return 1;
   }
   const int plan = wino_plan(B, K, N, H, W);
-  if (!plan || !U) return false;
+  if (!plan || !U) return 0;
   const int bn = plan >> 8, nt = plan & 255;
   if (plan == 1) {
     if (!weights_ready)
       hipLaunchKernelGGL(wino_weights, dim3((unsigned)((K * N / 64 + 3) / 4)), dim3(256), 0, s, w, dgrad ? nullptr : U, dgrad ? U : nullptr, Cin, Cout);
     if (W == 4) wino_sk_launch<4>(x, U, bias, res, y, B, K, N, act, s); else wino_sk_launch<8>(x, U, bias, res, y, B, K, N, act, s);
-    return true;
+    return 1;
   }
   if (!weights_ready)
     hipLaunchKernelGGL(wino_weights, dim3((unsigned)((K * N / 64 + 3) / 4)), dim3(256), 0, s, w, dgrad ? nullptr : U, dgrad ? U : nullptr, Cin, Cout);
@@ -535,7 +535,7 @@
   else wino_launch_t<GEO_, 32, 32>(x, U, bias, res, y, B, K, N, act, s)
   if (W == 64) { AFD_WINO(64); } else if (W == 32) { AFD_WINO(32); } else if (W == 16) { AFD_WINO(16); } else if (W == 8) { AFD_WINO(8); } else { AFD_WINO(4); }
 #undef AFD_WINO
-  return true;
+  return 1;
 }
 
 
diff --git a/include/afd.h b/include/afd.h
--- a/include/afd.h
+++ b/include/afd.h
@@ -62,6 +62,7 @@
 int afd_colsum2(const float* in, float* out_a, float* out_b, int rows, int C, int accumulate, afd_stream_t stream);
 
 int afd_debug_conv_path(int mode);
+int afd_conv3x3_walk_grid(int tiles, int blocks, int tiles_per_image, int slots, int forced, int* grid_x);
 int afd_conv_fwd(const float* x, const float* w, const float* bias, const float* res, float* y,
                  int B, int Cin, int Cout, int H, int W, int ksize, int act, afd_stream_t stream);
 int afd_conv_dgrad(const float* dy, const float* w, float* dx,
```

After: 38520 images/s (median of 5 runs). No clear change (+0.1%).
